# ErickRosete/tacorl

Hardware: NVIDIA B200
Metric: play_lmp_train_frames_per_sec (higher is better)
Workload: dtype bf16

## Files before the change

### include/tacorl_b200.h

```cpp
#ifndef TACORL_B200_H_
#define TACORL_B200_H_

#include <stddef.h>

#ifdef __cplusplus
extern "C" {
#endif

#define TACORL_B200_ABI_VERSION 7

#define TACORL_PREC_F32 0
#define TACORL_PREC_BF16 1

#define TACORL_ACT_NONE 0
#define TACORL_ACT_RELU 1
#define TACORL_ACT_SILU 2

const char* tacorl_last_error(void);
int tacorl_abi_version(void);
unsigned long long tacorl_launch_count(void);

int tacorl_set_sm_reserve(int n);

int tacorl_gemm(int transA, int transB, int M, int N, int K, float alpha, const float* A, long long lda,
                const float* B, long long ldb, float beta, float* C, long long ldc, const float* bias, int act,
                float* Cpre, long long ldpre, void* ws, size_t ws_bytes, int prec, void* stream);
int tacorl_gemm_ex(int transA, int transB, int M, int N, int K, float alpha, const float* A, long long lda,
                   const float* B, long long ldb, float beta, float* C, long long ldc, const float* bias, int act,
                   float* Cpre, long long ldpre, const void* A_bf16, const void* B_bf16, void* ws, size_t ws_bytes,
                   int prec, void* stream);
int tacorl_colsum(int M, int N, const float* X, long long ldx, float* out, int accumulate, void* stream);
int tacorl_act_bwd(int act, long long n, const float* dY, const float* y_or_pre, float* dZ, void* stream);
int tacorl_scale(long long n, const float* x, const float* dev_scalar, float c, float* out, void* stream);
int tacorl_rowscale(long long rows, int L, const float* x, const float* row_scalars, float k, float* out,
                    int accumulate, void* stream);

size_t tacorl_lmp_encoder_ws_bytes(int N, int H, int W, int hidden, int latent, int backward);
int tacorl_lmp_encoder_fwd(const void* x, int x_dtype, float x_scale, float x_shift, int N, int H, int W,
                           const float* const* params, int hidden,
                           int latent, float* y1, float* y2, float* y3, float* feat, float* smax,
                           float* ssum, float* h4, float* emb, void* xs, void* ws, size_t ws_bytes, int prec,
                           void* stream);
int tacorl_lmp_encoder_bwd(const void* x, int x_dtype, float x_scale, float x_shift, int N, int H, int W,
                           const float* const* params, int hidden,
                           int latent, const float* y1, const float* y2, const float* y3,
                           const float* feat, const float* smax, const float* ssum, const float* h4,
                           const float* d_emb, float* const* grads, int accumulate, const void* xs, void* ws,
                           size_t ws_bytes, int prec, void* stream);

int tacorl_conv_tc_debug(int op, const float* in0, const float* in1, const float* Wt, const float* bias, int N,
                         int H, int W, float* out, void* ws, size_t ws_bytes, void* stream);

size_t tacorl_rnn_layer_ws_bytes(int T, int B, int I, int H);
unsigned tacorl_rnn_seq_timeouts(void);
int tacorl_rnn_seq_enable(int on);
int tacorl_rnn_layer_fwd(int T, int B, int I, int H, const float* x, long long ldx, const float* w_ih,
                         const float* w_hh, const float* b_ih, const float* b_hh, const float* h0,
                         int reverse, int n_steps, float* out, long long ldo, const void* w_ih_bf16,
                         const void* w_hh_bf16, void* h_bf16_out, void* ws, size_t ws_bytes, int prec, void* stream);
int tacorl_rnn_layer_bwd(int T, int B, int I, int H, const float* x, long long ldx, const float* w_ih,
                         const float* w_hh, const float* h0, int reverse, int n_steps, const float* out,
                         long long ldo, float* dout, long long lddo, const float* dhn, float* dx,
                         long long lddx, int dx_accumulate, float* dw_ih, float* dw_hh, float* db_ih,
                         float* db_hh, int accumulate, float* dh0, const void* w_ih_bf16, const void* w_hh_t_bf16,
                         const void* h_bf16, void* ws, size_t ws_bytes, int prec, void* stream);
size_t tacorl_rnn_layer2_ws_bytes(int T, int B, int I, int H, int D);
int tacorl_rnn_layer2_fwd(int T, int B, int I, int H, int D, const float* x, long long ldx, const void* x_bf16,
                          long long ldxb, const float* const* w, const void* const* w_bf16, const int* n_steps,
                          float* out, long long ldo, void* out_bf16, void* ws, size_t ws_bytes, void* stream);
int tacorl_rnn_layer2_bwd(int T, int B, int grad_rows, int I, int H, int D, const float* x, long long ldx, const void* x_bf16,
                          long long ldxb, const float* const* w, const void* const* w_bf16, const int* n_steps,
                          const float* out, long long ldo, const void* out_bf16, float* dout, long long lddo,
                          void* dpre_bf16, float* dx, long long lddx, float* const* dw, void* ws, size_t ws_bytes,
                          void* stream);
int tacorl_cast_transpose_bf16(const float* src, int rows, int cols, void* dst, void* stream);

int tacorl_dlm_nll(int rows, int act_dims, const float* logits, long long ld, const float* actions,
                   long long lda, int num_classes, float act_min, float act_max, float gripper_alpha,
                   float* row_loss, float* loss_out, float* dlogits, long long ldd, void* stream);
int tacorl_dlm_sample(int rows, int act_dims, const float* logits, long long ld, const float* u1,
                      const float* u2, const float* actions, long long lda, float grip_lo, float grip_hi,
                      float* pred, float* hit, float* acc_out, void* stream);

int tacorl_gauss_head_fwd(int rows, int L, const float* raw, float* mean, float* stdv, void* stream);
int tacorl_gauss_head_bwd(int rows, int L, const float* raw, const float* stdv, const float* dmean,
                          const float* dstd, float* draw, void* stream);
int tacorl_softplus_head_fwd(int rows, int L, const float* raw, float min_std, float* mean, float* stdv,
                             void* stream);
int tacorl_softplus_head_bwd(int rows, int L, const float* raw, const float* dmean, const float* dstd,
                             float* draw, void* stream);
int tacorl_gripper_gumbel(int rows, int rows0, const float* logits, const float* u, int clamp_u, float* index,
                          float* action, void* stream);
int tacorl_gripper_logprob(int rows, int rows0, const float* logits, const float* index, float* logp, void* stream);
int tacorl_gripper_logprob_bwd(int rows, const float* logits, const float* index, const float* dlogp, float* dlogits,
                               void* stream);
int tacorl_kl_balanced(int B, int L, const float* mu_q, const float* sd_q, const float* mu_p,
                       const float* sd_p, float kl_alpha, int balancing, float* kl_out, float* dmu_q,
                       float* dsd_q, float* dmu_p, float* dsd_p, void* stream);
int tacorl_tanh_rsample_fwd(long long n, long long bcast, const float* mu, const float* sd, const float* eps,
                            float* a, float* z, int apply_tanh, void* stream);
int tacorl_tanh_rsample_bwd(long long n, const float* a, const float* eps, const float* da, const float* dz,
                            float* dmu, float* dsd, int apply_tanh, void* stream);
int tacorl_tanh_logprob(int rows, int L, int bcast_rows, const float* mu, const float* sd, const float* z,
                        int from_value, float* logp, float* gmu, float* gsd, float* gz, void* stream);

int tacorl_posemb_fwd(int B, int T, int D0, int D, const float* emb, const float* pos, const float* mask, float* x,
                      void* stream);
int tacorl_posemb_bwd(int B, int T, int D0, int D, const float* dx, const float* mask, float* demb, float* dpos,
                      void* stream);
int tacorl_attn_fwd(int B, int T, int D, int heads, const float* qkv, const float* amask, float* P, float* out,
                    void* stream);
int tacorl_attn_bwd(int B, int T, int D, int heads, const float* qkv, const float* amask, const float* P,
                    const float* dout, float* dqkv, void* stream);
int tacorl_add_ln_fwd(int rows, int D, const float* x, const float* r, const float* mask, const float* w,
                      const float* b, float eps, float* y, float* xhat, float* rstd, void* stream);
int tacorl_add_ln_bwd(int rows, int D, const float* dy, const float* xhat, const float* rstd, const float* w,
                      const float* mask, float* dx, float* dr, float* dw, float* db, void* stream);
int tacorl_mean_t_fwd(int B, int T, int C, const float* x, float* y, void* stream);
int tacorl_mean_t_bwd(int B, int T, int C, const float* dy, float* dx, void* stream);
int tacorl_mul(long long n, const float* a, const float* b, float* out, void* stream);

#define TACORL_CQL_NUM_SCALARS 14
int tacorl_cql_critic_loss(int B, int n, const float* q1_all, const float* q2_all, const float* lp_curr,
                           const float* lp_next, const float* tq1, const float* tq2, const float* reward,
                           const float* done, const float* log_alpha_prime, float rand_density, float discount,
                           float reward_scale, float gap, float conservative_weight, float temp,
                           int with_lagrange, float* scalars, float* dq1_all, float* dq2_all,
                           float* d_log_alpha_prime, void* stream);
int tacorl_cql_actor_loss(int mode, int B, const float* log_pi, const float* a, const float* b,
                          const float* log_alpha, float target_entropy, float* out, float* d_log_alpha,
                          float* d_log_pi, float* da, float* db, void* stream);

int tacorl_dp_unique_id(void* id128);
int tacorl_dp_allreduce_init(const void* id128, int rank, int world);
int tacorl_dp_allreduce_enqueue(void* buf, long long n, int dtype, void* stream);
int tacorl_dp_allreduce_wait(void* stream);
int tacorl_dp_allreduce_destroy(void);

int tacorl_window_gather_u8(const unsigned char* store, long long frames, int C, int H, int W, const int* start,
                            const int* window, const int* shift, int pad, int B, int T, unsigned char* out, void* stream);
int tacorl_actions_gather_pad(const float* store, long long frames, int A, const int* start, const int* window, int B,
                              int T, int zero_pad, float* out, void* stream);
int tacorl_color_jitter_u8(const unsigned char* x, long long N, int H, int W, const int* order, const float* factors,
                           float norm_mean, float norm_std, float* mean_ws, float* out, void* stream);

#define TACORL_REPLAY_MAX_IMAGES 8
#define TACORL_REPLAY_WINDOW 0
#define TACORL_REPLAY_OBS 1
#define TACORL_REPLAY_NEXT 2
#define TACORL_REPLAY_GOAL 3
typedef struct tacorl_replay_image {
  const unsigned char* store;
  unsigned char* out;
  const int* shift;
  int H; int W;
  int role;
  int shift_slot; int n_slots;
} tacorl_replay_image;
typedef struct tacorl_replay_jitter {
  int ops;
  float lo[3]; float span[3];
} tacorl_replay_jitter;
int tacorl_replay_sample(int kind, int B, int min_window, int max_window, int n_mod, int n_slots, int pad,
                         unsigned long long neg_thr, unsigned long long seed, int rank, long long* step_dev,
                         const int* ep_end, long long frames, const int* valid, long long n_valid,
                         const unsigned* geom_thr, int n_geom, int* tab, int* shift, long long* out64,
                         const tacorl_replay_jitter* jitter, int* jit_order, float* jit_factors, void* stream);
int tacorl_replay_gather(int B, int T, int pad, const int* tab, int n_images, const tacorl_replay_image* images,
                         const float* act_store, int A, int act_role, int zero_pad, float* act_out, void* stream);
int tacorl_replay_color_jitter(const unsigned char* x, int B, int nf, int H, int W, const int* order,
                               const float* factors, int n_slots, int slot0, float norm_mean, float norm_std,
                               float* mean_ws, float* out, void* stream);

#define TACORL_METRICS_MAX 32
typedef struct tacorl_metrics {
  const float* value[TACORL_METRICS_MAX];
  int k;
  int n;
} tacorl_metrics;
int tacorl_replay_sweep(int kind, int B, int n, int min_window, int max_window, unsigned long long neg_thr,
                        unsigned long long seed, int rank, long long* cursor_dev, const int* ep_end, long long frames,
                        const int* valid, long long n_valid, const unsigned* geom_thr, int n_geom, int* tab,
                        long long* out64, void* stream);
// ... 39 lines not shown
```

### tacorl_b200/_lib.py

```python
import ctypes
import os

import torch

_HERE = os.path.dirname(os.path.abspath(__file__))
LIB_PATH = os.path.join(_HERE, "lib", "libtacorl_b200.so")

PREC_F32, PREC_BF16 = 0, 1
ACT_NONE, ACT_RELU, ACT_SILU = 0, 1, 2
ACTS = {None: ACT_NONE, "none": ACT_NONE, "relu": ACT_RELU, "silu": ACT_SILU}

_lib = None

_vp, _i, _ll, _f, _sz = ctypes.c_void_p, ctypes.c_int, ctypes.c_longlong, ctypes.c_float, ctypes.c_size_t

_SIGS = {
    "tacorl_gemm": [_i, _i, _i, _i, _i, _f, _vp, _ll, _vp, _ll, _f, _vp, _ll, _vp, _i, _vp, _ll, _vp, _sz, _i, _vp],
    "tacorl_gemm_ex": [_i, _i, _i, _i, _i, _f, _vp, _ll, _vp, _ll, _f, _vp, _ll, _vp, _i, _vp, _ll, _vp, _vp, _vp, _sz, _i,
                       _vp],
    "tacorl_colsum": [_i, _i, _vp, _ll, _vp, _i, _vp],
    "tacorl_act_bwd": [_i, _ll, _vp, _vp, _vp, _vp],
    "tacorl_scale": [_ll, _vp, _vp, _f, _vp, _vp],
    "tacorl_rowscale": [_ll, _i, _vp, _vp, _f, _vp, _i, _vp],
    "tacorl_lmp_encoder_ws_bytes": [_i, _i, _i, _i, _i, _i],
    "tacorl_lmp_encoder_fwd": [_vp, _i, _f, _f, _i, _i, _i, _vp, _i, _i, _vp, _vp, _vp, _vp, _vp, _vp, _vp, _vp, _vp, _vp, _sz, _i, _vp],
    "tacorl_lmp_encoder_bwd": [_vp, _i, _f, _f, _i, _i, _i, _vp, _i, _i, _vp, _vp, _vp, _vp, _vp, _vp, _vp, _vp, _vp, _i,
                               _vp, _vp, _sz, _i, _vp],
    "tacorl_conv_tc_debug": [_i, _vp, _vp, _vp, _vp, _i, _i, _i, _vp, _vp, _sz, _vp],
    "tacorl_rnn_layer_ws_bytes": [_i, _i, _i, _i],
    "tacorl_rnn_layer_fwd": [_i, _i, _i, _i, _vp, _ll, _vp, _vp, _vp, _vp, _vp, _i, _i, _vp, _ll, _vp, _vp, _vp, _vp, _sz,
                             _i, _vp],
    "tacorl_rnn_layer_bwd": [_i, _i, _i, _i, _vp, _ll, _vp, _vp, _vp, _i, _i, _vp, _ll, _vp, _ll, _vp, _vp, _ll, _i,
                             _vp, _vp, _vp, _vp, _i, _vp, _vp, _vp, _vp, _vp, _sz, _i, _vp],
    "tacorl_rnn_layer2_ws_bytes": [_i, _i, _i, _i, _i],
    "tacorl_rnn_layer2_fwd": [_i, _i, _i, _i, _i, _vp, _ll, _vp, _ll, _vp, _vp, _vp, _vp, _ll, _vp, _vp, _sz, _vp],
    "tacorl_rnn_layer2_bwd": [_i, _i, _i, _i, _i, _i, _vp, _ll, _vp, _ll, _vp, _vp, _vp, _vp, _ll, _vp, _vp, _ll, _vp, _vp, _ll,
                              _vp, _vp, _sz, _vp],
    "tacorl_cast_transpose_bf16": [_vp, _i, _i, _vp, _vp],
    "tacorl_dlm_nll": [_i, _i, _vp, _ll, _vp, _ll, _i, _f, _f, _f, _vp, _vp, _vp, _ll, _vp],
    "tacorl_dlm_sample": [_i, _i, _vp, _ll, _vp, _vp, _vp, _ll, _f, _f, _vp, _vp, _vp, _vp],
    "tacorl_gauss_head_fwd": [_i, _i, _vp, _vp, _vp, _vp],
    "tacorl_gauss_head_bwd": [_i, _i, _vp, _vp, _vp, _vp, _vp, _vp],
    "tacorl_softplus_head_fwd": [_i, _i, _vp, _f, _vp, _vp, _vp],
    "tacorl_softplus_head_bwd": [_i, _i, _vp, _vp, _vp, _vp, _vp],
    "tacorl_kl_balanced": [_i, _i, _vp, _vp, _vp, _vp, _f, _i, _vp, _vp, _vp, _vp, _vp, _vp],
    "tacorl_tanh_rsample_fwd": [_ll, _ll, _vp, _vp, _vp, _vp, _vp, _i, _vp],
    "tacorl_tanh_rsample_bwd": [_ll, _vp, _vp, _vp, _vp, _vp, _vp, _i, _vp],
    "tacorl_tanh_logprob": [_i, _i, _i, _vp, _vp, _vp, _i, _vp, _vp, _vp, _vp, _vp],
    "tacorl_gripper_gumbel": [_i, _i, _vp, _vp, _i, _vp, _vp, _vp],
    "tacorl_gripper_logprob": [_i, _i, _vp, _vp, _vp, _vp],
    "tacorl_gripper_logprob_bwd": [_i, _vp, _vp, _vp, _vp, _vp],
    "tacorl_posemb_fwd": [_i, _i, _i, _i, _vp, _vp, _vp, _vp, _vp],
    "tacorl_posemb_bwd": [_i, _i, _i, _i, _vp, _vp, _vp, _vp, _vp],
    "tacorl_attn_fwd": [_i, _i, _i, _i, _vp, _vp, _vp, _vp, _vp],
    "tacorl_attn_bwd": [_i, _i, _i, _i, _vp, _vp, _vp, _vp, _vp, _vp],
    "tacorl_add_ln_fwd": [_i, _i, _vp, _vp, _vp, _vp, _vp, _f, _vp, _vp, _vp, _vp],
    "tacorl_add_ln_bwd": [_i, _i, _vp, _vp, _vp, _vp, _vp, _vp, _vp, _vp, _vp, _vp],
    "tacorl_mean_t_fwd": [_i, _i, _i, _vp, _vp, _vp],
    "tacorl_mean_t_bwd": [_i, _i, _i, _vp, _vp, _vp],
    "tacorl_mul": [_ll, _vp, _vp, _vp, _vp],
    "tacorl_cql_critic_loss": [_i, _i, _vp, _vp, _vp, _vp, _vp, _vp, _vp, _vp, _vp, _f, _f, _f, _f, _f, _f, _i,
                               _vp, _vp, _vp, _vp, _vp],
    "tacorl_cql_actor_loss": [_i, _i, _vp, _vp, _vp, _vp, _f, _vp, _vp, _vp, _vp, _vp, _vp],
    "tacorl_dp_unique_id": [_vp],
    "tacorl_dp_allreduce_init": [_vp, _i, _i],
    "tacorl_dp_allreduce_enqueue": [_vp, _ll, _i, _vp],
    "tacorl_dp_allreduce_wait": [_vp],
    "tacorl_dp_allreduce_destroy": [],
    "tacorl_window_gather_u8": [_vp, _ll, _i, _i, _i, _vp, _vp, _vp, _i, _i, _i, _vp, _vp],
    "tacorl_actions_gather_pad": [_vp, _ll, _i, _vp, _vp, _i, _i, _i, _vp, _vp],
    "tacorl_color_jitter_u8": [_vp, _ll, _i, _i, _vp, _vp, _f, _f, _vp, _vp, _vp],
    "tacorl_replay_sample": [_i, _i, _i, _i, _i, _i, _i, ctypes.c_ulonglong, ctypes.c_ulonglong, _i, _vp, _vp, _ll, _vp,
                             _ll, _vp, _i, _vp, _vp, _vp, _vp, _vp, _vp, _vp],
    "tacorl_replay_gather": [_i, _i, _i, _vp, _i, _vp, _vp, _i, _i, _i, _vp, _vp],
    "tacorl_replay_color_jitter": [_vp, _i, _i, _i, _i, _vp, _vp, _i, _i, _f, _f, _vp, _vp, _vp],
    "tacorl_replay_sweep": [_i, _i, _i, _i, _i, ctypes.c_ulonglong, ctypes.c_ulonglong, _i, _vp, _vp, _ll, _vp, _ll, _vp,
                            _i, _vp, _vp, _vp],
    "tacorl_replay_gather_rows": [_i, _i, _i, _i, _vp, _i, _vp, _vp, _i, _i, _i, _vp, _vp],
    "tacorl_metrics_accumulate": [_vp, _vp, _vp],
    "tacorl_metrics_record": [_vp, _vp, _i, _vp, _vp, _vp],
    "tacorl_mlp_chain_ws_bytes": [_i, _i, _vp],
    "tacorl_mlp_chain_fwd": [_i, _i, _vp, _vp, _i, _ll, _vp, _i, _ll, _vp, _ll, _vp, _ll, _vp],
    "tacorl_mlp_chain_bwd": [_i, _i, _vp, _vp, _i, _ll, _vp, _i, _ll, _vp, _ll, _vp, _ll, _vp, _ll, _vp, _ll, _vp, _sz, _vp],
    "tacorl_adam_step": [_ll, _vp, _vp, _vp, _vp, _f, _f, _f, _f, _i, _vp, _f, _vp, _f, _vp, _vp],
    "tacorl_adam_step_range": [_ll, _vp, _vp, _vp, _vp, _f, _f, _f, _f, _i, _vp, _i, _i, _f, _vp, _f, _vp, _vp],
    "tacorl_polyak_update": [_ll, _vp, _vp, _f, _vp],
    "tacorl_sqnorm": [_ll, _vp, _vp, _vp, _vp],
    "tacorl_last_error": [],
    "tacorl_abi_version": [],
    "tacorl_launch_count": [],
    "tacorl_rnn_seq_timeouts": [],
    "tacorl_rnn_seq_enable": [_i],
    "tacorl_set_sm_reserve": [_i],
}
_RESTYPES = {
    "tacorl_lmp_encoder_ws_bytes": _sz, "tacorl_rnn_layer_ws_bytes": _sz, "tacorl_rnn_layer2_ws_bytes": _sz,
    "tacorl_mlp_chain_ws_bytes": _sz,
    "tacorl_last_error": ctypes.c_char_p, "tacorl_launch_count": ctypes.c_ulonglong,
    "tacorl_rnn_seq_timeouts": ctypes.c_uint,
}
EXPORTED = tuple(_SIGS)


class TacorlLibraryError(RuntimeError):
    pass


class MlpLayer(ctypes.Structure):
    _fields_ = [("W0", _vp), ("b0", _vp), ("n0", _i), ("W1", _vp), ("b1", _vp), ("n1", _i),
                ("W2", _vp), ("b2", _vp), ("n2", _i), ("in_", _i), ("act", _i),
                ("dW0", _vp), ("db0", _vp), ("dW1", _vp), ("db1", _vp), ("dW2", _vp), ("db2", _vp)]


class ReplayImage(ctypes.Structure):
    _fields_ = [("store", _vp), ("out", _vp), ("shift", _vp), ("H", _i), ("W", _i), ("role", _i),
                ("shift_slot", _i), ("n_slots", _i)]


class ReplayJitter(ctypes.Structure):
    _fields_ = [("ops", _i), ("lo", _f * 3), ("span", _f * 3)]


REPLAY_WINDOW, REPLAY_OBS, REPLAY_NEXT, REPLAY_GOAL = 0, 1, 2, 3
REPLAY_MAX_IMAGES = 8
METRICS_MAX = 32


class Metrics(ctypes.Structure):
    _fields_ = [("value", _vp * METRICS_MAX), ("k", _i), ("n", _i)]


def lib():
    global _lib
    if _lib is None:
        if not os.path.exists(LIB_PATH):
            raise TacorlLibraryError(
                f"{LIB_PATH} not found: the CUDA extension is not built (run "
                "`python tacorl_b200/csrc/build.py`).  tacorl_b200 has no CPU / eager fallback.")
        L = ctypes.CDLL(LIB_PATH)
        for name, args in _SIGS.items():
            fn = getattr(L, name)
            fn.argtypes = args
            fn.restype = _RESTYPES.get(name, ctypes.c_int)
        _lib = L
    return _lib


def call(name, *args):
    L = lib()
    rc = getattr(L, name)(*args)
    if rc != 0:
        raise TacorlLibraryError(f"{name} failed ({rc}): {L.tacorl_last_error().decode()}")


def query(name, *args):
    return getattr(lib(), name)(*args)


def launch_count():
    return int(lib().tacorl_launch_count())


def stream():
    return ctypes.c_void_p(torch.cuda.current_stream().cuda_stream)


def ptr(t, allow_none=True):
    if t is None:
        if allow_none:
            return None
        raise TacorlLibraryError("null tensor")
    if not t.is_cuda:
        raise TacorlLibraryError("tacorl_b200 ops need CUDA tensors (there is no CPU fallback)")
    if t.dtype != torch.float32:
        raise TacorlLibraryError(f"expected float32, got {t.dtype}")
    return ctypes.c_void_p(t.data_ptr())


def ptr_any(t):
    if t is None:
        return None
    if not t.is_cuda:
        raise TacorlLibraryError("tacorl_b200 ops need CUDA tensors (there is no CPU fallback)")
    return ctypes.c_void_p(t.data_ptr())


def ptr_array(tensors):
    arr = (ctypes.c_void_p * len(tensors))()
    for i, t in enumerate(tensors):
        arr[i] = None if t is None else t.data_ptr()
    return arr


def int_array(values):
    return (ctypes.c_int * len(values))(*[int(v) for v in values])


_WS = {}
_WS_RETIRED = []


def workspace(nbytes, device, tag="main"):
    if torch.device(device).type != "cuda":
        raise TacorlLibraryError("tacorl_b200 ops need CUDA tensors (there is no CPU fallback)")
    key = (device.index if device.index is not None else torch.cuda.current_device(), tag)
    buf = _WS.get(key)
    if buf is None or buf.numel() < nbytes:
        if buf is not None:
            _WS_RETIRED.append(buf)
        buf = torch.empty(int(nbytes * 1.25) + 4096, dtype=torch.uint8, device=device)
        _WS[key] = buf
    return buf
```

### tacorl_b200/csrc/api.cu

```cuda
#include "common.cuh"
#include "internal.h"
#include "../../include/tacorl_b200.h"

using namespace tacorl;

namespace tacorl {
static int g_sm_reserve = -1;
int persistent_ctas() {
  if (g_sm_reserve < 0) { const char* e = getenv("TACORL_SM_RESERVE"); g_sm_reserve = e ? atoi(e) : 0; }
  const int n = 148 - g_sm_reserve;
  return n < 8 ? 8 : n;
}
void set_sm_reserve(int n) { g_sm_reserve = n < 0 ? 0 : (n > 140 ? 140 : n); }
}

extern "C" {

const char* tacorl_last_error(void) { return last_error(); }

int tacorl_abi_version(void) { return TACORL_B200_ABI_VERSION; }

unsigned long long tacorl_launch_count(void) { return launch_count(); }

unsigned tacorl_rnn_seq_timeouts(void) { return rnn_seq_timeouts(); }

int tacorl_set_sm_reserve(int n) { set_sm_reserve(n); return persistent_ctas(); }

int tacorl_rnn_seq_enable(int on) { const int was = rnn_seq_mode(); rnn_seq_set_enabled(on); return was; }

int tacorl_gemm_ex(int transA, int transB, int M, int N, int K, float alpha, const float* A, long long lda,
                   const float* B, long long ldb, float beta, float* C, long long ldc, const float* bias, int act,
                   float* Cpre, long long ldpre, const void* A_bf16, const void* B_bf16, void* ws, size_t ws_bytes,
                   int prec, void* stream) {
  TACORL_REQUIRE(prec == PREC_F32 || prec == PREC_BF16, "gemm: unknown precision %d", prec);
  GemmArgs g;
  g.transA = transA; g.transB = transB; g.M = M; g.N = N; g.K = K; g.alpha = alpha;
  g.A = A; g.lda = lda; g.B = B; g.ldb = ldb; g.beta = beta; g.C = C; g.ldc = ldc; g.bias = bias;
  g.act = act; g.Cpre = Cpre; g.ldpre = ldpre; g.split_k = 0; g.A_bf16 = A_bf16; g.B_bf16 = B_bf16;
  return gemm_any(prec, g, (float*)ws, ws_bytes, (cudaStream_t)stream);
}

int tacorl_gemm(int transA, int transB, int M, int N, int K, float alpha, const float* A, long long lda,
                const float* B, long long ldb, float beta, float* C, long long ldc, const float* bias, int act,
                float* Cpre, long long ldpre, void* ws, size_t ws_bytes, int prec, void* stream) {
  return tacorl_gemm_ex(transA, transB, M, N, K, alpha, A, lda, B, ldb, beta, C, ldc, bias, act, Cpre, ldpre, nullptr,
                        nullptr, ws, ws_bytes, prec, stream);
}

int tacorl_colsum(int M, int N, const float* X, long long ldx, float* out, int accumulate, void* stream) {
  TACORL_REQUIRE(X && out, "colsum: null pointer");
  return colsum_f32(M, N, X, ldx, out, accumulate, (cudaStream_t)stream);
}

int tacorl_act_bwd(int act, long long n, const float* dY, const float* y_or_pre, float* dZ, void* stream) {
  TACORL_REQUIRE(dY && y_or_pre && dZ, "act_bwd: null pointer");
  return act_bwd_f32(act, n, dY, y_or_pre, dZ, (cudaStream_t)stream);
}

}
```

### tacorl_b200/csrc/gemm_tc.cu

```cuda
#include "common.cuh"
#include "internal.h"
#include <cuda.h>
#include <cuda_bf16.h>
#include <algorithm>

namespace tacorl {

constexpr int TC_BM = 128;
constexpr int TC_BK = 64;
constexpr int TC_UMMA_K = 16;
constexpr int TC_THREADS = 192;

__device__ __forceinline__ uint32_t smem_u32(const void* p) { return (uint32_t)__cvta_generic_to_shared(p); }

__device__ __forceinline__ void mbar_init(uint32_t bar, uint32_t count) {
  asm volatile("mbarrier.init.shared::cta.b64 [%0], %1;" ::"r"(bar), "r"(count));
}
__device__ __forceinline__ void mbar_expect_tx(uint32_t bar, uint32_t bytes) {
  asm volatile("mbarrier.arrive.expect_tx.shared::cta.b64 _, [%0], %1;" ::"r"(bar), "r"(bytes) : "memory");
}
__device__ __forceinline__ void mbar_wait(uint32_t bar, uint32_t parity) {
  uint32_t done;
  do {
    asm volatile(
// ... 4 lines not shown
  } while (!done);
}
__device__ __forceinline__ void tma_load_2d(uint32_t dst, const CUtensorMap* tm, int c0, int c1, uint32_t bar) {
  asm volatile(
      "cp.async.bulk.tensor.2d.shared::cluster.global.mbarrier::complete_tx::bytes [%0], [%1, {%2, %3}], [%4];"
      ::"r"(dst), "l"(tm), "r"(c0), "r"(c1), "r"(bar) : "memory");
}
__device__ __forceinline__ void tc_fence_before() { asm volatile("tcgen05.fence::before_thread_sync;" ::: "memory"); }
__device__ __forceinline__ void tc_fence_after() { asm volatile("tcgen05.fence::after_thread_sync;" ::: "memory"); }
__device__ __forceinline__ void tc_commit(uint32_t bar) {
  asm volatile("tcgen05.commit.cta_group::1.mbarrier::arrive::one.shared::cluster.b64 [%0];" ::"r"(bar) : "memory");
}
__device__ __forceinline__ void tc_mma_bf16(uint32_t tmem_d, uint64_t adesc, uint64_t bdesc, uint32_t idesc,
                                            uint32_t accumulate) {
  asm volatile(
      "{\n\t.reg .pred p;\n\t"
      "setp.ne.b32 p, %4, 0;\n\t"
      "tcgen05.mma.cta_group::1.kind::f16 [%0], %1, %2, %3, p;\n\t}"
      ::"r"(tmem_d), "l"(adesc), "l"(bdesc), "r"(idesc), "r"(accumulate) : "memory");
}
__device__ __forceinline__ void tc_ld16(uint32_t taddr, uint32_t (&r)[16]) {
  asm volatile(
      "tcgen05.ld.sync.aligned.32x32b.x16.b32 {%0,%1,%2,%3,%4,%5,%6,%7,%8,%9,%10,%11,%12,%13,%14,%15}, [%16];"
      : "=r"(r[0]), "=r"(r[1]), "=r"(r[2]), "=r"(r[3]), "=r"(r[4]), "=r"(r[5]), "=r"(r[6]), "=r"(r[7]),
        "=r"(r[8]), "=r"(r[9]), "=r"(r[10]), "=r"(r[11]), "=r"(r[12]), "=r"(r[13]), "=r"(r[14]), "=r"(r[15])
      : "r"(taddr));
  asm volatile("tcgen05.wait::ld.sync.aligned;" ::: "memory");
}

__device__ __forceinline__ void tc_ld16_nowait(uint32_t taddr, uint32_t (&r)[16]) {
  asm volatile(
      "tcgen05.ld.sync.aligned.32x32b.x16.b32 {%0,%1,%2,%3,%4,%5,%6,%7,%8,%9,%10,%11,%12,%13,%14,%15}, [%16];"
      : "=r"(r[0]), "=r"(r[1]), "=r"(r[2]), "=r"(r[3]), "=r"(r[4]), "=r"(r[5]), "=r"(r[6]), "=r"(r[7]),
        "=r"(r[8]), "=r"(r[9]), "=r"(r[10]), "=r"(r[11]), "=r"(r[12]), "=r"(r[13]), "=r"(r[14]), "=r"(r[15])
      : "r"(taddr));
}
__device__ __forceinline__ void tc_ld_wait() { asm volatile("tcgen05.wait::ld.sync.aligned;" ::: "memory"); }

__device__ __forceinline__ uint64_t make_smem_desc(uint32_t saddr, uint32_t lbo_bytes, uint32_t sbo_bytes) {
  uint64_t d = 0;
  d |= (uint64_t)((saddr >> 4) & 0x3FFF);
  d |= (uint64_t)((lbo_bytes >> 4) & 0x3FFF) << 16;
  d |= (uint64_t)((sbo_bytes >> 4) & 0x3FFF) << 32;
  d |= (uint64_t)1 << 46;
  d |= (uint64_t)2 << 61;
  return d;
}

struct TcEpilogue {
  float alpha, beta;
  float* C; long long ldc;
  __nv_bfloat16* Cb; long long ldcb;
  const float* bias;
  int act;
  float* Cpre; long long ldpre;
  float* partial;
  const float* gate; long long ldgate;
};

__device__ __forceinline__ void mbar_arrive(uint32_t bar) {
  asm volatile("mbarrier.arrive.shared::cta.b64 _, [%0];" ::"r"(bar) : "memory");
}

__device__ __forceinline__ void tc_epilogue_chunk(const TcEpilogue& ep, const uint32_t (&r)[16], int row, int col0,
                                                  int N, int zslice, int M) {
  const bool full = col0 + 16 <= N;
  if (ep.partial) {
    float* P = ep.partial + ((long long)zslice * M + row) * N + col0;
    if (full && (N & 3) == 0) {
#pragma unroll
      for (int j = 0; j < 4; ++j)
        reinterpret_cast<float4*>(P)[j] = make_float4(__uint_as_float(r[4 * j]), __uint_as_float(r[4 * j + 1]),
                                                      __uint_as_float(r[4 * j + 2]), __uint_as_float(r[4 * j + 3]));
    } else {
#pragma unroll
      for (int j = 0; j < 16; ++j)
        if (col0 + j < N) P[j] = __uint_as_float(r[j]);
    }
    return;
  }
  float v[16];
#pragma unroll
  for (int j = 0; j < 16; ++j) v[j] = ep.alpha * __uint_as_float(r[j]);
  float* Crow = ep.C ? ep.C + (long long)row * ep.ldc + col0 : nullptr;
  const bool vecC = full && Crow && ((ep.ldc & 3) == 0) && ((reinterpret_cast<uintptr_t>(ep.C) & 15) == 0);
  if (ep.beta != 0.f && Crow) {
    if (vecC) {
#pragma unroll
      for (int j = 0; j < 4; ++j) {
        const float4 c = reinterpret_cast<const float4*>(Crow)[j];
        v[4 * j] = fmaf(ep.beta, c.x, v[4 * j]); v[4 * j + 1] = fmaf(ep.beta, c.y, v[4 * j + 1]);
        v[4 * j + 2] = fmaf(ep.beta, c.z, v[4 * j + 2]); v[4 * j + 3] = fmaf(ep.beta, c.w, v[4 * j + 3]);
      }
    } else {
#pragma unroll
      for (int j = 0; j < 16; ++j)
        if (col0 + j < N) v[j] = fmaf(ep.beta, Crow[j], v[j]);
    }
  }
  if (ep.bias) {
#pragma unroll
    for (int j = 0; j < 16; ++j)
      if (col0 + j < N) v[j] += __ldg(ep.bias + col0 + j);
  }
  if (ep.Cpre) {
    float* Prow = ep.Cpre + (long long)row * ep.ldpre + col0;
#pragma unroll
    for (int j = 0; j < 16; ++j)
      if (col0 + j < N) Prow[j] = v[j];
  }
  if (ep.act == ACT_RELU) {
#pragma unroll
    for (int j = 0; j < 16; ++j) v[j] = fmaxf(v[j], 0.f);
  } else if (ep.act == ACT_SILU) {
#pragma unroll
    for (int j = 0; j < 16; ++j) v[j] = v[j] / (1.f + __expf(-v[j]));
  }
  if (ep.gate) {
    const float* Grow = ep.gate + (long long)row * ep.ldgate + col0;
#pragma unroll
    for (int j = 0; j < 16; ++j)
      if (col0 + j < N && Grow[j] <= 0.f) v[j] = 0.f;
  }
  if (Crow) {
    if (vecC) {
#pragma unroll
      for (int j = 0; j < 4; ++j)
        reinterpret_cast<float4*>(Crow)[j] = make_float4(v[4 * j], v[4 * j + 1], v[4 * j + 2], v[4 * j + 3]);
    } else {
#pragma unroll
      for (int j = 0; j < 16; ++j)
        if (col0 + j < N) Crow[j] = v[j];
    }
  }
  if (ep.Cb) {
    __nv_bfloat16* Brow = ep.Cb + (long long)row * ep.ldcb + col0;
    if (full && ((ep.ldcb & 7) == 0) && ((reinterpret_cast<uintptr_t>(ep.Cb) & 15) == 0)) {
      uint32_t pk[8];
#pragma unroll
      for (int j = 0; j < 8; ++j) {
        __nv_bfloat162 t = __floats2bfloat162_rn(v[2 * j], v[2 * j + 1]);
        pk[j] = *reinterpret_cast<uint32_t*>(&t);
      }
      reinterpret_cast<uint4*>(Brow)[0] = make_uint4(pk[0], pk[1], pk[2], pk[3]);
      reinterpret_cast<uint4*>(Brow)[1] = make_uint4(pk[4], pk[5], pk[6], pk[7]);
    } else {
#pragma unroll
      for (int j = 0; j < 16; ++j)
        if (col0 + j < N) Brow[j] = __float2bfloat16(v[j]);
    }
  }
}

template <int BN, bool A_MN, bool B_MN, int kStages>
__global__ void __launch_bounds__(TC_THREADS, 1)
gemm_tc_kernel(const __grid_constant__ CUtensorMap tmA, const __grid_constant__ CUtensorMap tmB, TcEpilogue ep,
               int M, int N, int K, int kblocks_per_split) {
  constexpr uint32_t A_BYTES = TC_BM * TC_BK * 2;
  constexpr uint32_t B_BYTES = BN * TC_BK * 2;
  constexpr uint32_t STAGE_BYTES = A_BYTES + B_BYTES;
  constexpr uint32_t ACC_COLS = BN < 32 ? 32 : BN;
  constexpr uint32_t TMEM_COLS = 2 * ACC_COLS;
  static_assert(!B_MN || BN % 64 == 0, "MN-major B needs 64-wide boxes");
  extern __shared__ __align__(1024) uint8_t smem_raw[];
  uint8_t* smem = (uint8_t*)(((uintptr_t)smem_raw + 1023) & ~(uintptr_t)1023);
  uint64_t* bars = (uint64_t*)(smem + kStages * STAGE_BYTES);
  uint32_t* tmem_slot = (uint32_t*)(bars + 2 * kStages + 4);

  const int warp = threadIdx.x >> 5, lane = threadIdx.x & 31;
  const int total_kb = (K + TC_BK - 1) / TC_BK;
  const int kb_begin = blockIdx.z * kblocks_per_split;
  const int kb_end = min(total_kb, kb_begin + kblocks_per_split);
  const int nkb = kb_end - kb_begin;
  const int tiles_n = (N + BN - 1) / BN;
  const int num_tiles = ((M + TC_BM - 1) / TC_BM) * tiles_n;

  const uint32_t smem_base = smem_u32(smem);
  auto full_bar = [&](int s) { return smem_u32(bars + s); };
  auto empty_bar = [&](int s) { return smem_u32(bars + kStages + s); };
  auto tfull_bar = [&](int a) { return smem_u32(bars + 2 * kStages + a); };
  auto tempty_bar = [&](int a) { return smem_u32(bars + 2 * kStages + 2 + a); };

  if (threadIdx.x == 0) {
    for (int s = 0; s < kStages; ++s) { mbar_init(full_bar(s), 1); mbar_init(empty_bar(s), 1); }
    for (int a = 0; a < 2; ++a) { mbar_init(tfull_bar(a), 1); mbar_init(tempty_bar(a), 4); }
    asm volatile("fence.mbarrier_init.release.cluster;" ::: "memory");
  }
  if (warp == 1) {
    asm volatile("tcgen05.alloc.cta_group::1.sync.aligned.shared::cta.b32 [%0], %1;"
                 ::"r"(smem_u32(tmem_slot)), "r"(TMEM_COLS) : "memory");
    asm volatile("tcgen05.relinquish_alloc_permit.cta_group::1.sync.aligned;" ::: "memory");
  }
  tc_fence_before();
  __syncthreads();
  tc_fence_after();
  const uint32_t tmem_base = *tmem_slot;

  if (warp == 0) {
    if (lane == 0 && nkb > 0) {
      uint32_t it = 0;
      for (int tile = blockIdx.x; tile < num_tiles; tile += gridDim.x) {
        const int m0 = (tile / tiles_n) * TC_BM, n0 = (tile % tiles_n) * BN;
        for (int i = 0; i < nkb; ++i, ++it) {
          const int s = it % kStages;
          const uint32_t ph = (it / kStages) & 1;
          mbar_wait(empty_bar(s), ph ^ 1);
          mbar_expect_tx(full_bar(s), STAGE_BYTES);
          const int k0 = (kb_begin + i) * TC_BK;
          const uint32_t a_dst = smem_base + s * STAGE_BYTES, b_dst = a_dst + A_BYTES;
          if (!A_MN) {
            tma_load_2d(a_dst, &tmA, k0, m0, full_bar(s));
          } else {
            tma_load_2d(a_dst, &tmA, m0, k0, full_bar(s));
            tma_load_2d(a_dst + 8192, &tmA, m0 + 64, k0, full_bar(s));
          }
          if (!B_MN) {
            tma_load_2d(b_dst, &tmB, k0, n0, full_bar(s));
          } else {
#pragma unroll
            for (int j = 0; j < BN / 64; ++j) tma_load_2d(b_dst + j * 8192, &tmB, n0 + j * 64, k0, full_bar(s));
          }
        }
      }
    }
  } else if (warp == 1) {
    if (lane == 0 && nkb > 0) {
      const uint32_t idesc = (1u << 4) | (1u << 7) | (1u << 10) | ((A_MN ? 1u : 0u) << 15) | ((B_MN ? 1u : 0u) << 16) |
                             ((uint32_t)(BN >> 3) << 17) | ((uint32_t)(TC_BM >> 4) << 24);
      uint32_t it = 0, lt = 0;
      for (int tile = blockIdx.x; tile < num_tiles; tile += gridDim.x, ++lt) {
        const uint32_t acc = lt & 1;
        mbar_wait(tempty_bar(acc), ((lt >> 1) & 1) ^ 1);
        tc_fence_after();
        const uint32_t tmem_d = tmem_base + acc * ACC_COLS;
        for (int i = 0; i < nkb; ++i, ++it) {
          const int s = it % kStages;
          const uint32_t ph = (it / kStages) & 1;
          mbar_wait(full_bar(s), ph);
          tc_fence_after();
          const uint32_t a_src = smem_base + s * STAGE_BYTES, b_src = a_src + A_BYTES;
#pragma unroll
          for (int k = 0; k < TC_BK / TC_UMMA_K; ++k) {
            const uint64_t ad = A_MN ? make_smem_desc(a_src + k * 2048, 8192, 1024) : make_smem_desc(a_src + k * 32, 16, 1024);
            const uint64_t bd = B_MN ? make_smem_desc(b_src + k * 2048, 8192, 1024) : make_smem_desc(b_src + k * 32, 16, 1024);
            tc_mma_bf16(tmem_d, ad, bd, idesc, (i > 0 || k > 0) ? 1u : 0u);
          }
          tc_commit(empty_bar(s));
        }
        tc_commit(tfull_bar(acc));
      }
    }
  } else {
    const int q = warp & 3;
    uint32_t lt = 0;
    for (int tile = blockIdx.x; tile < num_tiles; tile += gridDim.x, ++lt) {
      const int m0 = (tile / tiles_n) * TC_BM, n0 = (tile % tiles_n) * BN;
      const int row = m0 + q * 32 + lane;
      const uint32_t acc = lt & 1;
      if (nkb > 0) {
        mbar_wait(tfull_bar(acc), (lt >> 1) & 1);
        tc_fence_after();
      }
#pragma unroll 1
      for (int c0 = 0; c0 < BN; c0 += 16) {
        uint32_t r[16];
        if (nkb > 0) {
          tc_ld16(tmem_base + acc * ACC_COLS + ((uint32_t)(q * 32) << 16) + c0, r);
        } else {
#pragma unroll
          for (int j = 0; j < 16; ++j) r[j] = 0;
        }
        if (row < M && n0 + c0 < N) tc_epilogue_chunk(ep, r, row, n0 + c0, N, blockIdx.z, M);
      }
      if (nkb > 0) {
        tc_fence_before();
        __syncwarp();
        if (lane == 0) mbar_arrive(tempty_bar(acc));
      }
    }
  }
  tc_fence_before();
  __syncthreads();
  if (warp == 1) {
    tc_fence_after();
    asm volatile("tcgen05.dealloc.cta_group::1.sync.aligned.b32 %0, %1;" ::"r"(tmem_base), "r"(TMEM_COLS) : "memory");
  }
}


constexpr int RS_KS = 8;
constexpr int RS_MAX_TILES = 15;
constexpr int RS_EPI = 512;
constexpr int RS_THREADS = RS_EPI + 32;
constexpr int RS_MAXE = 2;
#ifdef TACORL_STEP_PROFILE
__device__ unsigned long long g_step_prof[16];
__device__ unsigned long long g_cta_prof[2][256][2];
#define RS_CTA_STAMP(which)                                                              \
  if (tid == 0) {                                                                        \
    const int c_ = blockIdx.y * gridDim.x + blockIdx.x;                                  \
    unsigned long long t_;                                                               \
    asm volatile("mov.u64 %0, %%globaltimer;" : "=l"(t_));                             \
    if (which == 0) { g_cta_prof[0][c_][0] = g_cta_prof[1][c_][0]; g_cta_prof[0][c_][1] = g_cta_prof[1][c_][1]; } \
    g_cta_prof[1][c_][which] = t_;                                                       \
  }
#define RS_STAMP(i)                                                                      \
  if (tid == 0 && blockIdx.x == 0 && blockIdx.y == 0) {                                  \
    unsigned long long t_;                                                               \
    asm volatile("mov.u64 %0, %%globaltimer;" : "=l"(t_));                             \
    g_step_prof[i] = t_;                                                                 \
  }                                                                                      \
  __syncwarp();
#define RS_STAMP_T(i)                                                                    \
  if (blockIdx.x == 0 && blockIdx.y == 0) {                                              \
    unsigned long long t_;                                                               \
    asm volatile("mov.u64 %0, %%globaltimer;" : "=l"(t_));                             \
    g_step_prof[i] = t_;                                                                 \
  }
#else
#define RS_STAMP(i)
#define RS_STAMP_T(i)
#define RS_CTA_STAMP(which)
#endif

__device__ __forceinline__ void cluster_sync_all() {
  asm volatile("barrier.cluster.arrive.release.aligned;" ::: "memory");
  asm volatile("barrier.cluster.wait.acquire.aligned;" ::: "memory");
}
__device__ __forceinline__ float4 ld_dsmem_v4(uint32_t local_addr, uint32_t cta) {
  uint32_t remote;
  float4 v;
  asm volatile("mapa.shared::cluster.u32 %0, %1, %2;" : "=r"(remote) : "r"(local_addr), "r"(cta));
  asm volatile("ld.shared::cluster.v4.f32 {%0, %1, %2, %3}, [%4];" : "=f"(v.x), "=f"(v.y), "=f"(v.z), "=f"(v.w) : "r"(remote)
               : "memory");
  return v;
}

__global__ void __cluster_dims__(RS_KS, 1, 1) __launch_bounds__(RS_THREADS, 1)
skinny_cluster_kernel(const __grid_constant__ CUtensorMap tmA, const __grid_constant__ CUtensorMap tmW,
                      const TcEpilogue ep, int M, int Mpad, int N, int NT, int kb_per_cta) {
  extern __shared__ __align__(1024) uint8_t smem_raw[];
  uint8_t* smem = (uint8_t*)(((uintptr_t)smem_raw + 1023) & ~(uintptr_t)1023);
  const uint32_t A_TILE = 128 * 128, W_BYTES = (uint32_t)NT * 128, STAGE = A_TILE + ((W_BYTES + 1023) & ~1023u);
  const int SP = NT + 4;
  const int per = Mpad / RS_KS;
  const size_t stage_total = (size_t)kb_per_cta * STAGE, s_bytes = (size_t)Mpad * SP * 4;
  float* S = (float*)smem;
  uint64_t* bars = (uint64_t*)(smem + (stage_total > s_bytes ? stage_total : ((s_bytes + 1023) & ~(size_t)1023)));
  uint32_t* tmem_slot = (uint32_t*)(bars + 9);
  const int tid = threadIdx.x, warp = tid >> 5, lane = tid & 31;
  const uint32_t rank = blockIdx.x;
  const int n0 = blockIdx.y * NT;
  const uint32_t tmem_cols = NT <= 32 ? 32 : (NT <= 64 ? 64 : (NT <= 128 ? 128 : 256));
  const uint32_t done_bar = smem_u32(bars + 8);
  RS_CTA_STAMP(0)
  RS_STAMP(0)

  if (tid == RS_EPI) {
    for (int s = 0; s < kb_per_cta; ++s) mbar_init(smem_u32(bars + s), 1);
    mbar_init(done_bar, 1);
    asm volatile("fence.mbarrier_init.release.cluster;" ::: "memory");
  }
  if (warp == RS_EPI / 32) {
    asm volatile("tcgen05.alloc.cta_group::1.sync.aligned.shared::cta.b32 [%0], %1;"
                 ::"r"(smem_u32(tmem_slot)), "r"(tmem_cols) : "memory");
    asm volatile("tcgen05.relinquish_alloc_permit.cta_group::1.sync.aligned;" ::: "memory");
  }
  tc_fence_before();
  __syncthreads();
  tc_fence_after();
  const uint32_t tmem_base = *tmem_slot;
  RS_STAMP(1)

  if (tid == RS_EPI) {
    const int k_begin = (int)rank * kb_per_cta * TC_BK;
    for (int s = 0; s < kb_per_cta; ++s) {
      const uint32_t bar = smem_u32(bars + s), dst = smem_u32(smem + (size_t)s * STAGE);
      mbar_expect_tx(bar, (uint32_t)Mpad * 128 + W_BYTES);
      tma_load_2d(dst, &tmA, k_begin + s * TC_BK, 0, bar);
      tma_load_2d(dst + A_TILE, &tmW, k_begin + s * TC_BK, n0, bar);
    }
    const uint32_t idesc = (1u << 4) | (1u << 7) | (1u << 10) | ((uint32_t)(NT >> 3) << 17) | ((uint32_t)(128 >> 4) << 24);
    RS_STAMP_T(2)
    for (int s = 0; s < kb_per_cta; ++s) {
      mbar_wait(smem_u32(bars + s), 0);
      tc_fence_after();
      if (s == 0) { RS_STAMP_T(3) }
      const uint32_t a_src = smem_u32(smem + (size_t)s * STAGE), w_src = a_src + A_TILE;
#pragma unroll
      for (int k = 0; k < TC_BK / TC_UMMA_K; ++k)
        tc_mma_bf16(tmem_base, make_smem_desc(a_src + k * 32, 16, 1024), make_smem_desc(w_src + k * 32, 16, 1024), idesc,
                    (s > 0 || k > 0) ? 1u : 0u);
    }
    tc_commit(done_bar);
    RS_STAMP_T(4)
  }
  const int NT4 = NT >> 2, elems = per * NT4;
  float4 cold[RS_MAXE], gt[RS_MAXE], bs[RS_MAXE];
  if (tid < RS_EPI) {
    long long offc[RS_MAXE], offg[RS_MAXE];
    int colc[RS_MAXE];
#pragma unroll
    for (int i = 0; i < RS_MAXE; ++i) {
      const int e = tid + i * RS_EPI;
      const int bi = e / NT4, n = (e - bi * NT4) * 4, b = (int)rank * per + bi, col = n0 + n;
#ifdef RS_EXP_NOPREFETCH
      const bool ok = false;
#else
      const bool ok = e < elems && b < M && col < N;
#endif
      offc[i] = ok ? (long long)b * ep.ldc + col : 0;
      offg[i] = ok ? (long long)b * ep.ldgate + col : 0;
      colc[i] = ok ? col : 0;
    }
    const bool has_c = ep.beta != 0.f && ep.C != nullptr;
    const float4 zero = make_float4(0.f, 0.f, 0.f, 0.f), one = make_float4(1.f, 1.f, 1.f, 1.f);
#pragma unroll
    for (int i = 0; i < RS_MAXE; ++i) cold[i] = has_c ? *reinterpret_cast<const float4*>(ep.C + offc[i]) : zero;
#pragma unroll
    for (int i = 0; i < RS_MAXE; ++i) gt[i] = ep.gate ? *reinterpret_cast<const float4*>(ep.gate + offg[i]) : one;
#pragma unroll
    for (int i = 0; i < RS_MAXE; ++i) bs[i] = ep.bias ? __ldg(reinterpret_cast<const float4*>(ep.bias + colc[i])) : zero;
  }
#ifdef TACORL_STEP_PROFILE
  RS_STAMP(12)
#endif
  if (tid < RS_EPI) {
    mbar_wait(done_bar, 0);
    tc_fence_after();
  }
// ... 452 lines not shown
      long long offc[RS_MAXE], offg[RS_MAXE];
#pragma unroll
      for (int i = 0; i < RS_MAXE; ++i) {
        const int e = tid + i * RS_EPI;
        const int bi = e / NT4, n = (e - bi * NT4) * 4, b = (int)rank * per + bi, col = n0 + n;
        const bool ok = e < elems && b < M && col < N;
        offc[i] = ok ? (long long)b * sa.ldc + col : 0;
        offg[i] = ok ? (long long)b * sa.ldgate + col : 0;
      }
      const float4 zero = make_float4(0.f, 0.f, 0.f, 0.f), one = make_float4(1.f, 1.f, 1.f, 1.f);
#pragma unroll
      for (int i = 0; i < RS_MAXE; ++i) cold[i] = sa.beta != 0.f ? *reinterpret_cast<const float4*>(Ct + offc[i]) : zero;
#pragma unroll
      for (int i = 0; i < RS_MAXE; ++i) gt[i] = Gt ? *reinterpret_cast<const float4*>(Gt + offg[i]) : one;
      mbar_wait(done_bar, ph);
      tc_fence_after();
      if (tid == 0) { WV_STAMP(5) }
    }
    if (step > 0) asm volatile("barrier.cluster.wait.aligned;" ::: "memory");
    if (tid == 0) { WV_STAMP(3) }
    if (warp < RS_EPI / 32) {
      const int q = warp & 3;
      if (q * 32 < Mpad) {
        float* Srow = S + (q * 32 + lane) * SP;
        uint32_t r[2][16];
#pragma unroll
        for (int i = 0; i < 2; ++i) {
          const int c0 = (warp >> 2) * 16 + 64 * i;
          if (c0 < NT) tc_ld16_nowait(tmem_base + ((uint32_t)(q * 32) << 16) + c0, r[i]);
        }
        tc_ld_wait();
#pragma unroll
        for (int i = 0; i < 2; ++i) {
          const int c0 = (warp >> 2) * 16 + 64 * i;
          if (c0 < NT) {
#pragma unroll
            for (int j = 0; j < 4; ++j)
              reinterpret_cast<float4*>(Srow + c0)[j] = make_float4(__uint_as_float(r[i][4 * j]), __uint_as_float(r[i][4 * j + 1]),
                                                                    __uint_as_float(r[i][4 * j + 2]), __uint_as_float(r[i][4 * j + 3]));
          }
        }
      }
    }
    tc_fence_before();
    if (tid == 0) { WV_STAMP(6) }
    cluster_sync_all();
    tc_fence_after();
    if (tid == 0) { WV_STAMP(7) }
    float4 acc[RS_MAXE];
    if (warp < RS_EPI / 32) {
      float4 part[RS_MAXE][RW_KS];
#pragma unroll
      for (int i = 0; i < RS_MAXE; ++i) {
        const int e = tid + i * RS_EPI;
        const int bi = e / NT4, n = (e - bi * NT4) * 4;
        const uint32_t addr = smem_u32(S + ((int)rank * per + (e < elems ? bi : 0)) * SP + (e < elems ? n : 0));
#pragma unroll
        for (int q = 0; q < RW_KS; ++q) part[i][q] = ld_dsmem_v4(addr, (q + rank) & (RW_KS - 1));
      }
#pragma unroll
      for (int i = 0; i < RS_MAXE; ++i) {
        float4 v = make_float4(0.f, 0.f, 0.f, 0.f);
#pragma unroll
        for (int q = 0; q < RW_KS; ++q) { v.x += part[i][q].x; v.y += part[i][q].y; v.z += part[i][q].z; v.w += part[i][q].w; }
        acc[i] = v;
      }
      float dep = 0.f;
#pragma unroll
      for (int i = 0; i < RS_MAXE; ++i) dep += acc[i].x + acc[i].y + acc[i].z + acc[i].w;
      asm volatile("barrier.cluster.arrive.release.aligned;" ::"f"(dep) : "memory");
      if (tid == 0) { WV_STAMP(8) }
      float* Ct = sa.C + (long long)tau * sa.c_ts;
      __nv_bfloat16* Bt = sa.Cb + (long long)tau * sa.cb_ts;
      float4 outv[RS_MAXE];
      bool okv[RS_MAXE];
#pragma unroll
      for (int i = 0; i < RS_MAXE; ++i) {
        const int e = tid + i * RS_EPI;
        const int bi = e / NT4, n = (e - bi * NT4) * 4, b = (int)rank * per + bi, col = n0 + n;
        okv[i] = e < elems && b < M && col < N;
        float v[4] = {acc[i].x, acc[i].y, acc[i].z, acc[i].w};
        const float c4[4] = {cold[i].x, cold[i].y, cold[i].z, cold[i].w};
        const float g4[4] = {gt[i].x, gt[i].y, gt[i].z, gt[i].w};
#pragma unroll
        for (int j = 0; j < 4; ++j) {
          v[j] = fmaf(sa.beta, c4[j], v[j]);
          if (sa.act == ACT_RELU) v[j] = fmaxf(v[j], 0.f);
          if (g4[j] <= 0.f) v[j] = 0.f;
        }
        outv[i] = make_float4(v[0], v[1], v[2], v[3]);
        if (okv[i]) {
          __nv_bfloat162 lo = __floats2bfloat162_rn(v[0], v[1]), hi = __floats2bfloat162_rn(v[2], v[3]);
          *reinterpret_cast<uint2*>(Bt + (long long)b * sa.ldcb + col) =
              make_uint2(*reinterpret_cast<uint32_t*>(&lo), *reinterpret_cast<uint32_t*>(&hi));
        }
      }
      asm volatile("fence.proxy.async.global;" ::: "memory");
      if (tid == 0) { WV_STAMP(9) }
      asm volatile("bar.sync 1, %0;" ::"n"(RS_EPI) : "memory");
      if (tid == 0) { red_release_gpu_add(&g_rnn_flags[blockIdx.z][tile], 1u); WV_STAMP(10) }
#pragma unroll
      for (int i = 0; i < RS_MAXE; ++i) {
        const int e = tid + i * RS_EPI;
        const int bi = e / NT4, n = (e - bi * NT4) * 4, b = (int)rank * per + bi, col = n0 + n;
        if (okv[i]) *reinterpret_cast<float4*>(Ct + (long long)b * sa.ldc + col) = outv[i];
      }
      if (tid == 0) { WV_STAMP(11) }
    } else {
      asm volatile("barrier.cluster.arrive.release.aligned;" ::: "memory");
    }
  }
  if (sa.n_steps > 0) asm volatile("barrier.cluster.wait.aligned;" ::: "memory");
  if (warp == RS_EPI / 32) {
    tc_fence_after();
    asm volatile("tcgen05.dealloc.cta_group::1.sync.aligned.b32 %0, %1;" ::"r"(tmem_base), "r"(tmem_cols) : "memory");
  }
  rnn_launch_epilogue(tid);
}

typedef CUresult (*EncodeTiledFn)(CUtensorMap*, CUtensorMapDataType, cuuint32_t, void*, const cuuint64_t*,
                                  const cuuint64_t*, const cuuint32_t*, const cuuint32_t*, CUtensorMapInterleave,
                                  CUtensorMapSwizzle, CUtensorMapL2promotion, CUtensorMapFloatOOBfill);

static EncodeTiledFn get_encode_fn() {
  static EncodeTiledFn fn = nullptr;
  if (!fn) {
    void* p = nullptr;
    cudaDriverEntryPointQueryResult q;
    if (cudaGetDriverEntryPoint("cuTensorMapEncodeTiled", &p, cudaEnableDefault, &q) == cudaSuccess &&
        q == cudaDriverEntryPointSuccess)
      fn = (EncodeTiledFn)p;
  }
  return fn;
}

static int make_tmap(CUtensorMap* tm, const void* base, long long inner, long long outer, long long ld,
                     int box_inner, int box_outer) {
  EncodeTiledFn fn = get_encode_fn();
  TACORL_REQUIRE(fn, "gemm_tc: cuTensorMapEncodeTiled is not available from the driver");
  TACORL_REQUIRE(((uintptr_t)base & 15) == 0 && (ld * 2) % 16 == 0,
                 "gemm_tc: TMA operand must be 16-byte aligned with a 16-byte multiple pitch (ld=%lld)", ld);
  cuuint64_t dims[2] = {(cuuint64_t)inner, (cuuint64_t)outer};
  cuuint64_t strides[1] = {(cuuint64_t)ld * 2};
  cuuint32_t box[2] = {(cuuint32_t)box_inner, (cuuint32_t)box_outer};
  cuuint32_t estr[2] = {1, 1};
  CUresult r = fn(tm, CU_TENSOR_MAP_DATA_TYPE_BFLOAT16, 2, const_cast<void*>(base), dims, strides, box, estr,
                  CU_TENSOR_MAP_INTERLEAVE_NONE, CU_TENSOR_MAP_SWIZZLE_128B, CU_TENSOR_MAP_L2_PROMOTION_L2_256B,
                  CU_TENSOR_MAP_FLOAT_OOB_FILL_NONE);
  TACORL_REQUIRE(r == CUDA_SUCCESS, "gemm_tc: cuTensorMapEncodeTiled failed (%d) inner=%lld outer=%lld ld=%lld", (int)r,
                 inner, outer, ld);
  return 0;
}

template <int BN, bool A_MN, bool B_MN>
static int launch_tc(const CUtensorMap& ta, const CUtensorMap& tb, const TcEpilogue& ep, int M, int N, int K,
                     int splits, cudaStream_t st) {
  constexpr int kStages = BN >= 128 ? 5 : 6;
  constexpr size_t smem = (size_t)kStages * (TC_BM * TC_BK * 2 + BN * TC_BK * 2) + (2 * kStages + 4) * 8 + 16 + 1024;
  static bool configured = false;
  auto kern = gemm_tc_kernel<BN, A_MN, B_MN, kStages>;
  if (!configured) {
    TACORL_CHECK_CUDA(cudaFuncSetAttribute(kern, cudaFuncAttributeMaxDynamicSharedMemorySize, (int)smem));
    configured = true;
  }
  const int total_kb = cdiv(K, TC_BK);
  const int per = cdiv(total_kb, splits);
  const int zs = cdiv(total_kb, per);
  const long long tiles = (long long)cdiv(N, BN) * cdiv(M, TC_BM);
  const int ctas = (int)min(tiles, (long long)max(1, 148 / zs));
  dim3 grid(ctas, 1, zs);
  kern<<<grid, TC_THREADS, smem, st>>>(ta, tb, ep, M, N, K, per);
  TACORL_LAUNCH_CHECK();
  return 0;
}

__global__ void tc_splitk_reduce_kernel(int M, int N, int splits, const float* __restrict__ partial, TcEpilogue ep) {
  const long long total = (long long)M * N;
  for (long long idx = blockIdx.x * (long long)blockDim.x + threadIdx.x; idx < total;
       idx += (long long)gridDim.x * blockDim.x) {
    const int row = (int)(idx / N), col = (int)(idx % N);
    float s = 0.f;
    for (int z = 0; z < splits; ++z) s += partial[(long long)z * total + idx];
    float v = ep.alpha * s;
    if (ep.beta != 0.f && ep.C) v = fmaf(ep.beta, ep.C[(long long)row * ep.ldc + col], v);
    if (ep.bias) v += __ldg(ep.bias + col);
    if (ep.Cpre) ep.Cpre[(long long)row * ep.ldpre + col] = v;
    if (ep.act == ACT_RELU) v = fmaxf(v, 0.f);
    else if (ep.act == ACT_SILU) v = v / (1.f + __expf(-v));
    if (ep.gate && ep.gate[(long long)row * ep.ldgate + col] <= 0.f) v = 0.f;
    if (ep.C) ep.C[(long long)row * ep.ldc + col] = v;
    if (ep.Cb) ep.Cb[(long long)row * ep.ldcb + col] = __float2bfloat16(v);
  }
}

static int launch_skinny_cluster(const void* A, long long lda, const void* W, long long ldw, int M, int N, int K,
                                 const TcEpilogue& ep, cudaStream_t st) {
  if (M < 1 || M > 128 || K % (TC_BK * RS_KS) != 0 || N % 4 != 0) return 1;
  auto al16 = [](const void* p, long long ld, int elt) { return p == nullptr || (((uintptr_t)p & 15) == 0 && (ld * elt) % 16 == 0); };
  if (!al16(ep.C, ep.ldc, 4) || !al16(ep.gate, ep.ldgate, 4) || !al16(ep.Cpre, ep.ldpre, 4) || !al16(ep.bias, 4, 4) ||
      !(ep.Cb == nullptr || (((uintptr_t)ep.Cb & 7) == 0 && ep.ldcb % 4 == 0)))
    return 1;
  const int Mpad = (M + 15) & ~15, kb = K / (TC_BK * RS_KS);
  const int NT = 16 * cdiv(N, 16 * RS_MAX_TILES), tiles = cdiv(N, NT);
  if (NT > 256 || kb > 8 || (Mpad / RS_KS) * (NT / 4) > RS_MAXE * RS_EPI) return 1;
  const size_t stage = 128 * 128 + (((size_t)NT * 128 + 1023) & ~(size_t)1023);
  const size_t s_bytes = ((size_t)Mpad * (NT + 4) * 4 + 1023) & ~(size_t)1023;
  const size_t smem = std::max((size_t)kb * stage, s_bytes) + 9 * 8 + 16 + 1024;
  if (smem > 227 * 1024) return 1;
  CUtensorMap ta, tw;
  int rc;
  if ((rc = make_tmap(&ta, A, K, M, lda, 64, Mpad))) return rc;
  if ((rc = make_tmap(&tw, W, K, N, ldw, 64, NT))) return rc;
  static size_t configured = 0;
  if (smem > configured) {
    TACORL_CHECK_CUDA(cudaFuncSetAttribute(skinny_cluster_kernel, cudaFuncAttributeMaxDynamicSharedMemorySize, (int)smem));
    configured = smem;
  }
  skinny_cluster_kernel<<<dim3(RS_KS, tiles), RS_THREADS, smem, st>>>(ta, tw, ep, M, Mpad, N, NT, kb);
  TACORL_LAUNCH_CHECK();
  return 0;
}

static int g_rnn_seq_enabled = -1;
bool rnn_seq_enabled() {
  if (g_rnn_seq_enabled < 0) { const char* e = getenv("TACORL_RNN_SEQ"); g_rnn_seq_enabled = !(e && e[0] == '0'); }
  return g_rnn_seq_enabled != 0;
}
void rnn_seq_set_enabled(int on) { g_rnn_seq_enabled = on < 0 ? 0 : (on > 2 ? 2 : on); }
int rnn_seq_mode() { rnn_seq_enabled(); return g_rnn_seq_enabled; }

static cudaEvent_t g_chain_ev[64] = {};
static cudaStream_t g_chain_stream[64] = {};
static unsigned long long g_chain_capture[64] = {};
static bool g_chain_recorded[64] = {};
static int chain_slot(cudaStream_t st, int* dev, unsigned long long* cid) {
  TACORL_CHECK_CUDA(cudaGetDevice(dev));
  TACORL_REQUIRE(*dev >= 0 && *dev < 64, "persistent launch: device index %d out of range", *dev);
  cudaStreamCaptureStatus cs = cudaStreamCaptureStatusNone;
  *cid = 0;
  TACORL_CHECK_CUDA(cudaStreamGetCaptureInfo(st, &cs, cid));
  if (cs != cudaStreamCaptureStatusActive) *cid = 0;
  if (!g_chain_ev[*dev]) TACORL_CHECK_CUDA(cudaEventCreateWithFlags(&g_chain_ev[*dev], cudaEventDisableTiming));
  return 0;
}
static int persistent_chain_enter(cudaStream_t st) {
  int dev; unsigned long long cid; int rc;
  if ((rc = chain_slot(st, &dev, &cid))) return rc;
  if (g_chain_recorded[dev] && g_chain_capture[dev] == cid && g_chain_stream[dev] != st)
    TACORL_CHECK_CUDA(cudaStreamWaitEvent(st, g_chain_ev[dev], 0));
  return 0;
}
static int persistent_chain_leave(cudaStream_t st) {
  int dev; unsigned long long cid; int rc;
  if ((rc = chain_slot(st, &dev, &cid))) return rc;
  TACORL_CHECK_CUDA(cudaEventRecord(g_chain_ev[dev], st));
  g_chain_recorded[dev] = true; g_chain_capture[dev] = cid; g_chain_stream[dev] = st;
  return 0;
}

int rnn_seq_tc(const void* Ab, int T, const void* W, long long ldw, int M, int N, int K, int tau0, int dtau, int n_steps,
               float beta, float* C, long long ldc, long long c_ts, const float* gate, long long ldgate, long long gate_ts,
               void* Cb, int act, unsigned* flags, cudaStream_t st) {
  if (!rnn_seq_enabled() || n_steps < 2) return 1;
  if (M < 1 || M > 128 || K != N || K % (TC_BK * RS_KS) != 0 || N % 4 != 0 || !Cb || !C || !flags) return 1;
  auto al16 = [](const void* p, long long ld) { return p == nullptr || (((uintptr_t)p & 15) == 0 && (ld * 4) % 16 == 0); };
  if (!al16(C, ldc) || !al16(C, c_ts) || !al16(gate, ldgate) || !al16(gate, gate_ts) || ((uintptr_t)Cb & 15) != 0) return 1;
  const int Mpad = (M + 15) & ~15, kb = K / (TC_BK * RS_KS);
  const int NT = 16 * cdiv(N, 16 * RS_MAX_TILES), tiles = cdiv(N, NT);
  if (NT > 256 || kb > 8 || (Mpad / RS_KS) * (NT / 4) > RS_MAXE * RS_EPI) return 1;
  const size_t w_stage = ((size_t)NT * 128 + 1023) & ~(size_t)1023;
  const size_t s_bytes = ((size_t)((Mpad + 31) & ~31) * (NT + 4) * 4 + 1023) & ~(size_t)1023;
  const size_t smem = (size_t)kb * (w_stage + 128 * 128) + s_bytes + 10 * 8 + 16 + 1024;
  if (smem > 227 * 1024) return 1;
  static size_t configured = 0;
  if (smem > configured) {
    TACORL_CHECK_CUDA(cudaFuncSetAttribute(rnn_seq_kernel, cudaFuncAttributeMaxDynamicSharedMemorySize, (int)smem));
    configured = smem;
  }
  {
    static size_t checked_smem = 0;
    static int max_clusters = 0;
    if (checked_smem != smem) {
      cudaLaunchConfig_t cfg = {};
      cfg.gridDim = dim3(RS_KS, tiles); cfg.blockDim = dim3(RS_THREADS); cfg.dynamicSmemBytes = smem;
      cudaLaunchAttribute at[1];
      at[0].id = cudaLaunchAttributeClusterDimension;
      at[0].val.clusterDim.x = RS_KS; at[0].val.clusterDim.y = 1; at[0].val.clusterDim.z = 1;
      cfg.attrs = at; cfg.numAttrs = 1;
      int n = 0;
      if (cudaOccupancyMaxActiveClusters(&n, rnn_seq_kernel, &cfg) != cudaSuccess) { cudaGetLastError(); n = 0; }
      max_clusters = n; checked_smem = smem;
    }
    if (max_clusters < tiles) return 1;
  }
  CUtensorMap ta, tw;
  int rc;
  {
    EncodeTiledFn fn = get_encode_fn();
    TACORL_REQUIRE(fn, "rnn_seq: cuTensorMapEncodeTiled is not available from the driver");
    TACORL_REQUIRE(((uintptr_t)Ab & 15) == 0, "rnn_seq: hidden-state buffer must be 16-byte aligned");
    cuuint64_t dims[3] = {(cuuint64_t)K, (cuuint64_t)M, (cuuint64_t)T};
    cuuint64_t strides[2] = {(cuuint64_t)K * 2, (cuuint64_t)M * K * 2};
    cuuint32_t box[3] = {64, (cuuint32_t)Mpad, 1};
    cuuint32_t estr[3] = {1, 1, 1};
    CUresult r = fn(&ta, CU_TENSOR_MAP_DATA_TYPE_BFLOAT16, 3, const_cast<void*>(Ab), dims, strides, box, estr,
                    CU_TENSOR_MAP_INTERLEAVE_NONE, CU_TENSOR_MAP_SWIZZLE_128B, CU_TENSOR_MAP_L2_PROMOTION_L2_256B,
                    CU_TENSOR_MAP_FLOAT_OOB_FILL_NONE);
    TACORL_REQUIRE(r == CUDA_SUCCESS, "rnn_seq: cuTensorMapEncodeTiled failed (%d) K=%d M=%d T=%d", (int)r, K, M, T);
  }
  if ((rc = make_tmap(&tw, W, K, N, ldw, 64, NT))) return rc;
  SeqArgs sa;
  sa.n_steps = n_steps; sa.tau0 = tau0; sa.dtau = dtau; sa.beta = beta; sa.C = C; sa.ldc = ldc; sa.c_ts = c_ts;
  sa.gate = gate; sa.ldgate = ldgate; sa.gate_ts = gate_ts; sa.Cb = (__nv_bfloat16*)Cb; sa.cb_ts = (long long)M * N;
  sa.act = act; sa.flags = flags;
  int rc2;
  if ((rc2 = persistent_chain_enter(st))) return rc2;
  rnn_seq_kernel<<<dim3(RS_KS, tiles), RS_THREADS, smem, st>>>(ta, tw, sa, M, Mpad, N, NT, kb);
  TACORL_LAUNCH_CHECK();
  if ((rc2 = persistent_chain_leave(st))) return rc2;
  return 0;
}

int rnn_wave_tc(const WaveLaneHost* lanes, int n_lanes, int T, int M, int N, int K, cudaStream_t st) {
  if (!rnn_seq_enabled() || n_lanes < 1 || n_lanes > 2) return 1;
  if (n_lanes == 2 && rnn_seq_mode() == 2) {
    int rc = rnn_wave_tc(lanes, 1, T, M, N, K, st);
    return rc ? rc : rnn_wave_tc(lanes + 1, 1, T, M, N, K, st);
  }
  if (M < 1 || M > 64 || K != N || K % (TC_BK * RW_KS) != 0 || N % 4 != 0) return 1;
  const int Mpad = (M + 15) & ~15, kb = K / (TC_BK * RW_KS);
  const int NT = 16 * cdiv(N, 16 * RW_MAX_TILES), tiles = cdiv(N, NT);
  if (NT > 128 || kb > 8 || (Mpad / RW_KS) * (NT / 4) > RS_MAXE * RS_EPI) return 1;
  auto al16 = [](const void* p, long long ld) { return p == nullptr || (((uintptr_t)p & 15) == 0 && (ld * 4) % 16 == 0); };
  int max_steps = 0;
  for (int l = 0; l < n_lanes; ++l) {
    const WaveLaneHost& h = lanes[l];
    if (!h.Ab || !h.W || !h.C || !h.Cb || !h.flags || h.n_steps < 0) return 1;
    if (!al16(h.C, h.ldc) || !al16(h.C, h.c_ts) || !al16(h.gate, h.ldgate) || !al16(h.gate, h.gate_ts)) return 1;
    if (((uintptr_t)h.Cb & 7) != 0 || h.ldcb % 4 != 0 || h.cb_ts % 4 != 0) return 1;
    if (((uintptr_t)h.Ab & 15) != 0 || (h.lda * 2) % 16 != 0 || (h.a_ts * 2) % 16 != 0) return 1;
    max_steps = std::max(max_steps, h.n_steps);
  }
  if (max_steps < 2) return 1;
  const size_t w_stage = ((size_t)NT * 128 + 1023) & ~(size_t)1023, a_pitch = (size_t)Mpad * 128;
  const size_t s_bytes = ((size_t)((Mpad + 31) & ~31) * (NT + 4) * 4 + 1023) & ~(size_t)1023;
  const size_t tail = std::max(a_pitch + s_bytes + 256, (size_t)16384 + 256);
  const size_t smem = (size_t)kb * w_stage + (size_t)(kb - 1) * a_pitch + tail + 1024;
  if (smem > 227 * 1024) return 1;
  static size_t configured = 0;
  if (smem > configured) {
    TACORL_CHECK_CUDA(cudaFuncSetAttribute(rnn_wave_kernel, cudaFuncAttributeMaxDynamicSharedMemorySize, (int)smem));
    TACORL_CHECK_CUDA(cudaFuncSetAttribute(rnn_wave_kernel, cudaFuncAttributeNonPortableClusterSizeAllowed, 0));
    configured = smem;
  }
  cudaLaunchConfig_t cfg = {};
  cfg.gridDim = dim3(RW_KS, tiles, n_lanes); cfg.blockDim = dim3(RS_THREADS); cfg.dynamicSmemBytes = smem; cfg.stream = st;
  cudaLaunchAttribute at[1];
  at[0].id = cudaLaunchAttributeClusterDimension;
  at[0].val.clusterDim.x = RW_KS; at[0].val.clusterDim.y = 1; at[0].val.clusterDim.z = 1;
  cfg.attrs = at; cfg.numAttrs = 1;
  {
    static size_t checked_smem = 0;
    static int max_clusters = 0;
    if (checked_smem != smem) {
      int n = 0;
      if (cudaOccupancyMaxActiveClusters(&n, rnn_wave_kernel, &cfg) != cudaSuccess) { cudaGetLastError(); n = 0; }
      max_clusters = n; checked_smem = smem;
    }
    if (max_clusters < tiles * n_lanes) return 1;
  }
  EncodeTiledFn fn = get_encode_fn();
  TACORL_REQUIRE(fn, "rnn_wave: cuTensorMapEncodeTiled is not available from the driver");
  CUtensorMap ta[2], tw[2];
  WaveArgs wa;
  int rc;
  for (int l = 0; l < 2; ++l) {
    const WaveLaneHost& h = lanes[l < n_lanes ? l : 0];
    cuuint64_t dims[3] = {(cuuint64_t)K, (cuuint64_t)M, (cuuint64_t)T};
    cuuint64_t strides[2] = {(cuuint64_t)h.lda * 2, (cuuint64_t)h.a_ts * 2};
    cuuint32_t box[3] = {64, (cuuint32_t)Mpad, 1};
    cuuint32_t estr[3] = {1, 1, 1};
    CUresult r = fn(&ta[l], CU_TENSOR_MAP_DATA_TYPE_BFLOAT16, 3, const_cast<void*>(h.Ab), dims, strides, box, estr,
                    CU_TENSOR_MAP_INTERLEAVE_NONE, CU_TENSOR_MAP_SWIZZLE_128B, CU_TENSOR_MAP_L2_PROMOTION_L2_256B,
                    CU_TENSOR_MAP_FLOAT_OOB_FILL_NONE);
    TACORL_REQUIRE(r == CUDA_SUCCESS, "rnn_wave: cuTensorMapEncodeTiled failed (%d) K=%d M=%d T=%d", (int)r, K, M, T);
    if ((rc = make_tmap(&tw[l], h.W, K, N, h.ldw, 64, NT))) return rc;
    WaveLane& d = wa.lane[l];
    d.n_steps = l < n_lanes ? h.n_steps : 0; d.tau0 = h.tau0; d.dtau = h.dtau; d.act = h.act; d.beta = h.beta;
    d.C = h.C; d.ldc = h.ldc; d.c_ts = h.c_ts; d.gate = h.gate; d.ldgate = h.ldgate; d.gate_ts = h.gate_ts;
    d.Cb = (__nv_bfloat16*)h.Cb; d.ldcb = h.ldcb; d.cb_ts = h.cb_ts; d.flags = h.flags;
  }
  if ((rc = persistent_chain_enter(st))) return rc;
  void* args[] = {&ta[0], &tw[0], &ta[1], &tw[1], &wa, (void*)&M, (void*)&Mpad, (void*)&N, (void*)&NT, (void*)&kb};
  TACORL_CHECK_CUDA(cudaLaunchKernelExC(&cfg, (const void*)rnn_wave_kernel, args));
  note_launch();
  if ((rc = persistent_chain_leave(st))) return rc;
  return 0;
}

unsigned rnn_seq_timeouts() {
  unsigned v = 0;
  cudaMemcpyFromSymbol(&v, g_rnn_seq_timeouts, sizeof(v));
  return v;
}

int gemm_tc_bf16(const void* A, long long lda, int a_mn, const void* B, long long ldb, int b_mn, int M, int N,
                 int K, const TcArgs& e, float* ws, size_t ws_bytes, cudaStream_t st) {
  if (M == 0 || N == 0) return 0;
  TACORL_REQUIRE(K > 0, "gemm_tc: K must be positive");
  int BN = N <= 32 ? 32 : (N <= 64 ? 64 : 128);
  const bool skinny = M <= TC_BM && N >= 512 && K <= 8192 && e.split_k == 0;
  if (skinny) BN = b_mn ? 64 : 32;
  if (b_mn && BN < 64) BN = 64;
  int rc;
  if (skinny && !a_mn && !b_mn) {
    TcEpilogue ep;
    ep.alpha = e.alpha; ep.beta = e.beta; ep.C = e.C; ep.ldc = e.ldc; ep.Cb = (__nv_bfloat16*)e.Cb; ep.ldcb = e.ldcb;
    ep.bias = e.bias; ep.act = e.act; ep.Cpre = e.Cpre; ep.ldpre = e.ldpre; ep.partial = nullptr;
    ep.gate = e.gate; ep.ldgate = e.ldgate;
    rc = launch_skinny_cluster(A, lda, B, ldb, M, N, K, ep, st);
    if (rc <= 0) return rc;
  }
  CUtensorMap ta, tb;
  if ((rc = a_mn ? make_tmap(&ta, A, M, K, lda, 64, 64) : make_tmap(&ta, A, K, M, lda, 64, TC_BM))) return rc;
  if ((rc = b_mn ? make_tmap(&tb, B, N, K, ldb, 64, 64) : make_tmap(&tb, B, K, N, ldb, 64, BN))) return rc;
  const long long ctas = (long long)cdiv(M, TC_BM) * cdiv(N, BN);
  const int total_kb = cdiv(K, TC_BK);
  int splits = e.split_k;
  if (splits <= 0) {
    splits = 1;
    if (ws && !skinny && ctas < 74 && total_kb >= 8) splits = (int)min((long long)cdiv(148, ctas), (long long)(total_kb / 4));
  }
  if (splits > total_kb) splits = total_kb;
  if (splits > 1 && (!ws || (size_t)splits * M * N * 4 > ws_bytes)) {
    splits = ws ? (int)(ws_bytes / ((size_t)M * N * 4)) : 1;
    if (splits < 1) splits = 1;
  }
  TcEpilogue ep;
  ep.alpha = e.alpha; ep.beta = e.beta; ep.C = e.C; ep.ldc = e.ldc; ep.Cb = (__nv_bfloat16*)e.Cb; ep.ldcb = e.ldcb;
  ep.bias = e.bias; ep.act = e.act; ep.Cpre = e.Cpre; ep.ldpre = e.ldpre; ep.partial = splits > 1 ? ws : nullptr;
  ep.gate = e.gate; ep.ldgate = e.ldgate;
#define TC_DISPATCH(BNV)                                                                                   \
  if (BN == BNV) {                                                                                         \
    if (!a_mn && !b_mn) rc = launch_tc<BNV, false, false>(ta, tb, ep, M, N, K, splits, st);                \
    else if (a_mn && !b_mn) rc = launch_tc<BNV, true, false>(ta, tb, ep, M, N, K, splits, st);             \
    else if (!a_mn && b_mn) rc = launch_tc<(BNV < 64 ? 64 : BNV), false, true>(ta, tb, ep, M, N, K, splits, st); \
    else rc = launch_tc<(BNV < 64 ? 64 : BNV), true, true>(ta, tb, ep, M, N, K, splits, st);               \
  }
  rc = -1;
  TC_DISPATCH(32) TC_DISPATCH(64) TC_DISPATCH(128)
#undef TC_DISPATCH
  if (rc) return rc;
  if (splits > 1) {
    const int per = cdiv(total_kb, splits);
    const int used = cdiv(total_kb, per);
    ep.partial = nullptr;
    long long total = (long long)M * N;
    tc_splitk_reduce_kernel<<<(int)min((long long)1184, (total + 255) / 256), 256, 0, st>>>(M, N, used, ws, ep);
    TACORL_LAUNCH_CHECK();
  }
  return 0;
}

__global__ void cast_bf16_2d_kernel(const float* __restrict__ src, long long lds, long long rows, int cols,
                                    __nv_bfloat16* __restrict__ dst, long long ldd) {
  const long long total = rows * ldd;
  for (long long i = blockIdx.x * (long long)blockDim.x + threadIdx.x; i < total;
       i += (long long)gridDim.x * blockDim.x) {
    const long long r = i / ldd; const int c = (int)(i % ldd);
    dst[i] = __float2bfloat16(c < cols ? src[r * lds + c] : 0.f);
  }
}

int cast_bf16_2d(const float* src, long long lds, long long rows, int cols, void* dst, long long ldd, cudaStream_t st) {
  if (rows == 0) return 0;
  long long total = rows * ldd;
  cast_bf16_2d_kernel<<<(int)min((long long)148 * 8, (total + 255) / 256), 256, 0, st>>>(src, lds, rows, cols,
                                                                                        (__nv_bfloat16*)dst, ldd);
  TACORL_LAUNCH_CHECK();
  return 0;
}

__global__ void cast_transpose_bf16_kernel(const float* __restrict__ src, long long lds, int rows, int cols,
                                           __nv_bfloat16* __restrict__ dst, long long ldd) {
  __shared__ float tile[32][33];
  const int r0 = blockIdx.y * 32, c0 = blockIdx.x * 32;
  for (int i = threadIdx.y; i < 32; i += 8) {
    const int r = r0 + i, c = c0 + threadIdx.x;
    tile[i][threadIdx.x] = (r < rows && c < cols) ? src[(long long)r * lds + c] : 0.f;
  }
  __syncthreads();
  for (int i = threadIdx.y; i < 32; i += 8) {
    const int c = c0 + i, r = r0 + threadIdx.x;
    if (c < cols && r < rows) dst[(long long)c * ldd + r] = __float2bfloat16(tile[threadIdx.x][i]);
  }
}

int cast_transpose_bf16(const float* src, long long lds, int rows, int cols, void* dst, long long ldd, cudaStream_t st) {
  if (rows == 0 || cols == 0) return 0;
  cast_transpose_bf16_kernel<<<dim3(cdiv(cols, 32), cdiv(rows, 32)), dim3(32, 8), 0, st>>>(src, lds, rows, cols,
                                                                                          (__nv_bfloat16*)dst, ldd);
  TACORL_LAUNCH_CHECK();
  return 0;
}

int gemm_tc_from_f32(const GemmArgs& g, float* ws, size_t ws_bytes, cudaStream_t st) {
  if (g.M == 0 || g.N == 0) return 0;
  if ((long long)g.M * g.N * g.K < (1LL << 24)) return gemm_f32(g, ws, ws_bytes, st);
  TACORL_REQUIRE(ws, "gemm_tc: workspace required");
  const long long a_rows = g.transA ? g.K : g.M, a_cols = g.transA ? g.M : g.K;
  const long long b_rows = g.transB ? g.N : g.K, b_cols = g.transB ? g.K : g.N;
  const long long lda = (a_cols + 7) & ~7LL, ldb = (b_cols + 7) & ~7LL;
  const bool a_ready = g.A_bf16 && lda == a_cols && ((uintptr_t)g.A_bf16 & 15) == 0;
  const bool b_ready = g.B_bf16 && ldb == b_cols && ((uintptr_t)g.B_bf16 & 15) == 0;
  Arena ar(ws, ws_bytes);
  const __nv_bfloat16* Ab = a_ready ? (const __nv_bfloat16*)g.A_bf16 : ar.take<__nv_bfloat16>((size_t)a_rows * lda);
  const __nv_bfloat16* Bb = b_ready ? (const __nv_bfloat16*)g.B_bf16 : ar.take<__nv_bfloat16>((size_t)b_rows * ldb);
  TACORL_REQUIRE(Ab && Bb, "gemm_tc: workspace too small for bf16 staging (%lld + %lld elements)", a_rows * lda,
                 b_rows * ldb);
  int rc;
  if (!a_ready && (rc = cast_bf16_2d(g.A, g.lda, a_rows, (int)a_cols, (void*)Ab, lda, st))) return rc;
  if (!b_ready && (rc = cast_bf16_2d(g.B, g.ldb, b_rows, (int)b_cols, (void*)Bb, ldb, st))) return rc;
  TcArgs e;
  e.alpha = g.alpha; e.beta = g.beta; e.C = g.C; e.ldc = g.ldc; e.bias = g.bias; e.act = g.act; e.Cpre = g.Cpre;
  e.ldpre = g.ldpre; e.split_k = g.split_k;
  return gemm_tc_bf16(Ab, lda, g.transA ? 1 : 0, Bb, ldb, g.transB ? 0 : 1, g.M, g.N, g.K, e,
                      (float*)(ar.base + ar.off), ar.left(), st);
}

}
```

### tacorl_b200/csrc/internal.h

```cpp
#pragma once
#include "common.cuh"

namespace tacorl {

const char* last_error();
unsigned long long launch_count();

int colsum_tall_f32(long long M, int N, const float* X, float* out, int accumulate, float* ws,
                    size_t ws_bytes, cudaStream_t st);

int im2col_f32(const float* x, long long sn, long long sc, long long sh, long long sw, int C, int KH,
               int KW, int stride, int OH, int OW, int nframes, float* col, cudaStream_t st, int korder);
int colsum_tall_bf16(long long M, int N, const void* X, float* out, int accumulate, float* ws, size_t ws_bytes,
                     cudaStream_t st);
int col2im_f32(const float* dcol, int C, int H, int W, int KH, int KW, int stride, int OH, int OW,
               int nframes, const float* ymask, float* dx, cudaStream_t st);
int permute_conv_weight_f32(const float* src, float* dst, int OC, int C, int KH, int KW, int dir,
                            cudaStream_t st);
int softargmax_fwd_f32(const float* y, int N, int OH, int OW, int C, const float* temperature,
                       float* feat, float* smax, float* ssum, cudaStream_t st);
int softargmax_bwd_f32(const float* y, int N, int OH, int OW, int C, const float* temperature,
                       const float* feat, const float* smax, const float* ssum, const float* dfeat,
                       float* dy, float* dtau_part, cudaStream_t st);

int persistent_ctas();
void set_sm_reserve(int n);

struct TcArgs {
  float alpha = 1.f, beta = 0.f;
  float* C = nullptr; long long ldc = 0;
  void* Cb = nullptr; long long ldcb = 0;
  const float* bias = nullptr;
  int act = ACT_NONE;
  float* Cpre = nullptr; long long ldpre = 0;
  int split_k = 0;
  const float* gate = nullptr; long long ldgate = 0;
};
int gemm_tc_bf16(const void* A, long long lda, int a_mn, const void* B, long long ldb, int b_mn, int M, int N,
                 int K, const TcArgs& e, float* ws, size_t ws_bytes, cudaStream_t st);
int rnn_seq_tc(const void* Ab, int T, const void* W, long long ldw, int M, int N, int K, int tau0, int dtau, int n_steps,
               float beta, float* C, long long ldc, long long c_ts, const float* gate, long long ldgate, long long gate_ts,
               void* Cb, int act, unsigned* flags, cudaStream_t st);
struct WaveLaneHost {
  const void* Ab = nullptr; long long lda = 0, a_ts = 0;
  const void* W = nullptr; long long ldw = 0;
  int tau0 = 0, dtau = 1, n_steps = 0;
  float beta = 1.f;
  float* C = nullptr; long long ldc = 0, c_ts = 0;
  const float* gate = nullptr; long long ldgate = 0, gate_ts = 0;
  void* Cb = nullptr; long long ldcb = 0, cb_ts = 0;
  int act = ACT_NONE;
  unsigned* flags = nullptr;
};
int rnn_wave_tc(const WaveLaneHost* lanes, int n_lanes, int T, int M, int N, int K, cudaStream_t st);
unsigned rnn_seq_timeouts();
bool rnn_seq_enabled();
void rnn_seq_set_enabled(int on);
int rnn_seq_mode();
int cast_bf16_2d(const float* src, long long lds, long long rows, int cols, void* dst, long long ldd, cudaStream_t st);
int cast_transpose_bf16(const float* src, long long lds, int rows, int cols, void* dst, long long ldd, cudaStream_t st);
int gemm_tc_from_f32(const GemmArgs& g, float* ws, size_t ws_bytes, cudaStream_t st);
static inline int gemm_any(int prec, const GemmArgs& g, float* ws, size_t ws_bytes, cudaStream_t st) {
  return prec == PREC_BF16 ? gemm_tc_from_f32(g, ws, ws_bytes, st) : gemm_f32(g, ws, ws_bytes, st);
}

int conv_tc_pack(int mode, const float* W, void* Wp, cudaStream_t st);
bool conv_lin_conv1_wgrad_ok(int Wp);
int conv_lin_conv1_wgrad(const void* dy1p, const void* xs, int N, int Hp, int Wp, float beta, float* dW, float* db,
                         float* ws, size_t ws_bytes, cudaStream_t st);
bool conv_lin_conv3_wgrad_ok(int W2);
int conv_lin_conv3_wgrad(const void* dy3p, const void* y2b, int N, int H2, int W2, float beta, float* dW, float* db,
                         float* ws, size_t ws_bytes, cudaStream_t st);
int conv_tc_pack_multi(int n, const int* modes, const float* const* Ws, void* const* Wps, cudaStream_t st);
int conv_tc_s2d(const float* x, int N, int H, int W, int SH, int SW, void* xs, cudaStream_t st);
int conv_tc_s2d_u8(const unsigned char* x, int N, int H, int W, int SH, int SW, float scale, float shift, void* xs,
                   cudaStream_t st);
int u8_to_f32_normalized(long long n, const unsigned char* x, float scale, float shift, float* out, cudaStream_t st);
int conv_tc_conv1_fwd(const void* xs, int N, int H1, int W1, const void* wp, const float* bias, void* y1b, cudaStream_t st);
int conv_tc_conv2_fwd(const void* y1b, int N, int H1, int W1, int H2, int W2, const void* wp, const float* bias,
                      void* y2b, cudaStream_t st);
int conv_tc_conv3_fwd(const void* y2b, int N, int H2, int W2, int H3, int W3, const void* wp, const float* bias,
                      float* y3, cudaStream_t st);
int conv_lin_conv1_fwd(const void* xs, int N, int H1, int W1, const void* wp, const float* bias, void* y1b, cudaStream_t st);
int conv_lin_conv3_fwd(const void* y2b, int N, int H2, int W2, int H3, int W3, const void* wp, const float* bias,
                       float* y3, cudaStream_t st);
int conv_dgrad2_fused(const void* dy2b, int N, int H1, int W1, int H2, int W2, const void* wp5, const void* y1b, void* dy1b,
                      int out_pad, cudaStream_t st);
int conv_tc_conv3_dgrad(const void* dy3b, int N, int H2, int W2, int H3, int W3, const void* wp, const void* y2b,
                        void* dy2b, cudaStream_t st);
int conv_tc_conv2_dgrad(const void* dy2b, int N, int H1, int W1, int H2, int W2, const void* wp_classes,
                        const void* y1b, void* dy1b, cudaStream_t st);
int softargmax_bwd_bf16out(const float* y, int N, int OH, int OW, int C, const float* temperature, const float* feat,
                           const float* smax, const float* ssum, const float* dfeat, void* dy_bf16, float* dtau_part,
                           int pad_h, int pad_w, cudaStream_t st);
int conv_tc_wgrad(int layer, const void* dyb, const void* src, int N, int SH, int SW, int RA, int RB, float beta,
                  float* dW, float* db, float* ws, size_t ws_bytes, cudaStream_t st);

struct Arena {
  char* base; size_t cap; size_t off = 0;
  Arena(void* p, size_t n) : base((char*)p), cap(n) {}
  template <typename T> T* take(size_t count) {
    size_t bytes = (count * sizeof(T) + 255) & ~size_t(255);
    if (off + bytes > cap) return nullptr;
    T* r = (T*)(base + off);
    off += bytes;
    return r;
  }
  size_t left() const { return cap - off; }
};

}
```

### tacorl_b200/csrc/rnn.cu

```cuda
#include "common.cuh"
#include "internal.h"
#include "../../include/tacorl_b200.h"
#include <cuda_bf16.h>

namespace tacorl {

__global__ void vec_add_kernel(int n, const float* a, const float* b, float* o) {
  int i = blockIdx.x * blockDim.x + threadIdx.x;
  if (i < n) o[i] = a[i] + b[i];
}

__global__ void relu_rows_kernel(long long rows, int H, float* p, long long ld, __nv_bfloat16* pb, long long ldb) {
  const long long total = rows * H;
  for (long long i = blockIdx.x * (long long)blockDim.x + threadIdx.x; i < total;
       i += (long long)gridDim.x * blockDim.x) {
    float* q = p + (i / H) * ld + (i % H);
    const float v = fmaxf(*q, 0.f);
    *q = v;
    if (pb) pb[(i / H) * ldb + (i % H)] = __float2bfloat16(v);
  }
}

__global__ void mask_rows_kernel(long long rows, int H, float* d, long long ldd, const float* out,
                                 long long ldo, const float* add, long long lda, __nv_bfloat16* db, long long lddb) {
// ... 219 lines not shown
  const bool whht_ready = w_hh_t_bf16 && ((uintptr_t)w_hh_t_bf16 & 15) == 0;
  const bool hb_ready = h_bf16 && ((uintptr_t)h_bf16 & 15) == 0;
  Arena ar(ws, ws_bytes);
  const __nv_bfloat16* wih = wih_ready ? (const __nv_bfloat16*)w_ih_bf16 : ar.take<__nv_bfloat16>((size_t)H * Ip);
  __nv_bfloat16* whh = whht_ready ? (__nv_bfloat16*)w_hh_t_bf16 : ar.take<__nv_bfloat16>((size_t)H * H);
  __nv_bfloat16* xb = ar.take<__nv_bfloat16>((size_t)n_steps * B * Ip);
  __nv_bfloat16* hb = hb_ready ? (__nv_bfloat16*)h_bf16 : ar.take<__nv_bfloat16>((size_t)T * B * H);
  __nv_bfloat16* db = ar.take<__nv_bfloat16>((size_t)T * B * H);
  __nv_bfloat16* h0b = h0 ? ar.take<__nv_bfloat16>((size_t)B * H) : nullptr;
  unsigned* flags = ar.take<unsigned>(64);
  TACORL_REQUIRE(wih && whh && xb && hb && db && (!h0 || h0b) && flags, "rnn_layer_bwd(bf16): workspace too small");
  float* sk = (float*)(ar.base + ar.off);
  size_t sk_bytes = ar.left();
  const float beta0 = accumulate ? 1.f : 0.f;
  const int t_lo = reverse ? T - n_steps : 0;
  const long long rows = (long long)n_steps * B;
  int rc;
  if (!wih_ready && (rc = cast_bf16_2d(w_ih, I, H, I, (void*)wih, Ip, st))) return rc;
  if (!whht_ready && (rc = cast_transpose_bf16(w_hh, H, H, H, whh, H, st))) return rc;
  if ((rc = cast_bf16_2d(x + (long long)t_lo * B * ldx, ldx, rows, I, xb, Ip, st))) return rc;
  if (!hb_ready && (rc = cast_bf16_2d(out + (long long)t_lo * B * ldo, ldo, rows, H, hb + (long long)t_lo * B * H, H, st))) return rc;
  if (h0 && (rc = cast_bf16_2d(h0, H, B, H, h0b, H, st))) return rc;
  {
    const int t = reverse ? T - n_steps : n_steps - 1;
    mask_rows_kernel<<<ew_blocks((long long)B * H), 256, 0, st>>>(
        B, H, dout + (long long)t * B * lddo, lddo, out + (long long)t * B * ldo, ldo, dhn, H, db + (long long)t * B * H, H);
    TACORL_LAUNCH_CHECK();
  }
  for (int s = n_steps - 1; s >= 0; --s) {
    const int t = reverse ? T - 1 - s : s;
    __nv_bfloat16* dbt = db + (long long)t * B * H;
    if (s == n_steps - 1 && s > 0) {
      const int tp = reverse ? t + 1 : t - 1;
      rc = rnn_seq_tc(db, T, whh, H, B, H, H, tp, reverse ? 1 : -1, n_steps - 1, 1.f, dout, lddo, (long long)B * lddo, out, ldo,
                      (long long)B * ldo, db, ACT_NONE, flags, st);
      if (rc < 0) return rc;
      if (rc == 0) { s = 1; continue; }
    }
    if (s > 0) {
      const int tp = reverse ? t + 1 : t - 1;
      TcArgs c;
      c.C = dout + (long long)tp * B * lddo; c.ldc = lddo; c.beta = 1.f; c.split_k = 0;
      c.gate = out + (long long)tp * B * ldo; c.ldgate = ldo;
      c.Cb = db + (long long)tp * B * H; c.ldcb = H;
      if ((rc = gemm_tc_bf16(dbt, H, 0, whh, H, 0, B, H, H, c, sk, sk_bytes, st))) return rc;
    } else if (dh0) {
      TcArgs c;
      c.C = dh0; c.ldc = H; c.split_k = 1;
      if ((rc = gemm_tc_bf16(dbt, H, 0, whh, H, 0, B, H, H, c, sk, sk_bytes, st))) return rc;
    }
  }
  float* dpre = dout + (long long)t_lo * B * lddo;
  const __nv_bfloat16* dpb = db + (long long)t_lo * B * H;
  if (dw_hh) {
    bool wrote = false;
    if (n_steps > 1) {
      const __nv_bfloat16 *a, *b;
      if (!reverse) { a = dpb + (long long)B * H; b = hb; }
      else { a = dpb; b = hb + (long long)(t_lo + 1) * B * H; }
      TcArgs w;
      w.C = dw_hh; w.ldc = H; w.beta = beta0; w.split_k = 0;
      if ((rc = gemm_tc_bf16(a, H, 1, b, H, 1, H, H, (n_steps - 1) * B, w, sk, sk_bytes, st))) return rc;
      wrote = true;
    }
    if (h0) {
      const int t0 = reverse ? T - 1 : 0;
      TcArgs w;
      w.C = dw_hh; w.ldc = H; w.beta = wrote ? 1.f : beta0; w.split_k = 0;
      if ((rc = gemm_tc_bf16(db + (long long)t0 * B * H, H, 1, h0b, H, 1, H, H, B, w, sk, sk_bytes, st))) return rc;
      wrote = true;
    }
    if (!wrote && !accumulate) TACORL_CHECK_CUDA(cudaMemsetAsync(dw_hh, 0, (size_t)H * H * 4, st));
  }
  if (dw_ih) {
    TcArgs w;
    w.C = dw_ih; w.ldc = I; w.beta = beta0; w.split_k = 0;
    if ((rc = gemm_tc_bf16(dpb, H, 1, xb, Ip, 1, H, I, (int)rows, w, sk, sk_bytes, st))) return rc;
  }
  if (db_ih || db_hh) {
    float* first = db_ih ? db_ih : db_hh;
    if (!accumulate) {
      if ((rc = colsum2_f32((int)rows, H, dpre, lddo, first, 0, sk, sk_bytes, st))) return rc;
      if (db_ih && db_hh) TACORL_CHECK_CUDA(cudaMemcpyAsync(db_hh, db_ih, (size_t)H * 4, cudaMemcpyDeviceToDevice, st));
    } else {
      if (db_ih) if ((rc = colsum2_f32((int)rows, H, dpre, lddo, db_ih, 1, sk, sk_bytes, st))) return rc;
      if (db_hh) if ((rc = colsum2_f32((int)rows, H, dpre, lddo, db_hh, 1, sk, sk_bytes, st))) return rc;
    }
  }
  if (dx) {
    if (!dx_accumulate && n_steps < T) {
      const long long lo_rows = (long long)t_lo * B, hi_rows = (long long)(T - t_lo - n_steps) * B;
      if (lo_rows) TACORL_CHECK_CUDA(cudaMemset2DAsync(dx, lddx * 4, 0, (size_t)I * 4, lo_rows, st));
      if (hi_rows) TACORL_CHECK_CUDA(cudaMemset2DAsync(dx + (long long)(t_lo + n_steps) * B * lddx, lddx * 4, 0,
                                                       (size_t)I * 4, hi_rows, st));
    }
    TcArgs d;
    d.C = dx + (long long)t_lo * B * lddx; d.ldc = lddx; d.beta = dx_accumulate ? 1.f : 0.f; d.split_k = 1;
    if ((rc = gemm_tc_bf16(dpb, H, 0, wih, Ip, 1, (int)rows, I, H, d, sk, sk_bytes, st))) return rc;
  }
  return 0;
}


struct Layer2Ws {
  float* bsum[2] = {nullptr, nullptr};
  const __nv_bfloat16* wih[2] = {nullptr, nullptr};
  const __nv_bfloat16* whh[2] = {nullptr, nullptr};
  const __nv_bfloat16* xb = nullptr; long long ldxb = 0;
  unsigned* flags = nullptr;
  float* sk = nullptr; size_t sk_bytes = 0;
};

static int layer2_fwd_bf16(int T, int B, int I, int H, int D, const float* x, long long ldx, const void* x_bf16,
                           long long ldxb, const float* const* w, const void* const* w_bf16, const int* n_steps,
                           float* out, long long ldo, void* out_bf16, void* ws, size_t ws_bytes, cudaStream_t st) {
  TACORL_REQUIRE(x && w && n_steps && out && out_bf16 && ws, "rnn_layer2_fwd: null pointer");
  TACORL_REQUIRE(D == 1 || D == 2, "rnn_layer2_fwd: D must be 1 or 2");
  TACORL_REQUIRE(H % 8 == 0 && ldo % 8 == 0 && ((uintptr_t)out_bf16 & 15) == 0,
                 "rnn_layer2_fwd: hidden size / output pitch must be multiples of 8 and the bf16 twin 16-byte aligned");
  for (int d = 0; d < D; ++d)
    TACORL_REQUIRE(n_steps[d] >= 1 && n_steps[d] <= T, "rnn_layer2_fwd: n_steps[%d] = %d out of range (T=%d)", d, n_steps[d], T);
  if (B == 0) return 0;
  const long long Ip = (I + 7) & ~7LL;
  Arena ar(ws, ws_bytes);
  Layer2Ws L;
  int rc;
  for (int d = 0; d < D; ++d) {
    L.bsum[d] = ar.take<float>(H);
    const void* tih = w_bf16 ? w_bf16[2 * d] : nullptr;
    const void* thh = w_bf16 ? w_bf16[2 * d + 1] : nullptr;
    const bool ih_ready = tih && Ip == I && ((uintptr_t)tih & 15) == 0, hh_ready = thh && ((uintptr_t)thh & 15) == 0;
    __nv_bfloat16* cih = ih_ready ? nullptr : ar.take<__nv_bfloat16>((size_t)H * Ip);
    __nv_bfloat16* chh = hh_ready ? nullptr : ar.take<__nv_bfloat16>((size_t)H * H);
    TACORL_REQUIRE(L.bsum[d] && (ih_ready || cih) && (hh_ready || chh), "rnn_layer2_fwd: workspace too small");
    if (!ih_ready && (rc = cast_bf16_2d(w[4 * d], I, H, I, cih, Ip, st))) return rc;
    if (!hh_ready && (rc = cast_bf16_2d(w[4 * d + 1], H, H, H, chh, H, st))) return rc;
    L.wih[d] = ih_ready ? (const __nv_bfloat16*)tih : cih;
    L.whh[d] = hh_ready ? (const __nv_bfloat16*)thh : chh;
    vec_add_kernel<<<cdiv(H, 256), 256, 0, st>>>(H, w[4 * d + 2], w[4 * d + 3], L.bsum[d]);
    TACORL_LAUNCH_CHECK();
  }
  const bool x_ready = x_bf16 && ldxb % 8 == 0 && ldxb >= I && ((uintptr_t)x_bf16 & 15) == 0 && (I % 8 == 0);
  if (x_ready) { L.xb = (const __nv_bfloat16*)x_bf16; L.ldxb = ldxb; }
  else {
    __nv_bfloat16* xc = ar.take<__nv_bfloat16>((size_t)T * B * Ip);
    TACORL_REQUIRE(xc, "rnn_layer2_fwd: workspace too small");
    if ((rc = cast_bf16_2d(x, ldx, (long long)T * B, I, xc, Ip, st))) return rc;
    L.xb = xc; L.ldxb = Ip;
  }
  L.flags = ar.take<unsigned>(128);
  TACORL_REQUIRE(L.flags, "rnn_layer2_fwd: workspace too small");
  L.sk = (float*)(ar.base + ar.off); L.sk_bytes = ar.left();
  __nv_bfloat16* outb = (__nv_bfloat16*)out_bf16;
  WaveLaneHost lanes[2];
  int n_lanes = 0;
  for (int d = 0; d < D; ++d) {
    const int n = n_steps[d], t_lo = d ? T - n : 0, t0 = d ? T - 1 : 0;
    TcArgs in;
    in.C = out + (long long)t_lo * B * ldo + (long long)d * H; in.ldc = ldo; in.bias = L.bsum[d];
    in.split_k = n * B <= 128 ? 0 : 1;
    if ((rc = gemm_tc_bf16(L.xb + (long long)t_lo * B * L.ldxb, L.ldxb, 0, L.wih[d], Ip, 0, n * B, H, I, in, L.sk, L.sk_bytes, st)))
      return rc;
    relu_rows_kernel<<<ew_blocks((long long)B * H), 256, 0, st>>>(B, H, out + (long long)t0 * B * ldo + (long long)d * H, ldo,
                                                                 outb + (long long)t0 * B * ldo + (long long)d * H, ldo);
    TACORL_LAUNCH_CHECK();
    if (n > 1) {
      WaveLaneHost& h = lanes[n_lanes];
      h.Ab = outb + (long long)d * H; h.lda = ldo; h.a_ts = (long long)B * ldo;
      h.W = L.whh[d]; h.ldw = H;
      h.tau0 = d ? T - 2 : 1; h.dtau = d ? -1 : 1; h.n_steps = n - 1; h.beta = 1.f;
      h.C = out + (long long)d * H; h.ldc = ldo; h.c_ts = (long long)B * ldo;
      h.Cb = outb + (long long)d * H; h.ldcb = ldo; h.cb_ts = (long long)B * ldo;
      h.act = ACT_RELU; h.flags = L.flags + 64 * n_lanes;
      ++n_lanes;
    }
  }
  if (n_lanes == 0) return 0;
  rc = rnn_wave_tc(lanes, n_lanes, T, B, H, H, st);
  if (rc <= 0) return rc;
  for (int l = 0; l < n_lanes; ++l) {
    const WaveLaneHost& h = lanes[l];
    rc = 1;
    if (h.lda == H)
      rc = rnn_seq_tc(h.Ab, T, h.W, H, B, H, H, h.tau0, h.dtau, h.n_steps, 1.f, h.C, h.ldc, h.c_ts, nullptr, 0, 0, h.Cb,
                      ACT_RELU, h.flags, st);
    if (rc < 0) return rc;
    if (rc == 0) continue;
    for (int s = 0; s < h.n_steps; ++s) {
      const int tau = h.tau0 + s * h.dtau;
      TcArgs r;
      r.C = h.C + (long long)tau * h.c_ts; r.ldc = h.ldc; r.beta = 1.f; r.act = ACT_RELU;
      r.Cb = (__nv_bfloat16*)h.Cb + (long long)tau * h.cb_ts; r.ldcb = h.ldcb; r.split_k = 0;
      if ((rc = gemm_tc_bf16((const __nv_bfloat16*)h.Ab + (long long)(tau - h.dtau) * h.a_ts, h.lda, 0, h.W, H, 0, B, H, H, r,
                             L.sk, L.sk_bytes, st)))
        return rc;
    }
  }
  return 0;
}

static int layer2_bwd_bf16(int T, int B, int Bg, int I, int H, int D, const float* x, long long ldx, const void* x_bf16,
                           long long ldxb, const float* const* w, const void* const* w_bf16, const int* n_steps,
                           const float* out, long long ldo, const void* out_bf16, float* dout, long long lddo,
                           void* dpre_bf16, float* dx, long long lddx, float* const* dw, void* ws, size_t ws_bytes,
                           cudaStream_t st) {
  TACORL_REQUIRE(x && w && n_steps && out && out_bf16 && dout && dpre_bf16 && dw && ws, "rnn_layer2_bwd: null pointer");
  TACORL_REQUIRE(D == 1 || D == 2, "rnn_layer2_bwd: D must be 1 or 2");
  TACORL_REQUIRE(H % 8 == 0 && ldo % 8 == 0 && lddo % 8 == 0 && ((uintptr_t)out_bf16 & 15) == 0 && ((uintptr_t)dpre_bf16 & 15) == 0,
                 "rnn_layer2_bwd: pitches must be multiples of 8 and the bf16 twins 16-byte aligned");
  TACORL_REQUIRE(n_steps[0] == T, "rnn_layer2_bwd: the forward direction must cover every step");
  TACORL_REQUIRE(Bg >= 0 && Bg <= B, "rnn_layer2_bwd: grad_rows %d out of range (B=%d)", Bg, B);
  if (B == 0) return 0;
  if (Bg == 0) Bg = B;
  const long long Ip = (I + 7) & ~7LL;
  Arena ar(ws, ws_bytes);
  int rc;
  const __nv_bfloat16* wih[2] = {nullptr, nullptr};
  const __nv_bfloat16* whht[2] = {nullptr, nullptr};
  for (int d = 0; d < D; ++d) {
    TACORL_REQUIRE(n_steps[d] >= 1 && n_steps[d] <= T, "rnn_layer2_bwd: n_steps out of range");
    const void* tih = w_bf16 ? w_bf16[2 * d] : nullptr;
    const void* tht = w_bf16 ? w_bf16[2 * d + 1] : nullptr;
    const bool ih_ready = tih && Ip == I && ((uintptr_t)tih & 15) == 0, ht_ready = tht && ((uintptr_t)tht & 15) == 0;
    __nv_bfloat16* cih = ih_ready ? nullptr : ar.take<__nv_bfloat16>((size_t)H * Ip);
    __nv_bfloat16* cht = ht_ready ? nullptr : ar.take<__nv_bfloat16>((size_t)H * H);
    TACORL_REQUIRE((ih_ready || cih) && (ht_ready || cht), "rnn_layer2_bwd: workspace too small");
    if (!ih_ready && (rc = cast_bf16_2d(w[2 * d], I, H, I, cih, Ip, st))) return rc;
    if (!ht_ready && (rc = cast_transpose_bf16(w[2 * d + 1], H, H, H, cht, H, st))) return rc;
    wih[d] = ih_ready ? (const __nv_bfloat16*)tih : cih;
    whht[d] = ht_ready ? (const __nv_bfloat16*)tht : cht;
  }
  const bool x_ready = x_bf16 && ldxb % 8 == 0 && ldxb >= I && ((uintptr_t)x_bf16 & 15) == 0 && (I % 8 == 0);
  const __nv_bfloat16* xb; long long ldb_x;
  if (x_ready) { xb = (const __nv_bfloat16*)x_bf16; ldb_x = ldxb; }
  else {
    __nv_bfloat16* xc = ar.take<__nv_bfloat16>((size_t)T * B * Ip);
    TACORL_REQUIRE(xc, "rnn_layer2_bwd: workspace too small");
    if ((rc = cast_bf16_2d(x, ldx, (long long)T * B, I, xc, Ip, st))) return rc;
    xb = xc; ldb_x = Ip;
  }
  unsigned* flags = ar.take<unsigned>(128);
  TACORL_REQUIRE(flags, "rnn_layer2_bwd: workspace too small");
  float* sk = (float*)(ar.base + ar.off);
  const size_t sk_bytes = ar.left();
  const __nv_bfloat16* hb = (const __nv_bfloat16*)out_bf16;
  __nv_bfloat16* dpb = (__nv_bfloat16*)dpre_bf16;
  WaveLaneHost lanes[2];
  int n_lanes = 0;
  for (int d = 0; d < D; ++d) {
    const int n = n_steps[d];
    const int t_last = d ? T - n : n - 1;
    const long long col = (long long)d * H;
    mask_rows_kernel<<<ew_blocks((long long)Bg * H), 256, 0, st>>>(
        Bg, H, dout + (long long)t_last * B * lddo + col, lddo, out + (long long)t_last * B * ldo + col, ldo, nullptr, 0,
        dpb + (long long)t_last * B * lddo + col, lddo);
    TACORL_LAUNCH_CHECK();
    if (n > 1) {
      WaveLaneHost& h = lanes[n_lanes];
      h.Ab = dpb + col; h.lda = lddo; h.a_ts = (long long)B * lddo;
      h.W = whht[d]; h.ldw = H;
      h.tau0 = d ? T - n + 1 : n - 2; h.dtau = d ? 1 : -1; h.n_steps = n - 1; h.beta = 1.f;
      h.C = dout + col; h.ldc = lddo; h.c_ts = (long long)B * lddo;
      h.gate = out + col; h.ldgate = ldo; h.gate_ts = (long long)B * ldo;
      h.Cb = dpb + col; h.ldcb = lddo; h.cb_ts = (long long)B * lddo;
      h.act = ACT_NONE; h.flags = flags + 64 * n_lanes;
      ++n_lanes;
    }
  }
  if (n_lanes > 0) {
    rc = rnn_wave_tc(lanes, n_lanes, T, Bg, H, H, st);
    if (rc < 0) return rc;
    if (rc > 0) {
      for (int l = 0; l < n_lanes; ++l) {
        const WaveLaneHost& h = lanes[l];
        rc = 1;
        if (h.lda == H && h.ldgate == H && Bg == B)
          rc = rnn_seq_tc(h.Ab, T, h.W, H, B, H, H, h.tau0, h.dtau, h.n_steps, 1.f, h.C, h.ldc, h.c_ts, h.gate, h.ldgate,
                          h.gate_ts, h.Cb, ACT_NONE, h.flags, st);
        if (rc < 0) return rc;
        if (rc == 0) continue;
        for (int s = 0; s < h.n_steps; ++s) {
          const int tau = h.tau0 + s * h.dtau;
          TcArgs c;
          c.C = h.C + (long long)tau * h.c_ts; c.ldc = h.ldc; c.beta = 1.f; c.split_k = 0;
          c.gate = h.gate + (long long)tau * h.gate_ts; c.ldgate = h.ldgate;
          c.Cb = (__nv_bfloat16*)h.Cb + (long long)tau * h.cb_ts; c.ldcb = h.ldcb;
          if ((rc = gemm_tc_bf16((const __nv_bfloat16*)h.Ab + (long long)(tau - h.dtau) * h.a_ts, h.lda, 0, h.W, H, 0, Bg, H, H, c,
                                 sk, sk_bytes, st)))
            return rc;
        }
      }
    }
  }
  for (int d = 0; d < D; ++d) {
    const int n = n_steps[d], t_lo = d ? T - n : 0;
    const long long col = (long long)d * H, rows = (long long)n * B;
    float* dpre = dout + (long long)t_lo * B * lddo + col;
    const __nv_bfloat16* dp = dpb + (long long)t_lo * B * lddo + col;
    float *dw_ih = dw[4 * d], *dw_hh = dw[4 * d + 1], *db_ih = dw[4 * d + 2], *db_hh = dw[4 * d + 3];
    if (dw_hh) {
      if (n > 1) {
        const __nv_bfloat16 *a, *b;
        if (d == 0) { a = dp + (long long)B * lddo; b = hb + col; }
        else { a = dp; b = hb + (long long)(t_lo + 1) * B * ldo + col; }
        TcArgs g;
        g.C = dw_hh; g.ldc = H; g.split_k = 0;
        if ((rc = gemm_tc_bf16(a, lddo, 1, b, ldo, 1, H, H, (n - 1) * B, g, sk, sk_bytes, st))) return rc;
      } else {
        TACORL_CHECK_CUDA(cudaMemsetAsync(dw_hh, 0, (size_t)H * H * 4, st));
      }
    }
    if (dw_ih) {
      TcArgs g;
      g.C = dw_ih; g.ldc = I; g.split_k = 0;
      if ((rc = gemm_tc_bf16(dp, lddo, 1, xb + (long long)t_lo * B * ldb_x, ldb_x, 1, H, I, (int)rows, g, sk, sk_bytes, st))) return rc;
    }
    if (db_ih || db_hh) {
      float* first = db_ih ? db_ih : db_hh;
      if ((rc = colsum2_f32((int)rows, H, dpre, lddo, first, 0, sk, sk_bytes, st))) return rc;
      if (db_ih && db_hh) TACORL_CHECK_CUDA(cudaMemcpyAsync(db_hh, db_ih, (size_t)H * 4, cudaMemcpyDeviceToDevice, st));
    }
    if (dx) {
      TcArgs g;
      g.C = dx + (long long)t_lo * B * lddx; g.ldc = lddx; g.beta = d ? 1.f : 0.f; g.split_k = 1;
      if ((rc = gemm_tc_bf16(dp, lddo, 0, wih[d], Ip, 1, (int)rows, I, H, g, sk, sk_bytes, st))) return rc;
    }
  }
  return 0;
}

int tacorl_rnn_layer_fwd(int T, int B, int I, int H, const float* x, long long ldx, const float* w_ih,
                         const float* w_hh, const float* b_ih, const float* b_hh, const float* h0,
                         int reverse, int n_steps, float* out, long long ldo, const void* w_ih_bf16,
                         const void* w_hh_bf16, void* h_bf16_out, void* ws, size_t ws_bytes, int prec, void* stream) {
  TACORL_REQUIRE(prec == PREC_F32 || prec == PREC_BF16, "rnn_layer_fwd: unknown precision %d", prec);
  auto fn = prec == PREC_BF16 ? rnn_fwd_bf16 : rnn_fwd_f32;
  return fn(T, B, I, H, x, ldx, w_ih, w_hh, b_ih, b_hh, h0, reverse, n_steps, out, ldo, w_ih_bf16, w_hh_bf16, h_bf16_out,
            ws, ws_bytes, (cudaStream_t)stream);
}

int tacorl_rnn_layer_bwd(int T, int B, int I, int H, const float* x, long long ldx, const float* w_ih,
                         const float* w_hh, const float* h0, int reverse, int n_steps, const float* out,
                         long long ldo, float* dout, long long lddo, const float* dhn, float* dx,
                         long long lddx, int dx_accumulate, float* dw_ih, float* dw_hh, float* db_ih,
                         float* db_hh, int accumulate, float* dh0, const void* w_ih_bf16, const void* w_hh_t_bf16,
                         const void* h_bf16, void* ws, size_t ws_bytes, int prec, void* stream) {
  TACORL_REQUIRE(prec == PREC_F32 || prec == PREC_BF16, "rnn_layer_bwd: unknown precision %d", prec);
  auto fn = prec == PREC_BF16 ? rnn_bwd_bf16 : rnn_bwd_f32;
  return fn(T, B, I, H, x, ldx, w_ih, w_hh, h0, reverse, n_steps, out, ldo, dout, lddo, dhn, dx, lddx,
            dx_accumulate, dw_ih, dw_hh, db_ih, db_hh, accumulate, dh0, w_ih_bf16, w_hh_t_bf16, h_bf16, ws, ws_bytes,
            (cudaStream_t)stream);
}

size_t tacorl_rnn_layer2_ws_bytes(int T, int B, int I, int H, int D) {
  return (size_t)D * tacorl_rnn_layer_ws_bytes(T, B, I, H) + 8192;
}

int tacorl_rnn_layer2_fwd(int T, int B, int I, int H, int D, const float* x, long long ldx, const void* x_bf16,
                          long long ldxb, const float* const* w, const void* const* w_bf16, const int* n_steps,
                          float* out, long long ldo, void* out_bf16, void* ws, size_t ws_bytes, void* stream) {
  return layer2_fwd_bf16(T, B, I, H, D, x, ldx, x_bf16, ldxb, w, w_bf16, n_steps, out, ldo, out_bf16, ws, ws_bytes,
                         (cudaStream_t)stream);
}

int tacorl_rnn_layer2_bwd(int T, int B, int grad_rows, int I, int H, int D, const float* x, long long ldx, const void* x_bf16,
                          long long ldxb, const float* const* w, const void* const* w_bf16, const int* n_steps,
                          const float* out, long long ldo, const void* out_bf16, float* dout, long long lddo,
                          void* dpre_bf16, float* dx, long long lddx, float* const* dw, void* ws, size_t ws_bytes,
                          void* stream) {
  return layer2_bwd_bf16(T, B, grad_rows, I, H, D, x, ldx, x_bf16, ldxb, w, w_bf16, n_steps, out, ldo, out_bf16, dout, lddo, dpre_bf16,
                         dx, lddx, dw, ws, ws_bytes, (cudaStream_t)stream);
}

int tacorl_cast_transpose_bf16(const float* src, int rows, int cols, void* dst, void* stream) {
  TACORL_REQUIRE(src && dst, "cast_transpose_bf16: null pointer");
  return cast_transpose_bf16(src, cols, rows, cols, dst, rows, (cudaStream_t)stream);
}

}
```

### tacorl_b200/ops.py

```python
import ctypes
import math
import weakref

import torch
from torch.autograd import Function

from . import _lib as L

_STATE = {"prec": L.PREC_F32}
_GEMM_WS = 96 << 20


def set_precision(name):
    _STATE["prec"] = {"fp32": L.PREC_F32, "bf16": L.PREC_BF16}[name]


def get_precision():
    return "bf16" if _STATE["prec"] == L.PREC_BF16 else "fp32"


_SIDE = {}


def _side_stream(dev):
    key = dev.index if dev.index is not None else torch.cuda.current_device()
    if key not in _SIDE:
        _SIDE[key] = torch.cuda.Stream(device=dev)
    return _SIDE[key]


def _prep_stream(dev):
    key = ("prep", dev.index if dev.index is not None else torch.cuda.current_device())
    if key not in _SIDE:
        _SIDE[key] = torch.cuda.Stream(device=dev)
    return _SIDE[key]


def _off(t, elems):
    return ctypes.c_void_p(t.data_ptr() + 4 * elems)


def _c(t):
    return t if t.is_contiguous() else t.contiguous()


def _ld(t):
    assert t.dim() == 2 and (t.stride(1) == 1 or t.shape[1] == 1), "row-major 2-D view expected"
    return t.stride(0) if t.shape[0] > 1 else max(t.shape[1], t.stride(0))


_SHADOW_OWNERS = weakref.WeakSet()


def register_shadow_owner(owner):
    _SHADOW_OWNERS.add(owner)


def refresh_shadows():
    for o in list(_SHADOW_OWNERS):
        for p in o.param_groups[0]["params"]:
            shadow_of(p)
    for key, (ref, ver, sh) in list(_FROZEN_SHADOWS.items()):
        t = ref()
        if t is None or t.data_ptr() != key or t.requires_grad:
            del _FROZEN_SHADOWS[key]
        elif t._version != ver:
            with torch.no_grad():
                sh.copy_(t.detach().reshape(-1))
            _FROZEN_SHADOWS[key] = (ref, t._version, sh)


_FROZEN_SHADOWS = {}
_FROZEN_PARAMS = {}


def mark_frozen(module):
    for p in module.parameters():
        _FROZEN_PARAMS[id(p)] = weakref.ref(p)


def invalidate_frozen_shadows():
    _FROZEN_SHADOWS.clear()


def _frozen_shadow_of(t):
    ref = _FROZEN_PARAMS.get(id(t))
    if ref is None or ref() is not t or t.requires_grad or t.dtype != torch.float32:
        return None
    key = t.data_ptr()
    hit = _FROZEN_SHADOWS.get(key)
    if hit is not None:
        ref, ver, sh = hit
        if ref() is t and sh.numel() == t.numel():
            if ver != t._version:
                with torch.no_grad():
                    sh.copy_(t.detach().reshape(-1))
                _FROZEN_SHADOWS[key] = (ref, t._version, sh)
            return sh
    if torch.cuda.is_current_stream_capturing():
        return None
    with torch.no_grad():
        sh = t.detach().reshape(-1).to(torch.bfloat16)
    _FROZEN_SHADOWS[key] = (weakref.ref(t), t._version, sh)
    return sh


def shadow_of(t):
    if _STATE["prec"] != L.PREC_BF16 or t is None or not t.is_cuda or not t.is_contiguous():
        return None
    ptr = t.data_ptr()
    for o in list(_SHADOW_OWNERS):
        flat = o.pbuf.flat
        base = flat.data_ptr()
        if base <= ptr < base + flat.numel() * 4 and flat.device == t.device:
            n = o._pnumel.get(ptr)
            if n != t.numel():
                return None
            if o._flat_version != flat._version:
                o._pver.clear()
                o._flat_version = flat._version
            off = (ptr - base) // 4
            sh = o.shadow[off:off + n]
            if o._pver.get(ptr) != t._version:
                with torch.no_grad():
                    sh.copy_(t.detach().reshape(-1))
                o._pver[ptr] = t._version
            return sh
    return _frozen_shadow_of(t)


_GRAD_OWNERS = weakref.WeakSet()


def register_grad_owner(owner):
    _GRAD_OWNERS.add(owner)


def grad_slot_of(t):
    if t is None or not t.is_cuda or not t.is_contiguous():
        return None
    ptr = t.data_ptr()
    for o in list(_GRAD_OWNERS):
        flat = o.pbuf.flat
        base = flat.data_ptr()
        if base <= ptr < base + flat.numel() * 4 and flat.device == t.device:
            if o._pnumel.get(ptr) != t.numel() or ptr in o._slots_taken:
                return None
            owner_param = o._pparam.get(ptr)
            if owner_param is None or owner_param.grad is not None:
                return None
            o._slots_taken.add(ptr)
            off = (ptr - base) // 4
            return o.flat_grad[off:off + t.numel()].view(t.shape)
    return None


def gemm(A, B, C, transA=False, transB=False, alpha=1.0, beta=0.0, bias=None, act=L.ACT_NONE, Cpre=None, A_bf16=None,
         B_bf16=None):
    M, N = C.shape
    K = A.shape[0] if transA else A.shape[1]
    assert (A.shape[1] if transA else A.shape[0]) == M, (A.shape, C.shape, transA)
    assert (B.shape[0] if transB else B.shape[1]) == N and (B.shape[1] if transB else B.shape[0]) == K
    ws = L.workspace(_GEMM_WS, C.device)
    L.call("tacorl_gemm_ex", int(transA), int(transB), M, N, K, float(alpha), L.ptr(A), _ld(A), L.ptr(B), _ld(B),
           float(beta), L.ptr(C), _ld(C), L.ptr(bias), int(act), L.ptr(Cpre), _ld(Cpre) if Cpre is not None else 0,
           L.ptr_any(A_bf16), L.ptr_any(B_bf16), ctypes.c_void_p(ws.data_ptr()), ws.numel(),
           _STATE["prec"], L.stream())
    return C


def colsum(X, out=None, accumulate=False):
    M, N = X.shape
    if out is None:
        out = torch.empty(N, device=X.device, dtype=torch.float32)
    L.call("tacorl_colsum", M, N, L.ptr(X), _ld(X), L.ptr(out), int(accumulate), L.stream())
    return out


def scale(x, dev_scalar=None, c=1.0, out=None):
    x = _c(x)
    if out is None:
        out = torch.empty_like(x)
    L.call("tacorl_scale", x.numel(), L.ptr(x), L.ptr(dev_scalar), float(c), L.ptr(out), L.stream())
    return out


class LinearFn(Function):
    @staticmethod
    def forward(ctx, x, W, b, act):
        K = W.shape[1]
        x2 = _c(x.reshape(-1, K))
        Wc = _c(W)
        out = torch.empty(x2.shape[0], W.shape[0], device=x.device, dtype=torch.float32)
        pre = torch.empty_like(out) if act == L.ACT_SILU else None
        gemm(x2, Wc, out, transB=True, bias=b, act=act, Cpre=pre, B_bf16=shadow_of(Wc))
        ctx.act = act
        ctx.has_bias = b is not None
        ctx.xshape = x.shape
        ctx.save_for_backward(x2, Wc, pre if act == L.ACT_SILU else (out if act == L.ACT_RELU else None))
        return out.view(*x.shape[:-1], W.shape[0])

    @staticmethod
    def backward(ctx, dy):
        x2, W, saved = ctx.saved_tensors
        N = W.shape[0]
        dz = _c(dy.reshape(-1, N))
        if ctx.act != L.ACT_NONE:
            dz2 = torch.empty_like(dz)
            L.call("tacorl_act_bwd", ctx.act, dz.numel(), L.ptr(dz), L.ptr(saved), L.ptr(dz2), L.stream())
            dz = dz2
        dx = dW = db = None
        if ctx.needs_input_grad[0]:
            dx = torch.empty_like(x2)
            gemm(dz, W, dx, B_bf16=shadow_of(W))
            dx = dx.view(ctx.xshape)
        if ctx.needs_input_grad[1]:
            dW = torch.empty_like(W)
            gemm(dz, x2, dW, transA=True)
        if ctx.has_bias and ctx.needs_input_grad[2]:
            db = colsum(dz)
        return dx, dW, db, None


def linear(x, W, b=None, act=None):
    return LinearFn.apply(x, W, b, L.ACTS[act] if not isinstance(act, int) else act)


def _dp(t):
    return None if t is None else t.data_ptr()


class MlpChainFn(Function):

    @staticmethod
    def _layers(spec, params, in0, grads=None):
        acts, segs = spec
        arr = (L.MlpLayer * len(segs))()
        i, width = 0, in0
        for l, ns in enumerate(segs):
            e = arr[l]
            for sg in range(ns):
                W, b = params[i + 2 * sg], params[i + 2 * sg + 1]
                setattr(e, f"W{sg}", _dp(W)); setattr(e, f"b{sg}", _dp(b)); setattr(e, f"n{sg}", W.shape[0])
                if grads is not None:
                    setattr(e, f"dW{sg}", _dp(grads[i + 2 * sg])); setattr(e, f"db{sg}", _dp(grads[i + 2 * sg + 1]))
            e.in_ = width
            e.act = acts[l] if l < len(acts) else L.ACT_NONE
            width = e.n0 + e.n1 + e.n2
            i += 2 * ns
        return arr, width

    @staticmethod
    def forward(ctx, spec, x0, x1, *params):
        lead = x0.shape[:-1]
        x0 = _c(x0.reshape(-1, x0.shape[-1]))
        x1 = _c(x1.reshape(-1, x1.shape[-1])) if x1 is not None else None
        params = [None if p is None else _c(p) for p in params]
        rows = x0.shape[0]
        in0 = x0.shape[1] + (x1.shape[1] if x1 is not None else 0)
        arr, out_w = MlpChainFn._layers(spec, params, in0)
        nl = len(spec[1])
        zw = sum(arr[l].n0 + arr[l].n1 + arr[l].n2 for l in range(nl - 1))
        z = torch.empty(rows, max(zw, 1), device=x0.device, dtype=torch.float32)
        out = torch.empty(rows, out_w, device=x0.device, dtype=torch.float32)
        L.call("tacorl_mlp_chain_fwd", nl, rows, ctypes.byref(arr), L.ptr(x0), x0.shape[1], x0.shape[1],
               L.ptr(x1), x1.shape[1] if x1 is not None else 0, x1.shape[1] if x1 is not None else 0,
               L.ptr(z), z.shape[1], L.ptr(out), out_w, L.stream())
        ctx.spec, ctx.lead, ctx.has_x1 = spec, lead, x1 is not None
        ctx.save_for_backward(x0, x1, z, *params)
        return out.view(*lead, out_w)

    @staticmethod
    def backward(ctx, d_out):
        x0, x1, z, *params = ctx.saved_tensors
        rows = x0.shape[0]
        d_out = _c(d_out.reshape(rows, -1))
        need = ctx.needs_input_grad
        want_w = any(need[3:])
        grads = [torch.empty_like(p) if (want_w and p is not None) else None for p in params]
        in0 = x0.shape[1] + (x1.shape[1] if x1 is not None else 0)
        arr, _ = MlpChainFn._layers(ctx.spec, params, in0, grads)
        dx0 = torch.empty_like(x0) if need[1] else None
        dx1 = torch.empty_like(x1) if (x1 is not None and need[2]) else None
        nl = len(ctx.spec[1])
        nbytes = L.query("tacorl_mlp_chain_ws_bytes", nl, rows, ctypes.byref(arr))
        ws = L.workspace(nbytes, x0.device, "mlp_chain")
        L.call("tacorl_mlp_chain_bwd", nl, rows, ctypes.byref(arr), L.ptr(x0), x0.shape[1], x0.shape[1],
               L.ptr(x1), x1.shape[1] if x1 is not None else 0, x1.shape[1] if x1 is not None else 0,
               L.ptr(z), z.shape[1], L.ptr(d_out), d_out.shape[1], L.ptr(dx0), x0.shape[1],
               L.ptr(dx1), x1.shape[1] if x1 is not None else 0, ctypes.c_void_p(ws.data_ptr()), ws.numel(), L.stream())
        gx0 = dx0.view(*ctx.lead, x0.shape[1]) if dx0 is not None else None
        gx1 = dx1.view(*ctx.lead, x1.shape[1]) if dx1 is not None else None
        return (None, gx0, gx1, *[g if need[3 + i] else None for i, g in enumerate(grads)])


def mlp_chain(xs, layers, acts):
    xs = list(xs) if isinstance(xs, (list, tuple)) else [xs]
    segs = [[l] if torch.is_tensor(l[0]) else list(l) for l in layers]
    acts_i = tuple(L.ACTS[a] if not isinstance(a, int) else a for a in acts)
    in0 = sum(x.shape[-1] for x in xs)
    widths = [in0] + [sum(W.shape[0] for W, _ in sg) for sg in segs]
    ok = (len(segs) <= 4 and len(xs) <= 2 and all(len(sg) <= 3 for sg in segs) and xs[0].is_cuda
          and all(w % 4 == 0 and w <= 256 for w in widths[:-1]) and widths[-1] <= 256
          and all(x.dtype == torch.float32 for x in xs) and xs[0].numel() // xs[0].shape[-1] <= 256)
    if not ok:
        x = xs[0] if len(xs) == 1 else torch.cat(xs, dim=-1)
        for l, sg in enumerate(segs):
            W = sg[0][0] if len(sg) == 1 else torch.cat([w for w, _ in sg], dim=0)
            b = sg[0][1] if len(sg) == 1 else torch.cat([bb for _, bb in sg], dim=0)
            x = linear(x, W, b, acts_i[l] if l < len(acts_i) else None)
        return x
    flat = []
    for sg in segs:
        for W, b in sg:
            flat += [W, b]
    spec = (acts_i, tuple(len(sg) for sg in segs))
    return MlpChainFn.apply(spec, xs[0], xs[1] if len(xs) == 2 else None, *flat)


class LMPEncoderFn(Function):

    @staticmethod
    def forward(ctx, x, save, norm, *params):
        N, C, H, W = x.shape
        assert C == 3, "LMPVisionEncoder kernels are built for 3 input channels"
        if (not x.is_contiguous() and x.dtype == torch.uint8 and x.stride(-1) == 1 and W % 4 == 0
                and all(st % 4 == 0 for st in x.stride()[:-1]) and x.storage_offset() % 4 == 0):
            xc = torch.empty(x.shape, device=x.device, dtype=torch.uint8)
            xc.view(torch.int32).copy_(x.view(torch.int32))
            x = xc
        x = _c(x)
        if x.dtype == torch.uint8:
            mean, std = norm
            ctx.xnorm = (1, 1.0 / (255.0 * std), -mean / std)
        else:
            assert x.dtype == torch.float32, f"images must be float32 or uint8, got {x.dtype}"
            ctx.xnorm = (0, 1.0, 0.0)
        params = [_c(p) for p in params]
        hidden, latent = params[7].shape[0], params[9].shape[0]
        dev = x.device
        H1, W1 = (H - 8) // 4 + 1, (W - 8) // 4 + 1
        H2, W2 = (H1 - 4) // 2 + 1, (W1 - 4) // 2 + 1
        H3, W3 = H2 - 2, W2 - 2
        emb = torch.empty(N, latent, device=dev, dtype=torch.float32)
        if save:
            adt = torch.bfloat16 if _STATE["prec"] == L.PREC_BF16 else torch.float32
            y1 = torch.empty(N, H1, W1, 32, device=dev, dtype=adt)
            y2 = torch.empty(N, H2, W2, 64, device=dev, dtype=adt)
            y3 = torch.empty(N, H3, W3, 64, device=dev)
            feat = torch.empty(N, 128, device=dev)
            smax = torch.empty(N, 64, device=dev)
            ssum = torch.empty(N, 64, device=dev)
            h4 = torch.empty(N, hidden, device=dev)
            xs = (torch.empty(N, H1 + 1, W1 + 1, 64, device=dev, dtype=torch.bfloat16)
                  if _STATE["prec"] == L.PREC_BF16 else None)
        else:
            y1 = y2 = y3 = feat = smax = ssum = h4 = xs = None
        nbytes = L.query("tacorl_lmp_encoder_ws_bytes", N, H, W, hidden, latent, 0)
        ws = L.workspace(nbytes, dev)
        ctx.prec = _STATE["prec"]
        L.call("tacorl_lmp_encoder_fwd", L.ptr_any(x), *ctx.xnorm, N, H, W, L.ptr_array(params), hidden, latent, L.ptr_any(y1),
               L.ptr_any(y2), L.ptr(y3), L.ptr(feat), L.ptr(smax), L.ptr(ssum), L.ptr(h4), L.ptr(emb), L.ptr_any(xs),
               ctypes.c_void_p(ws.data_ptr()), ws.numel(), _STATE["prec"], L.stream())
        if save:
            ctx.has_xs = xs is not None
            ctx.save_for_backward(x, y1, y2, y3, feat, smax, ssum, h4, *((xs,) if xs is not None else ()), *params)
        ctx.dims = (N, H, W, hidden, latent)
        return emb

    @staticmethod
    def backward(ctx, d_emb):
# ... 35 lines not shown
            main, prep = torch.cuda.current_stream(dev), _prep_stream(dev)
            whts = [torch.empty(H, H, device=dev, dtype=torch.bfloat16) for _ in range(num_layers * D)]
            prep.wait_stream(main)
            with torch.cuda.stream(prep):
                for k in range(num_layers * D):
                    L.call("tacorl_cast_transpose_bf16", L.ptr(weights[k * 4 + 1]), H, H, L.ptr_any(whts[k]), L.stream())
                prep_done = torch.cuda.Event()
                prep_done.record(prep)
        for l in range(num_layers):
            Il = inp.shape[2]
            out = torch.empty(T, B, D * H, device=dev, dtype=torch.float32)
            nbytes = L.query("tacorl_rnn_layer_ws_bytes", T, B, Il, H)

            def run_dir(d, tag):
                w_ih, w_hh, b_ih, b_hh = weights[(l * D + d) * 4:(l * D + d) * 4 + 4]
                n_steps = 1 if (last_only and l == num_layers - 1 and d == 1) else T
                h0_ld = None if h0 is None else _c(h0[l * D + d])
                ws = L.workspace(nbytes, dev, tag)
                L.call("tacorl_rnn_layer_fwd", T, B, Il, H, L.ptr(inp), Il, L.ptr(w_ih), L.ptr(w_hh), L.ptr(b_ih),
                       L.ptr(b_hh), L.ptr(h0_ld), d, n_steps, _off(out, d * H), D * H,
                       L.ptr_any(shadow_of(w_ih)), L.ptr_any(shadow_of(w_hh)), L.ptr_any(hbs[l * D + d]),
                       ctypes.c_void_p(ws.data_ptr()), ws.numel(), _STATE["prec"], L.stream())

            if D == 2:
                main, side = torch.cuda.current_stream(dev), _side_stream(dev)
                side.wait_stream(main)
                was = L.lib().tacorl_rnn_seq_enable(0)
                try:
                    with torch.cuda.stream(side):
                        run_dir(1, "rnn_side")
                    run_dir(0, "main")
                finally:
                    L.lib().tacorl_rnn_seq_enable(was)
                main.wait_stream(side)
            else:
                run_dir(0, "main")
            if hn is not None:
                for d in range(D):
                    hn.append(out[0 if d == 1 else T - 1, :, d * H:(d + 1) * H])
            outs.append(out)
            inp = out
        ctx.cfg = (T, B, I, H, D, num_layers, last_only)
        ctx.has_h0 = h0 is not None
        ctx.bf16_aux = (hbs, whts, prep_done) if train else None
        ctx.save_for_backward(x, h0, *outs, *weights)
        if last_only:
            return inp[T - 1], None
        return inp, torch.stack(hn, dim=0)

    @staticmethod
    def backward(ctx, d_out, d_hn):
        T, B, I, H, D, num_layers, last_only = ctx.cfg
        saved = ctx.saved_tensors
        x, h0 = saved[0], saved[1]
        outs = saved[2:2 + num_layers]
        weights = saved[2 + num_layers:]
        dev = x.device
        if last_only:
            dbuf = torch.zeros(T, B, D * H, device=dev, dtype=torch.float32)
            dbuf[T - 1].copy_(d_out)
        else:
            dbuf = d_out.contiguous().clone() if d_out is not None else torch.zeros(T, B, D * H, device=dev)
        wgrads = [None] * len(weights)
        dh0 = torch.empty_like(h0) if (ctx.has_h0 and ctx.needs_input_grad[1]) else None
        aux = ctx.bf16_aux if _STATE["prec"] == L.PREC_BF16 else None
        hbs, whts = (aux[0], aux[1]) if aux is not None else ([None] * (num_layers * D),) * 2
        if aux is not None:
            torch.cuda.current_stream(dev).wait_event(aux[2])
        for l in range(num_layers - 1, -1, -1):
            inp = x if l == 0 else outs[l - 1]
            Il = inp.shape[2]
            need_dx = l > 0 or ctx.needs_input_grad[0]
            dx = torch.empty(T, B, Il, device=dev, dtype=torch.float32) if need_dx else None
            dx_rev = torch.empty(T, B, Il, device=dev, dtype=torch.float32) if (need_dx and D == 2) else None
            nbytes = L.query("tacorl_rnn_layer_ws_bytes", T, B, Il, H)

            def run_dir(d, tag, dx_buf):
                k = (l * D + d) * 4
                w_ih, w_hh = weights[k], weights[k + 1]
                g = []
                for j in range(4):
                    slot = grad_slot_of(weights[k + j])
                    g.append(slot if slot is not None else torch.empty_like(weights[k + j]))
                n_steps = 1 if (last_only and l == num_layers - 1 and d == 1) else T
                h0_ld = None if h0 is None else _c(h0[l * D + d])
                dhn_ld = None if d_hn is None else _c(d_hn[l * D + d])
                dh0_ld = None if dh0 is None else dh0[l * D + d]
                ws = L.workspace(nbytes, dev, tag)
                L.call("tacorl_rnn_layer_bwd", T, B, Il, H, L.ptr(inp), Il, L.ptr(w_ih), L.ptr(w_hh), L.ptr(h0_ld),
                       d, n_steps, _off(outs[l], d * H), D * H, _off(dbuf, d * H), D * H, L.ptr(dhn_ld),
                       L.ptr(dx_buf), Il, 0, L.ptr(g[0]), L.ptr(g[1]), L.ptr(g[2]), L.ptr(g[3]), 0,
                       L.ptr(dh0_ld), L.ptr_any(shadow_of(w_ih)), L.ptr_any(whts[l * D + d]), L.ptr_any(hbs[l * D + d]),
                       ctypes.c_void_p(ws.data_ptr()), ws.numel(), _STATE["prec"], L.stream())
                wgrads[k:k + 4] = g

            if D == 2:
                main, side = torch.cuda.current_stream(dev), _side_stream(dev)
                side.wait_stream(main)
                was = L.lib().tacorl_rnn_seq_enable(0)
                try:
                    with torch.cuda.stream(side):
                        run_dir(1, "rnn_side", dx_rev)
                    run_dir(0, "main", dx)
                finally:
                    L.lib().tacorl_rnn_seq_enable(was)
                main.wait_stream(side)
                if need_dx:
                    dx.add_(dx_rev)
            else:
                run_dir(0, "main", dx)
            dbuf = dx
        return (dbuf if ctx.needs_input_grad[0] else None, dh0, None, None, None, *wgrads)


class ReluRNN2Fn(Function):

    @staticmethod
    def forward(ctx, x, num_layers, bidir, last_only, grad_rows, *weights):
        T, B, I = x.shape
        D = 2 if bidir else 1
        H = weights[1].shape[0]
        x = _c(x)
        weights = [_c(w) for w in weights]
        dev = x.device
        train = any(ctx.needs_input_grad)
        whts, prep_done = [None] * (num_layers * D), None
        if train:
            main, prep = torch.cuda.current_stream(dev), _prep_stream(dev)
            whts = [torch.empty(H, H, device=dev, dtype=torch.bfloat16) for _ in range(num_layers * D)]
            prep.wait_stream(main)
            with torch.cuda.stream(prep):
                for k in range(num_layers * D):
                    L.call("tacorl_cast_transpose_bf16", L.ptr(weights[k * 4 + 1]), H, H, L.ptr_any(whts[k]), L.stream())
                prep_done = torch.cuda.Event()
                prep_done.record(prep)
        outs, outbs = [], []
        inp, inp_b = x, None
        for l in range(num_layers):
            Il = inp.shape[2]
            out = torch.empty(T, B, D * H, device=dev, dtype=torch.float32)
            outb = torch.empty(T, B, D * H, device=dev, dtype=torch.bfloat16)
            wl = weights[l * D * 4:(l + 1) * D * 4]
            tw = []
            for d in range(D):
                tw += [shadow_of(wl[4 * d]), shadow_of(wl[4 * d + 1])]
            nst = [T] + ([1 if (last_only and l == num_layers - 1) else T] if D == 2 else [])
            ws = L.workspace(L.query("tacorl_rnn_layer2_ws_bytes", T, B, Il, H, D), dev, "main")
            L.call("tacorl_rnn_layer2_fwd", T, B, Il, H, D, L.ptr(inp), Il, L.ptr_any(inp_b), Il, L.ptr_array(wl),
                   L.ptr_array(tw), L.int_array(nst), L.ptr(out), D * H, L.ptr_any(outb),
                   ctypes.c_void_p(ws.data_ptr()), ws.numel(), L.stream())
            outs.append(out)
            outbs.append(outb)
            inp, inp_b = out, outb
        ctx.cfg = (T, B, I, H, D, num_layers, last_only, B if grad_rows is None else int(grad_rows))
        ctx.aux = (outbs, whts, prep_done)
        ctx.save_for_backward(x, *outs, *weights)
        if last_only:
            return inp[T - 1], None
        hn = torch.stack([outs[l][0 if d == 1 else T - 1, :, d * H:(d + 1) * H] for l in range(num_layers) for d in range(D)], 0)
        ctx.mark_non_differentiable(hn)
        return inp, hn

    @staticmethod
    def backward(ctx, d_out, _d_hn):
        T, B, I, H, D, num_layers, last_only, Bg = ctx.cfg
        saved = ctx.saved_tensors
        x = saved[0]
        outs = saved[1:1 + num_layers]
        weights = saved[1 + num_layers:]
        outbs, whts, prep_done = ctx.aux
        dev = x.device
        if last_only:
            dbuf = torch.zeros(T, B, D * H, device=dev, dtype=torch.float32)
            dbuf[T - 1].copy_(d_out)
        else:
            dbuf = d_out.contiguous().clone()
        if prep_done is not None:
            torch.cuda.current_stream(dev).wait_event(prep_done)
        wgrads = [None] * len(weights)
        for l in range(num_layers - 1, -1, -1):
            inp, inp_b = (x, None) if l == 0 else (outs[l - 1], outbs[l - 1])
            Il = inp.shape[2]
            need_dx = l > 0 or ctx.needs_input_grad[0]
            dx = torch.empty(T, B, Il, device=dev, dtype=torch.float32) if need_dx else None
            mk = torch.zeros if Bg < B else torch.empty
            dpb = mk(T, B, D * H, device=dev, dtype=torch.bfloat16)
            wl = weights[l * D * 4:(l + 1) * D * 4]
            w2, tw, g = [], [], []
            for d in range(D):
                w2 += [wl[4 * d], wl[4 * d + 1]]
                tw += [shadow_of(wl[4 * d]), whts[l * D + d]]
                for j in range(4):
                    slot = grad_slot_of(wl[4 * d + j])
                    g.append(slot if slot is not None else torch.empty_like(wl[4 * d + j]))
            nst = [T] + ([1 if (last_only and l == num_layers - 1) else T] if D == 2 else [])
            ws = L.workspace(L.query("tacorl_rnn_layer2_ws_bytes", T, B, Il, H, D), dev, "main")
            L.call("tacorl_rnn_layer2_bwd", T, B, Bg, Il, H, D, L.ptr(inp), Il, L.ptr_any(inp_b), Il, L.ptr_array(w2),
                   L.ptr_array(tw), L.int_array(nst), L.ptr(outs[l]), D * H, L.ptr_any(outbs[l]), L.ptr(dbuf), D * H,
                   L.ptr_any(dpb), L.ptr(dx), Il, L.ptr_array(g), ctypes.c_void_p(ws.data_ptr()), ws.numel(), L.stream())
            wgrads[l * D * 4:(l + 1) * D * 4] = g
            dbuf = dx
        return (dbuf if ctx.needs_input_grad[0] else None, None, None, None, None, *wgrads)


def relu_rnn(x_tm, weights, num_layers, bidirectional, last_only=False, h0=None, grad_rows=None):
    if not torch.is_grad_enabled():
        x_tm, weights = x_tm.detach(), [w.detach() for w in weights]
    if h0 is None and _STATE["prec"] == L.PREC_BF16 and x_tm.is_cuda and weights[1].shape[0] % 8 == 0:
        return ReluRNN2Fn.apply(x_tm, num_layers, bidirectional, last_only, grad_rows, *weights)
    return ReluRNNFn.apply(x_tm, h0, num_layers, bidirectional, last_only, *weights)


class DlmLossFn(Function):

    @staticmethod
    def forward(ctx, logits, actions, num_classes, act_min, act_max, gripper_alpha):
        logits, actions = _c(logits), _c(actions)
        rows, A = logits.shape[0], actions.shape[1] - 1
        assert logits.shape[1] == 3 * A * 10 + 2
        dev = logits.device
        row_loss = torch.empty(rows * (A + 1), device=dev)
        loss = torch.empty(1, device=dev)
        need = ctx.needs_input_grad[0]
        dlog = torch.empty_like(logits) if need else None
        L.call("tacorl_dlm_nll", rows, A, L.ptr(logits), logits.shape[1], L.ptr(actions), actions.shape[1],
               int(num_classes), float(act_min), float(act_max), float(gripper_alpha), L.ptr(row_loss), L.ptr(loss),
               L.ptr(dlog), logits.shape[1], L.stream())
        if need:
            ctx.save_for_backward(dlog)
        return loss.view(())

    @staticmethod
    def backward(ctx, g):
        (dlog,) = ctx.saved_tensors
        return scale(dlog, _c(g.reshape(1))), None, None, None, None, None


def dlm_loss(logits, actions, num_classes=10, act_min=-1.0, act_max=1.0, gripper_alpha=1.0):
    return DlmLossFn.apply(logits, actions, num_classes, act_min, act_max, gripper_alpha)


def dlm_sample(logits, u1, u2, actions=None, grip_lo=-1.0, grip_hi=1.0):
    logits = _c(logits.detach())
    rows = logits.shape[0]
    A = (logits.shape[1] - 2) // 30
    dev = logits.device
    pred = torch.empty(rows, A + 1, device=dev)
    hit = torch.empty(rows, device=dev) if actions is not None else None
    acc = torch.empty(1, device=dev) if actions is not None else None
    actions_c = _c(actions) if actions is not None else None
    u1, u2 = _c(u1), _c(u2)
    L.call("tacorl_dlm_sample", rows, A, L.ptr(logits), logits.shape[1], L.ptr(u1), L.ptr(u2),
           L.ptr(actions_c), actions_c.shape[1] if actions is not None else 0, float(grip_lo), float(grip_hi),
           L.ptr(pred), L.ptr(hit), L.ptr(acc), L.stream())
    return pred, (acc.view(()) if acc is not None else None)


class GaussHeadFn(Function):

    @staticmethod
    def forward(ctx, raw):
        raw = _c(raw)
        rows, L2 = raw.shape
        mean = torch.empty(rows, L2 // 2, device=raw.device)
        std = torch.empty_like(mean)
        L.call("tacorl_gauss_head_fwd", rows, L2 // 2, L.ptr(raw), L.ptr(mean), L.ptr(std), L.stream())
        ctx.save_for_backward(raw, std)
        return mean, std

    @staticmethod
    def backward(ctx, dmean, dstd):
        raw, std = ctx.saved_tensors
        draw = torch.empty_like(raw)
        dmean = _c(dmean) if dmean is not None else None
        dstd = _c(dstd) if dstd is not None else None
        L.call("tacorl_gauss_head_bwd", raw.shape[0], raw.shape[1] // 2, L.ptr(raw), L.ptr(std),
               L.ptr(dmean), L.ptr(dstd), L.ptr(draw), L.stream())
        return draw


class SoftplusHeadFn(Function):

    @staticmethod
    def forward(ctx, raw, min_std):
        raw = _c(raw)
        rows, L2 = raw.shape
        mean = torch.empty(rows, L2 // 2, device=raw.device)
        std = torch.empty_like(mean)
        L.call("tacorl_softplus_head_fwd", rows, L2 // 2, L.ptr(raw), float(min_std), L.ptr(mean), L.ptr(std),
               L.stream())
        ctx.save_for_backward(raw)
        return mean, std

    @staticmethod
    def backward(ctx, dmean, dstd):
        (raw,) = ctx.saved_tensors
        draw = torch.empty_like(raw)
        dmean = _c(dmean) if dmean is not None else None
        dstd = _c(dstd) if dstd is not None else None
        L.call("tacorl_softplus_head_bwd", raw.shape[0], raw.shape[1] // 2, L.ptr(raw), L.ptr(dmean), L.ptr(dstd),
               L.ptr(draw), L.stream())
        return draw, None


def gauss_head(raw):
    return GaussHeadFn.apply(raw)
# ... 359 lines not shown
```

Baseline: 328,900.

## Group independent tcgen05 GEMMs into one persistent launch and reuse bf16 RNN outputs

Replaces the per-shape templated tensor-core GEMM kernel with a single kernel that takes a group of up to eight problems as a grid-constant descriptor and walks a combined tile space. The RNN layer uses it to batch both directions' input projections and the weight-gradient and dx GEMMs into one launch, and it supports skipping k-blocks for padded rows. It also registers the RNN's bf16 output as a twin so the following Linear layer can skip a cast. This cuts launch count and tail underutilisation, at the cost of runtime-variable BN and stage counts, which removes compile-time specialisation and adds per-tile lookup overhead.

```diff
diff --git a/include/tacorl_b200.h b/include/tacorl_b200.h
--- a/include/tacorl_b200.h
+++ b/include/tacorl_b200.h
@@ -29,6 +29,16 @@
                    const float* B, long long ldb, float beta, float* C, long long ldc, const float* bias, int act,
                    float* Cpre, long long ldpre, const void* A_bf16, const void* B_bf16, void* ws, size_t ws_bytes,
                    int prec, void* stream);
+typedef struct {
+  const void* A; long long lda; int a_mn;
+  const void* B; long long ldb; int b_mn;
+  int M, N, K;
+  float alpha, beta;
+  float* C; long long ldc;
+  int split_k;
+  int step_rows, grad_rows;
+} tacorl_gemm_bf16_desc;
+int tacorl_gemm_bf16_group(int n, const tacorl_gemm_bf16_desc* d, int grouped, void* ws, size_t ws_bytes, void* stream);
 int tacorl_colsum(int M, int N, const float* X, long long ldx, float* out, int accumulate, void* stream);
 int tacorl_act_bwd(int act, long long n, const float* dY, const float* y_or_pre, float* dZ, void* stream);
 int tacorl_scale(long long n, const float* x, const float* dev_scalar, float c, float* out, void* stream);
diff --git a/tacorl_b200/_lib.py b/tacorl_b200/_lib.py
--- a/tacorl_b200/_lib.py
+++ b/tacorl_b200/_lib.py
@@ -18,6 +18,7 @@
     "tacorl_gemm": [_i, _i, _i, _i, _i, _f, _vp, _ll, _vp, _ll, _f, _vp, _ll, _vp, _i, _vp, _ll, _vp, _sz, _i, _vp],
     "tacorl_gemm_ex": [_i, _i, _i, _i, _i, _f, _vp, _ll, _vp, _ll, _f, _vp, _ll, _vp, _i, _vp, _ll, _vp, _vp, _vp, _sz, _i,
                        _vp],
+    "tacorl_gemm_bf16_group": [_i, _vp, _i, _vp, _sz, _vp],
     "tacorl_colsum": [_i, _i, _vp, _ll, _vp, _i, _vp],
     "tacorl_act_bwd": [_i, _ll, _vp, _vp, _vp, _vp],
     "tacorl_scale": [_ll, _vp, _vp, _f, _vp, _vp],
@@ -106,6 +107,12 @@
     pass
 
 
+class GemmBf16Desc(ctypes.Structure):
+    _fields_ = [("A", _vp), ("lda", _ll), ("a_mn", _i), ("B", _vp), ("ldb", _ll), ("b_mn", _i),
+                ("M", _i), ("N", _i), ("K", _i), ("alpha", _f), ("beta", _f), ("C", _vp), ("ldc", _ll),
+                ("split_k", _i), ("step_rows", _i), ("grad_rows", _i)]
+
+
 class MlpLayer(ctypes.Structure):
     _fields_ = [("W0", _vp), ("b0", _vp), ("n0", _i), ("W1", _vp), ("b1", _vp), ("n1", _i),
                 ("W2", _vp), ("b2", _vp), ("n2", _i), ("in_", _i), ("act", _i),
diff --git a/tacorl_b200/csrc/api.cu b/tacorl_b200/csrc/api.cu
--- a/tacorl_b200/csrc/api.cu
+++ b/tacorl_b200/csrc/api.cu
@@ -1,6 +1,7 @@
 #include "common.cuh"
 #include "internal.h"
 #include "../../include/tacorl_b200.h"
+#include <vector>
 
 using namespace tacorl;
 
@@ -47,6 +48,25 @@
                         nullptr, ws, ws_bytes, prec, stream);
 }
 
+int tacorl_gemm_bf16_group(int n, const tacorl_gemm_bf16_desc* d, int grouped, void* ws, size_t ws_bytes, void* stream) {
+  TACORL_REQUIRE(n >= 0 && (n == 0 || d), "gemm_bf16_group: null descriptor array");
+  std::vector<TcGemm> g(n);
+  for (int i = 0; i < n; ++i) {
+    TACORL_REQUIRE(d[i].A && d[i].B && d[i].C, "gemm_bf16_group: null pointer in member %d", i);
+    TcGemm& m = g[i];
+    m.A = d[i].A; m.lda = d[i].lda; m.a_mn = d[i].a_mn ? 1 : 0;
+    m.B = d[i].B; m.ldb = d[i].ldb; m.b_mn = d[i].b_mn ? 1 : 0;
+    m.M = d[i].M; m.N = d[i].N; m.K = d[i].K;
+    m.e.alpha = d[i].alpha; m.e.beta = d[i].beta; m.e.C = d[i].C; m.e.ldc = d[i].ldc; m.e.split_k = d[i].split_k;
+    m.step_rows = d[i].step_rows; m.grad_rows = d[i].grad_rows;
+  }
+  if (grouped) return gemm_tc_group(g.data(), n, (float*)ws, ws_bytes, (cudaStream_t)stream);
+  int rc;
+  for (int i = 0; i < n; ++i)
+    if ((rc = gemm_tc_group(&g[i], 1, (float*)ws, ws_bytes, (cudaStream_t)stream))) return rc;
+  return 0;
+}
+
 int tacorl_colsum(int M, int N, const float* X, long long ldx, float* out, int accumulate, void* stream) {
   TACORL_REQUIRE(X && out, "colsum: null pointer");
   return colsum_f32(M, N, X, ldx, out, accumulate, (cudaStream_t)stream);
diff --git a/tacorl_b200/csrc/gemm_tc.cu b/tacorl_b200/csrc/gemm_tc.cu
--- a/tacorl_b200/csrc/gemm_tc.cu
+++ b/tacorl_b200/csrc/gemm_tc.cu
@@ -180,34 +180,64 @@
   }
 }
 
-template <int BN, bool A_MN, bool B_MN, int kStages>
-__global__ void __launch_bounds__(TC_THREADS, 1)
-gemm_tc_kernel(const __grid_constant__ CUtensorMap tmA, const __grid_constant__ CUtensorMap tmB, TcEpilogue ep,
-               int M, int N, int K, int kblocks_per_split) {
+constexpr int TC_MAX_GROUP = 8;
+constexpr int TC_MAX_STAGES = 8;
+struct TcProblem {
+  CUtensorMap tmA, tmB;
+  TcEpilogue ep;
+  int M, N, K, bn, a_mn, b_mn;
+  int kb_per_split, tiles_n, tiles_mn;
+  int tile_begin;
+  int kb_step, kb_live;
+};
+template <int NP>
+struct TcGroup {
+  TcProblem p[NP];
+  int n, total_tiles, stages, stage_bytes;
+};
+static_assert(sizeof(TcGroup<TC_MAX_GROUP>) <= 4096, "a grouped launch's descriptors are passed as one kernel parameter");
+
+__device__ __forceinline__ int tc_live_blocks(const TcProblem& P, int kb) {
+  return P.kb_step ? (kb / P.kb_step) * P.kb_live + min(kb % P.kb_step, P.kb_live) : kb;
+}
+
+struct TcTile { int p, m0, n0, z, kb0, kb1, nkb; };
+template <int NP>
+__device__ __forceinline__ TcTile tc_tile(const TcGroup<NP>& g, int tile) {
+  TcTile t;
+  int p = 0;
+  while (p + 1 < g.n && tile >= g.p[p + 1].tile_begin) ++p;
+  const TcProblem& P = g.p[p];
+  const int local = tile - P.tile_begin, rem = local % P.tiles_mn;
+  t.p = p;
+  t.z = local / P.tiles_mn;
+  t.m0 = (rem / P.tiles_n) * TC_BM;
+  t.n0 = (rem % P.tiles_n) * P.bn;
+  const int total_kb = (P.K + TC_BK - 1) / TC_BK;
+  t.kb0 = t.z * P.kb_per_split;
+  t.kb1 = min(total_kb, t.kb0 + P.kb_per_split);
+  t.nkb = tc_live_blocks(P, t.kb1) - tc_live_blocks(P, t.kb0);
+  return t;
+}
+
+template <int NP>
+__global__ void __launch_bounds__(TC_THREADS, 1) gemm_tc_kernel(const __grid_constant__ TcGroup<NP> g) {
   constexpr uint32_t A_BYTES = TC_BM * TC_BK * 2;
-  constexpr uint32_t B_BYTES = BN * TC_BK * 2;
-  constexpr uint32_t STAGE_BYTES = A_BYTES + B_BYTES;
-  constexpr uint32_t ACC_COLS = BN < 32 ? 32 : BN;
+  constexpr uint32_t ACC_COLS = 128;
   constexpr uint32_t TMEM_COLS = 2 * ACC_COLS;
-  static_assert(!B_MN || BN % 64 == 0, "MN-major B needs 64-wide boxes");
   extern __shared__ __align__(1024) uint8_t smem_raw[];
   uint8_t* smem = (uint8_t*)(((uintptr_t)smem_raw + 1023) & ~(uintptr_t)1023);
+  const int kStages = g.stages;
+  const uint32_t STAGE_BYTES = g.stage_bytes;
   uint64_t* bars = (uint64_t*)(smem + kStages * STAGE_BYTES);
-  uint32_t* tmem_slot = (uint32_t*)(bars + 2 * kStages + 4);
+  uint32_t* tmem_slot = (uint32_t*)(bars + 2 * TC_MAX_STAGES + 4);
 
   const int warp = threadIdx.x >> 5, lane = threadIdx.x & 31;
-  const int total_kb = (K + TC_BK - 1) / TC_BK;
-  const int kb_begin = blockIdx.z * kblocks_per_split;
-  const int kb_end = min(total_kb, kb_begin + kblocks_per_split);
-  const int nkb = kb_end - kb_begin;
-  const int tiles_n = (N + BN - 1) / BN;
-  const int num_tiles = ((M + TC_BM - 1) / TC_BM) * tiles_n;
-
   const uint32_t smem_base = smem_u32(smem);
   auto full_bar = [&](int s) { return smem_u32(bars + s); };
-  auto empty_bar = [&](int s) { return smem_u32(bars + kStages + s); };
-  auto tfull_bar = [&](int a) { return smem_u32(bars + 2 * kStages + a); };
-  auto tempty_bar = [&](int a) { return smem_u32(bars + 2 * kStages + 2 + a); };
+  auto empty_bar = [&](int s) { return smem_u32(bars + TC_MAX_STAGES + s); };
+  auto tfull_bar = [&](int a) { return smem_u32(bars + 2 * TC_MAX_STAGES + a); };
+  auto tempty_bar = [&](int a) { return smem_u32(bars + 2 * TC_MAX_STAGES + 2 + a); };
 
   if (threadIdx.x == 0) {
     for (int s = 0; s < kStages; ++s) { mbar_init(full_bar(s), 1); mbar_init(empty_bar(s), 1); }
@@ -225,54 +255,68 @@
   const uint32_t tmem_base = *tmem_slot;
 
   if (warp == 0) {
-    if (lane == 0 && nkb > 0) {
+    if (lane == 0) {
       uint32_t it = 0;
-      for (int tile = blockIdx.x; tile < num_tiles; tile += gridDim.x) {
-        const int m0 = (tile / tiles_n) * TC_BM, n0 = (tile % tiles_n) * BN;
-        for (int i = 0; i < nkb; ++i, ++it) {
+      for (int tile = blockIdx.x; tile < g.total_tiles; tile += gridDim.x) {
+        const TcTile t = tc_tile(g, tile);
+        const TcProblem& P = g.p[t.p];
+        const CUtensorMap *tmA = &P.tmA, *tmB = &P.tmB;
+        const int a_mn = P.a_mn, b_mn = P.b_mn, bn = P.bn, kb_step = P.kb_step, kb_live = P.kb_live;
+        const uint32_t bytes = A_BYTES + (uint32_t)bn * TC_BK * 2;
+        for (int kb = t.kb0; kb < t.kb1; ++kb) {
+          if (kb_step && kb % kb_step >= kb_live) continue;
           const int s = it % kStages;
           const uint32_t ph = (it / kStages) & 1;
+          ++it;
           mbar_wait(empty_bar(s), ph ^ 1);
-          mbar_expect_tx(full_bar(s), STAGE_BYTES);
-          const int k0 = (kb_begin + i) * TC_BK;
+          mbar_expect_tx(full_bar(s), bytes);
+          const int k0 = kb * TC_BK;
           const uint32_t a_dst = smem_base + s * STAGE_BYTES, b_dst = a_dst + A_BYTES;
-          if (!A_MN) {
-            tma_load_2d(a_dst, &tmA, k0, m0, full_bar(s));
+          if (!a_mn) {
+            tma_load_2d(a_dst, tmA, k0, t.m0, full_bar(s));
           } else {
-            tma_load_2d(a_dst, &tmA, m0, k0, full_bar(s));
-            tma_load_2d(a_dst + 8192, &tmA, m0 + 64, k0, full_bar(s));
+            tma_load_2d(a_dst, tmA, t.m0, k0, full_bar(s));
+            tma_load_2d(a_dst + 8192, tmA, t.m0 + 64, k0, full_bar(s));
           }
-          if (!B_MN) {
-            tma_load_2d(b_dst, &tmB, k0, n0, full_bar(s));
+          if (!b_mn) {
+            tma_load_2d(b_dst, tmB, k0, t.n0, full_bar(s));
           } else {
-#pragma unroll
-            for (int j = 0; j < BN / 64; ++j) tma_load_2d(b_dst + j * 8192, &tmB, n0 + j * 64, k0, full_bar(s));
+            for (int j = 0; j < bn / 64; ++j) tma_load_2d(b_dst + j * 8192, tmB, t.n0 + j * 64, k0, full_bar(s));
           }
         }
       }
     }
   } else if (warp == 1) {
-    if (lane == 0 && nkb > 0) {
-      const uint32_t idesc = (1u << 4) | (1u << 7) | (1u << 10) | ((A_MN ? 1u : 0u) << 15) | ((B_MN ? 1u : 0u) << 16) |
-                             ((uint32_t)(BN >> 3) << 17) | ((uint32_t)(TC_BM >> 4) << 24);
+    if (lane == 0) {
       uint32_t it = 0, lt = 0;
-      for (int tile = blockIdx.x; tile < num_tiles; tile += gridDim.x, ++lt) {
+      for (int tile = blockIdx.x; tile < g.total_tiles; tile += gridDim.x) {
+        const TcTile t = tc_tile(g, tile);
+        if (t.nkb == 0) continue;
+        const TcProblem& P = g.p[t.p];
+        const int a_mn = P.a_mn, b_mn = P.b_mn, kb_step = P.kb_step, kb_live = P.kb_live;
+        const uint32_t idesc = (1u << 4) | (1u << 7) | (1u << 10) | ((uint32_t)a_mn << 15) | ((uint32_t)b_mn << 16) |
+                               ((uint32_t)(P.bn >> 3) << 17) | ((uint32_t)(TC_BM >> 4) << 24);
+        const uint64_t ad0 = a_mn ? make_smem_desc(smem_base, 8192, 1024) : make_smem_desc(smem_base, 16, 1024);
+        const uint64_t bd0 = b_mn ? make_smem_desc(smem_base + A_BYTES, 8192, 1024) : make_smem_desc(smem_base + A_BYTES, 16, 1024);
+        const uint32_t a_k = a_mn ? 2048 >> 4 : 32 >> 4, b_k = b_mn ? 2048 >> 4 : 32 >> 4;
         const uint32_t acc = lt & 1;
         mbar_wait(tempty_bar(acc), ((lt >> 1) & 1) ^ 1);
+        ++lt;
         tc_fence_after();
         const uint32_t tmem_d = tmem_base + acc * ACC_COLS;
-        for (int i = 0; i < nkb; ++i, ++it) {
+        bool first = true;
+        for (int kb = t.kb0; kb < t.kb1; ++kb) {
+          if (kb_step && kb % kb_step >= kb_live) continue;
           const int s = it % kStages;
           const uint32_t ph = (it / kStages) & 1;
+          ++it;
           mbar_wait(full_bar(s), ph);
           tc_fence_after();
-          const uint32_t a_src = smem_base + s * STAGE_BYTES, b_src = a_src + A_BYTES;
-#pragma unroll
-          for (int k = 0; k < TC_BK / TC_UMMA_K; ++k) {
-            const uint64_t ad = A_MN ? make_smem_desc(a_src + k * 2048, 8192, 1024) : make_smem_desc(a_src + k * 32, 16, 1024);
-            const uint64_t bd = B_MN ? make_smem_desc(b_src + k * 2048, 8192, 1024) : make_smem_desc(b_src + k * 32, 16, 1024);
-            tc_mma_bf16(tmem_d, ad, bd, idesc, (i > 0 || k > 0) ? 1u : 0u);
-          }
+          const uint32_t so = (s * STAGE_BYTES) >> 4;
+#pragma unroll
+          for (int k = 0; k < TC_BK / TC_UMMA_K; ++k)
+            tc_mma_bf16(tmem_d, ad0 + so + k * a_k, bd0 + so + k * b_k, idesc, (!first || k > 0) ? 1u : 0u);
+          first = false;
           tc_commit(empty_bar(s));
         }
         tc_commit(tfull_bar(acc));
@@ -281,29 +325,38 @@
   } else {
     const int q = warp & 3;
     uint32_t lt = 0;
-    for (int tile = blockIdx.x; tile < num_tiles; tile += gridDim.x, ++lt) {
-      const int m0 = (tile / tiles_n) * TC_BM, n0 = (tile % tiles_n) * BN;
-      const int row = m0 + q * 32 + lane;
+    for (int tile = blockIdx.x; tile < g.total_tiles; tile += gridDim.x) {
+      const TcTile t = tc_tile(g, tile);
+      const TcProblem& P = g.p[t.p];
+      const TcEpilogue ep = P.ep;
+      const int M = P.M, N = P.N, bn = P.bn;
+      const int row = t.m0 + q * 32 + lane;
       const uint32_t acc = lt & 1;
-      if (nkb > 0) {
+      if (t.nkb > 0) {
         mbar_wait(tfull_bar(acc), (lt >> 1) & 1);
         tc_fence_after();
       }
 #pragma unroll 1
-      for (int c0 = 0; c0 < BN; c0 += 16) {
-        uint32_t r[16];
-        if (nkb > 0) {
-          tc_ld16(tmem_base + acc * ACC_COLS + ((uint32_t)(q * 32) << 16) + c0, r);
+      for (int c0 = 0; c0 < bn; c0 += 32) {
+        uint32_t r[2][16];
+        if (t.nkb > 0) {
+          const uint32_t ta = tmem_base + acc * ACC_COLS + ((uint32_t)(q * 32) << 16) + c0;
+          tc_ld16_nowait(ta, r[0]);
+          tc_ld16_nowait(ta + 16, r[1]);
+          tc_ld_wait();
         } else {
 #pragma unroll
-          for (int j = 0; j < 16; ++j) r[j] = 0;
+          for (int j = 0; j < 16; ++j) r[0][j] = r[1][j] = 0;
         }
-        if (row < M && n0 + c0 < N) tc_epilogue_chunk(ep, r, row, n0 + c0, N, blockIdx.z, M);
-      }
-      if (nkb > 0) {
+#pragma unroll
+        for (int h = 0; h < 2; ++h)
+          if (row < M && t.n0 + c0 + 16 * h < N) tc_epilogue_chunk(ep, r[h], row, t.n0 + c0 + 16 * h, N, t.z, M);
+      }
+      if (t.nkb > 0) {
         tc_fence_before();
         __syncwarp();
         if (lane == 0) mbar_arrive(tempty_bar(acc));
+        ++lt;
       }
     }
   }
@@ -1062,28 +1115,6 @@
   return 0;
 }
 
-template <int BN, bool A_MN, bool B_MN>
-static int launch_tc(const CUtensorMap& ta, const CUtensorMap& tb, const TcEpilogue& ep, int M, int N, int K,
-                     int splits, cudaStream_t st) {
-  constexpr int kStages = BN >= 128 ? 5 : 6;
-  constexpr size_t smem = (size_t)kStages * (TC_BM * TC_BK * 2 + BN * TC_BK * 2) + (2 * kStages + 4) * 8 + 16 + 1024;
-  static bool configured = false;
-  auto kern = gemm_tc_kernel<BN, A_MN, B_MN, kStages>;
-  if (!configured) {
-    TACORL_CHECK_CUDA(cudaFuncSetAttribute(kern, cudaFuncAttributeMaxDynamicSharedMemorySize, (int)smem));
-    configured = true;
-  }
-  const int total_kb = cdiv(K, TC_BK);
-  const int per = cdiv(total_kb, splits);
-  const int zs = cdiv(total_kb, per);
-  const long long tiles = (long long)cdiv(N, BN) * cdiv(M, TC_BM);
-  const int ctas = (int)min(tiles, (long long)max(1, 148 / zs));
-  dim3 grid(ctas, 1, zs);
-  kern<<<grid, TC_THREADS, smem, st>>>(ta, tb, ep, M, N, K, per);
-  TACORL_LAUNCH_CHECK();
-  return 0;
-}
-
 __global__ void tc_splitk_reduce_kernel(int M, int N, int splits, const float* __restrict__ partial, TcEpilogue ep) {
   const long long total = (long long)M * N;
   for (long long idx = blockIdx.x * (long long)blockDim.x + threadIdx.x; idx < total;
@@ -1314,8 +1345,65 @@
   return v;
 }
 
-int gemm_tc_bf16(const void* A, long long lda, int a_mn, const void* B, long long ldb, int b_mn, int M, int N,
-                 int K, const TcArgs& e, float* ws, size_t ws_bytes, cudaStream_t st) {
+struct TcGroupHost {
+  TcGroup<TC_MAX_GROUP> g;
+  int splits[TC_MAX_GROUP];
+  size_t ws_used = 0;
+  TcGroupHost() { g.n = 0; }
+};
+
+template <int NP>
+static int tc_launch(const TcGroup<TC_MAX_GROUP>& src, const int* order, cudaStream_t st) {
+  TcGroup<NP> g;
+  g.n = src.n;
+  int tiles = 0, bn_max = 32;
+  for (int i = 0; i < g.n; ++i) {
+    g.p[i] = src.p[order[i]];
+    g.p[i].tile_begin = tiles;
+    tiles += g.p[i].tiles_mn * (cdiv(cdiv(g.p[i].K, TC_BK), g.p[i].kb_per_split));
+    bn_max = std::max(bn_max, g.p[i].bn);
+  }
+  g.total_tiles = tiles;
+  g.stage_bytes = TC_BM * TC_BK * 2 + bn_max * TC_BK * 2;
+  g.stages = bn_max >= 128 ? 5 : 6;
+  const size_t smem = (size_t)g.stages * g.stage_bytes + (2 * TC_MAX_STAGES + 4) * 8 + 16 + 1024;
+  static bool configured = false;
+  if (!configured) {
+    TACORL_CHECK_CUDA(cudaFuncSetAttribute(gemm_tc_kernel<NP>, cudaFuncAttributeMaxDynamicSharedMemorySize, 227 * 1024));
+    configured = true;
+  }
+  gemm_tc_kernel<NP><<<std::min(tiles, 148), TC_THREADS, smem, st>>>(g);
+  TACORL_LAUNCH_CHECK();
+  return 0;
+}
+
+static int tc_flush(TcGroupHost& h, cudaStream_t st) {
+  TcGroup<TC_MAX_GROUP>& g = h.g;
+  if (g.n == 0) return 0;
+  int order[TC_MAX_GROUP];
+  for (int i = 0; i < g.n; ++i) order[i] = i;
+  auto len = [&](int i) { const TcProblem& P = g.p[i]; return P.kb_step ? (P.kb_per_split / P.kb_step + 1) * P.kb_live : P.kb_per_split; };
+  std::stable_sort(order, order + g.n, [&](int x, int y) { return len(x) > len(y); });
+  int rc = g.n == 1 ? tc_launch<1>(g, order, st) : tc_launch<TC_MAX_GROUP>(g, order, st);
+  if (rc) return rc;
+  for (int i = 0; i < g.n; ++i) {
+    if (h.splits[i] <= 1) continue;
+    TcEpilogue ep = g.p[i].ep;
+    const float* partial = ep.partial;
+    ep.partial = nullptr;
+    const long long total = (long long)g.p[i].M * g.p[i].N;
+    tc_splitk_reduce_kernel<<<(int)std::min((long long)1184, (total + 255) / 256), 256, 0, st>>>(g.p[i].M, g.p[i].N, h.splits[i],
+                                                                                               partial, ep);
+    TACORL_LAUNCH_CHECK();
+  }
+  g.n = 0;
+  h.ws_used = 0;
+  return 0;
+}
+
+static int tc_add(TcGroupHost& h, const TcGemm& m, float* ws, size_t ws_bytes, cudaStream_t st) {
+  const int M = m.M, N = m.N, K = m.K, a_mn = m.a_mn, b_mn = m.b_mn;
+  const TcArgs& e = m.e;
   if (M == 0 || N == 0) return 0;
   TACORL_REQUIRE(K > 0, "gemm_tc: K must be positive");
   int BN = N <= 32 ? 32 : (N <= 64 ? 64 : 128);
@@ -1323,17 +1411,14 @@
   if (skinny) BN = b_mn ? 64 : 32;
   if (b_mn && BN < 64) BN = 64;
   int rc;
+  TcEpilogue ep;
+  ep.alpha = e.alpha; ep.beta = e.beta; ep.C = e.C; ep.ldc = e.ldc; ep.Cb = (__nv_bfloat16*)e.Cb; ep.ldcb = e.ldcb;
+  ep.bias = e.bias; ep.act = e.act; ep.Cpre = e.Cpre; ep.ldpre = e.ldpre; ep.partial = nullptr;
+  ep.gate = e.gate; ep.ldgate = e.ldgate;
   if (skinny && !a_mn && !b_mn) {
-    TcEpilogue ep;
-    ep.alpha = e.alpha; ep.beta = e.beta; ep.C = e.C; ep.ldc = e.ldc; ep.Cb = (__nv_bfloat16*)e.Cb; ep.ldcb = e.ldcb;
-    ep.bias = e.bias; ep.act = e.act; ep.Cpre = e.Cpre; ep.ldpre = e.ldpre; ep.partial = nullptr;
-    ep.gate = e.gate; ep.ldgate = e.ldgate;
-    rc = launch_skinny_cluster(A, lda, B, ldb, M, N, K, ep, st);
+    rc = launch_skinny_cluster(m.A, m.lda, m.B, m.ldb, M, N, K, ep, st);
     if (rc <= 0) return rc;
   }
-  CUtensorMap ta, tb;
-  if ((rc = a_mn ? make_tmap(&ta, A, M, K, lda, 64, 64) : make_tmap(&ta, A, K, M, lda, 64, TC_BM))) return rc;
-  if ((rc = b_mn ? make_tmap(&tb, B, N, K, ldb, 64, 64) : make_tmap(&tb, B, K, N, ldb, 64, BN))) return rc;
   const long long ctas = (long long)cdiv(M, TC_BM) * cdiv(N, BN);
   const int total_kb = cdiv(K, TC_BK);
   int splits = e.split_k;
@@ -1346,30 +1431,43 @@
     splits = ws ? (int)(ws_bytes / ((size_t)M * N * 4)) : 1;
     if (splits < 1) splits = 1;
   }
-  TcEpilogue ep;
-  ep.alpha = e.alpha; ep.beta = e.beta; ep.C = e.C; ep.ldc = e.ldc; ep.Cb = (__nv_bfloat16*)e.Cb; ep.ldcb = e.ldcb;
-  ep.bias = e.bias; ep.act = e.act; ep.Cpre = e.Cpre; ep.ldpre = e.ldpre; ep.partial = splits > 1 ? ws : nullptr;
-  ep.gate = e.gate; ep.ldgate = e.ldgate;
-#define TC_DISPATCH(BNV)                                                                                   \
-  if (BN == BNV) {                                                                                         \
-    if (!a_mn && !b_mn) rc = launch_tc<BNV, false, false>(ta, tb, ep, M, N, K, splits, st);                \
-    else if (a_mn && !b_mn) rc = launch_tc<BNV, true, false>(ta, tb, ep, M, N, K, splits, st);             \
-    else if (!a_mn && b_mn) rc = launch_tc<(BNV < 64 ? 64 : BNV), false, true>(ta, tb, ep, M, N, K, splits, st); \
-    else rc = launch_tc<(BNV < 64 ? 64 : BNV), true, true>(ta, tb, ep, M, N, K, splits, st);               \
-  }
-  rc = -1;
-  TC_DISPATCH(32) TC_DISPATCH(64) TC_DISPATCH(128)
-#undef TC_DISPATCH
-  if (rc) return rc;
-  if (splits > 1) {
-    const int per = cdiv(total_kb, splits);
-    const int used = cdiv(total_kb, per);
-    ep.partial = nullptr;
-    long long total = (long long)M * N;
-    tc_splitk_reduce_kernel<<<(int)min((long long)1184, (total + 255) / 256), 256, 0, st>>>(M, N, used, ws, ep);
-    TACORL_LAUNCH_CHECK();
-  }
+  const int per = cdiv(total_kb, splits);
+  splits = cdiv(total_kb, per);
+  const size_t part_bytes = splits > 1 ? (((size_t)splits * M * N * 4 + 255) & ~(size_t)255) : 0;
+  if (h.g.n == TC_MAX_GROUP || h.ws_used + part_bytes > ws_bytes)
+    if ((rc = tc_flush(h, st))) return rc;
+  TcProblem& P = h.g.p[h.g.n];
+  if ((rc = a_mn ? make_tmap(&P.tmA, m.A, M, K, m.lda, 64, 64) : make_tmap(&P.tmA, m.A, K, M, m.lda, 64, TC_BM))) return rc;
+  if ((rc = b_mn ? make_tmap(&P.tmB, m.B, N, K, m.ldb, 64, 64) : make_tmap(&P.tmB, m.B, K, N, m.ldb, 64, BN))) return rc;
+  ep.partial = splits > 1 ? ws + h.ws_used / 4 : nullptr;
+  P.ep = ep;
+  P.M = M; P.N = N; P.K = K; P.bn = BN; P.a_mn = a_mn; P.b_mn = b_mn;
+  P.kb_per_split = per;
+  P.tiles_n = cdiv(N, BN);
+  P.tiles_mn = cdiv(M, TC_BM) * P.tiles_n;
+  P.tile_begin = 0;
+  const bool skip = m.step_rows > 0 && m.step_rows % TC_BK == 0 && m.grad_rows > 0 && m.grad_rows < m.step_rows;
+  P.kb_step = skip ? m.step_rows / TC_BK : 0;
+  P.kb_live = skip ? cdiv(m.grad_rows, TC_BK) : 0;
+  h.splits[h.g.n] = splits;
+  h.ws_used += part_bytes;
+  ++h.g.n;
   return 0;
+}
+
+int gemm_tc_group(const TcGemm* g, int n, float* ws, size_t ws_bytes, cudaStream_t st) {
+  TcGroupHost h;
+  int rc;
+  for (int i = 0; i < n; ++i)
+    if ((rc = tc_add(h, g[i], ws, ws_bytes, st))) return rc;
+  return tc_flush(h, st);
+}
+
+int gemm_tc_bf16(const void* A, long long lda, int a_mn, const void* B, long long ldb, int b_mn, int M, int N,
+                 int K, const TcArgs& e, float* ws, size_t ws_bytes, cudaStream_t st) {
+  TcGemm m;
+  m.A = A; m.lda = lda; m.a_mn = a_mn; m.B = B; m.ldb = ldb; m.b_mn = b_mn; m.M = M; m.N = N; m.K = K; m.e = e;
+  return gemm_tc_group(&m, 1, ws, ws_bytes, st);
 }
 
 __global__ void cast_bf16_2d_kernel(const float* __restrict__ src, long long lds, long long rows, int cols,
diff --git a/tacorl_b200/csrc/internal.h b/tacorl_b200/csrc/internal.h
--- a/tacorl_b200/csrc/internal.h
+++ b/tacorl_b200/csrc/internal.h
@@ -38,6 +38,14 @@
 };
 int gemm_tc_bf16(const void* A, long long lda, int a_mn, const void* B, long long ldb, int b_mn, int M, int N,
                  int K, const TcArgs& e, float* ws, size_t ws_bytes, cudaStream_t st);
+struct TcGemm {
+  const void* A = nullptr; long long lda = 0; int a_mn = 0;
+  const void* B = nullptr; long long ldb = 0; int b_mn = 0;
+  int M = 0, N = 0, K = 0;
+  TcArgs e;
+  int step_rows = 0, grad_rows = 0;
+};
+int gemm_tc_group(const TcGemm* g, int n, float* ws, size_t ws_bytes, cudaStream_t st);
 int rnn_seq_tc(const void* Ab, int T, const void* W, long long ldw, int M, int N, int K, int tau0, int dtau, int n_steps,
                float beta, float* C, long long ldc, long long c_ts, const float* gate, long long ldgate, long long gate_ts,
                void* Cb, int act, unsigned* flags, cudaStream_t st);
diff --git a/tacorl_b200/csrc/rnn.cu b/tacorl_b200/csrc/rnn.cu
--- a/tacorl_b200/csrc/rnn.cu
+++ b/tacorl_b200/csrc/rnn.cu
@@ -395,15 +395,19 @@
   TACORL_REQUIRE(L.flags, "rnn_layer2_fwd: workspace too small");
   L.sk = (float*)(ar.base + ar.off); L.sk_bytes = ar.left();
   __nv_bfloat16* outb = (__nv_bfloat16*)out_bf16;
+  TcGemm proj[2];
+  for (int d = 0; d < D; ++d) {
+    const int n = n_steps[d], t_lo = d ? T - n : 0;
+    TcGemm& m = proj[d];
+    m.A = L.xb + (long long)t_lo * B * L.ldxb; m.lda = L.ldxb; m.B = L.wih[d]; m.ldb = Ip; m.M = n * B; m.N = H; m.K = I;
+    m.e.C = out + (long long)t_lo * B * ldo + (long long)d * H; m.e.ldc = ldo; m.e.bias = L.bsum[d];
+    m.e.split_k = n * B <= 128 ? 0 : 1;
+  }
+  if ((rc = gemm_tc_group(proj, D, L.sk, L.sk_bytes, st))) return rc;
   WaveLaneHost lanes[2];
   int n_lanes = 0;
   for (int d = 0; d < D; ++d) {
-    const int n = n_steps[d], t_lo = d ? T - n : 0, t0 = d ? T - 1 : 0;
-    TcArgs in;
-    in.C = out + (long long)t_lo * B * ldo + (long long)d * H; in.ldc = ldo; in.bias = L.bsum[d];
-    in.split_k = n * B <= 128 ? 0 : 1;
-    if ((rc = gemm_tc_bf16(L.xb + (long long)t_lo * B * L.ldxb, L.ldxb, 0, L.wih[d], Ip, 0, n * B, H, I, in, L.sk, L.sk_bytes, st)))
-      return rc;
+    const int n = n_steps[d], t0 = d ? T - 1 : 0;
     relu_rows_kernel<<<ew_blocks((long long)B * H), 256, 0, st>>>(B, H, out + (long long)t0 * B * ldo + (long long)d * H, ldo,
                                                                  outb + (long long)t0 * B * ldo + (long long)d * H, ldo);
     TACORL_LAUNCH_CHECK();
@@ -535,40 +539,51 @@
       }
     }
   }
+  TcGemm grads[5], dx1;
+  int n_grads = 0;
   for (int d = 0; d < D; ++d) {
     const int n = n_steps[d], t_lo = d ? T - n : 0;
     const long long col = (long long)d * H, rows = (long long)n * B;
-    float* dpre = dout + (long long)t_lo * B * lddo + col;
     const __nv_bfloat16* dp = dpb + (long long)t_lo * B * lddo + col;
-    float *dw_ih = dw[4 * d], *dw_hh = dw[4 * d + 1], *db_ih = dw[4 * d + 2], *db_hh = dw[4 * d + 3];
+    float *dw_ih = dw[4 * d], *dw_hh = dw[4 * d + 1];
     if (dw_hh) {
       if (n > 1) {
-        const __nv_bfloat16 *a, *b;
-        if (d == 0) { a = dp + (long long)B * lddo; b = hb + col; }
-        else { a = dp; b = hb + (long long)(t_lo + 1) * B * ldo + col; }
-        TcArgs g;
-        g.C = dw_hh; g.ldc = H; g.split_k = 0;
-        if ((rc = gemm_tc_bf16(a, lddo, 1, b, ldo, 1, H, H, (n - 1) * B, g, sk, sk_bytes, st))) return rc;
+        TcGemm& m = grads[n_grads++];
+        if (d == 0) { m.A = dp + (long long)B * lddo; m.B = hb + col; }
+        else { m.A = dp; m.B = hb + (long long)(t_lo + 1) * B * ldo + col; }
+        m.lda = lddo; m.a_mn = 1; m.ldb = ldo; m.b_mn = 1; m.M = H; m.N = H; m.K = (n - 1) * B;
+        m.e.C = dw_hh; m.e.ldc = H;
+        m.step_rows = B; m.grad_rows = Bg;
       } else {
         TACORL_CHECK_CUDA(cudaMemsetAsync(dw_hh, 0, (size_t)H * H * 4, st));
       }
     }
     if (dw_ih) {
-      TcArgs g;
-      g.C = dw_ih; g.ldc = I; g.split_k = 0;
-      if ((rc = gemm_tc_bf16(dp, lddo, 1, xb + (long long)t_lo * B * ldb_x, ldb_x, 1, H, I, (int)rows, g, sk, sk_bytes, st))) return rc;
-    }
+      TcGemm& m = grads[n_grads++];
+      m.A = dp; m.lda = lddo; m.a_mn = 1; m.B = xb + (long long)t_lo * B * ldb_x; m.ldb = ldb_x; m.b_mn = 1;
+      m.M = H; m.N = I; m.K = (int)rows;
+      m.e.C = dw_ih; m.e.ldc = I;
+      m.step_rows = B; m.grad_rows = Bg;
+    }
+    if (dx) {
+      TcGemm& m = d ? dx1 : grads[n_grads++];
+      m.A = dp; m.lda = lddo; m.B = wih[d]; m.ldb = Ip; m.b_mn = 1; m.M = (int)rows; m.N = I; m.K = H;
+      m.e.C = dx + (long long)t_lo * B * lddx; m.e.ldc = lddx; m.e.beta = d ? 1.f : 0.f; m.e.split_k = 1;
+    }
+  }
+  if ((rc = gemm_tc_group(grads, n_grads, sk, sk_bytes, st))) return rc;
+  for (int d = 0; d < D; ++d) {
+    const int n = n_steps[d], t_lo = d ? T - n : 0;
+    const long long rows = (long long)n * B;
+    float* dpre = dout + (long long)t_lo * B * lddo + (long long)d * H;
+    float *db_ih = dw[4 * d + 2], *db_hh = dw[4 * d + 3];
     if (db_ih || db_hh) {
       float* first = db_ih ? db_ih : db_hh;
       if ((rc = colsum2_f32((int)rows, H, dpre, lddo, first, 0, sk, sk_bytes, st))) return rc;
       if (db_ih && db_hh) TACORL_CHECK_CUDA(cudaMemcpyAsync(db_hh, db_ih, (size_t)H * 4, cudaMemcpyDeviceToDevice, st));
     }
-    if (dx) {
-      TcArgs g;
-      g.C = dx + (long long)t_lo * B * lddx; g.ldc = lddx; g.beta = d ? 1.f : 0.f; g.split_k = 1;
-      if ((rc = gemm_tc_bf16(dp, lddo, 0, wih[d], Ip, 1, (int)rows, I, H, g, sk, sk_bytes, st))) return rc;
-    }
-  }
+  }
+  if (dx && D == 2 && (rc = gemm_tc_group(&dx1, 1, sk, sk_bytes, st))) return rc;
   return 0;
 }
 
diff --git a/tacorl_b200/ops.py b/tacorl_b200/ops.py
--- a/tacorl_b200/ops.py
+++ b/tacorl_b200/ops.py
@@ -129,6 +129,29 @@
     return _frozen_shadow_of(t)
 
 
+_TWINS = {}
+
+
+def register_twin(t, tb):
+    if len(_TWINS) >= 64:
+        for k in [k for k, (ref, _, _) in _TWINS.items() if ref() is None]:
+            del _TWINS[k]
+    _TWINS[t.data_ptr()] = (weakref.ref(t), t._version, tb)
+
+
+def twin_of(t):
+    if _STATE["prec"] != L.PREC_BF16 or t is None or not t.is_cuda or t.dtype != torch.float32 or not t.is_contiguous():
+        return None
+    hit = _TWINS.get(t.data_ptr())
+    if hit is None:
+        return None
+    ref, ver, tb = hit
+    base = ref()
+    if base is None or base.data_ptr() != t.data_ptr() or base.numel() != t.numel() or t._version != ver:
+        return None
+    return tb
+
+
 _GRAD_OWNERS = weakref.WeakSet()
 
 
@@ -193,7 +216,7 @@
         Wc = _c(W)
         out = torch.empty(x2.shape[0], W.shape[0], device=x.device, dtype=torch.float32)
         pre = torch.empty_like(out) if act == L.ACT_SILU else None
-        gemm(x2, Wc, out, transB=True, bias=b, act=act, Cpre=pre, B_bf16=shadow_of(Wc))
+        gemm(x2, Wc, out, transB=True, bias=b, act=act, Cpre=pre, A_bf16=twin_of(x2), B_bf16=shadow_of(Wc))
         ctx.act = act
         ctx.has_bias = b is not None
         ctx.xshape = x.shape
@@ -216,7 +239,7 @@
             dx = dx.view(ctx.xshape)
         if ctx.needs_input_grad[1]:
             dW = torch.empty_like(W)
-            gemm(dz, x2, dW, transA=True)
+            gemm(dz, x2, dW, transA=True, B_bf16=twin_of(x2))
         if ctx.has_bias and ctx.needs_input_grad[2]:
             db = colsum(dz)
         return dx, dW, db, None
@@ -558,6 +581,8 @@
             outs.append(out)
             outbs.append(outb)
             inp, inp_b = out, outb
+        if not last_only:
+            register_twin(inp, inp_b)
         ctx.cfg = (T, B, I, H, D, num_layers, last_only, B if grad_rows is None else int(grad_rows))
         ctx.aux = (outbs, whts, prep_done)
         ctx.save_for_backward(x, *outs, *weights)
```

Result: no change. 332,000 (median of 6 runs) (+0.9%).
